# YaqiXia/Voltrix-SpMM

Hardware: AMD Instinct MI355X
Metric: spmm_gflops (higher is better)
Workload: dtype f16

## Files before the change

### include/voltrix_capi.h

```cpp
#ifndef VOLTRIX_CAPI_H_
#define VOLTRIX_CAPI_H_

#include <stdint.h>

#ifdef __cplusplus
extern "C" {
#endif

#define VOLTRIX_ABI_VERSION 2

#define VOLTRIX_CSR_AUTO (-1)
#define VOLTRIX_SLAB_AUTO (-1)
#define VOLTRIX_BLK_H 16
#define VOLTRIX_BLK_W 8

enum voltrix_rc {
  VOLTRIX_OK = 0,
  VOLTRIX_ERR_BAD_SHAPE = 1,
  VOLTRIX_ERR_LAUNCH = 2,
  VOLTRIX_ERR_BAD_CONFIG = 3,
  VOLTRIX_ERR_OVERFLOW = 4,
  VOLTRIX_ERR_DUPLICATE = 5
};

int voltrix_abi_version(void);


void voltrix_launch_preprocess(void* edge_list, void* node_pointer, int num_nodes, void* block_partition,
                               void* edge_to_column, void* edge_to_row, void* pointer1, int* return_code);

void voltrix_launch_hmat_gen(void* node_pointer, void* edge_list, void* block_partition, void* edge_to_column,
                             void* edge_to_row, void* pointer1, int num_row_windows, int num_nodes, int num_edges,
                             void* hspa, void* hind, int* return_code);

void voltrix_launch_hmat_packed_swizzle(int num_row_windows, void* pointer1, void* hspa, void* hspa_packed,
                                        int* return_code);

void voltrix_launch_spmm(void* blk_offsets, void* hspa_packed, void* hind, int num_nodes, int num_edges,
                         int embedding_dim, void* input, void* output, void* stream, int* return_code);


void voltrix_launch_spmm_f32_tile(void* blk_offsets, void* hspa_packed, void* hind, int num_nodes, int num_edges,
                                  int embedding_dim, void* input, void* output, int fs, int depth, int waves,
                                  void* window_order, void* out_scale, void* stream, int* return_code);

void voltrix_launch_spmm_f16(void* blk_offsets, void* hspa_packed, void* hind, int num_nodes, int num_edges,
                             int embedding_dim, void* input, void* output, void* stream, int* return_code);
void voltrix_launch_spmm_f16_tile(void* blk_offsets, void* hspa_packed, void* hind, int num_nodes, int num_edges,
                                  int embedding_dim, void* input, void* output, int fs, int depth, int waves,
                                  void* window_order, void* out_scale, void* stream, int* return_code);

int64_t voltrix_spmm_f32_workspace_bytes(int64_t input_rows, int embedding_dim);
void voltrix_launch_spmm_f32_as_f16(void* blk_offsets, void* hspa_packed, void* hind, int num_nodes, int num_edges,
                                    int embedding_dim, void* input, int64_t input_rows, void* output, void* workspace,
                                    void* stream, int* return_code);

void voltrix_launch_spmm_bf16(void* blk_offsets, void* hspa_packed, void* hind, int num_nodes, int num_edges,
                              int embedding_dim, void* input, void* output, void* stream, int* return_code);
void voltrix_launch_spmm_bf16_tile(void* blk_offsets, void* hspa_packed, void* hind, int num_nodes, int num_edges,
                                   int embedding_dim, void* input, void* output, int fs, int depth, int waves,
                                   void* window_order, void* out_scale, void* stream, int* return_code);

void voltrix_launch_spmm_f16_sched(void* blk_offsets, void* hspa_packed, void* hind, int num_nodes, int num_edges,
                                   int embedding_dim, void* input, void* output, int fs, int depth, int waves,
                                   void* window_order, void* out_scale, int atomic_out, void* units, void* unit_ptr,
                                   int max_units_per_xcd, void* partials, void* row_map, int units_per_wave, void* stream,
                                   int* return_code);
void voltrix_launch_spmm_bf16_sched(void* blk_offsets, void* hspa_packed, void* hind, int num_nodes, int num_edges,
                                    int embedding_dim, void* input, void* output, int fs, int depth, int waves,
                                    void* window_order, void* out_scale, int atomic_out, void* units, void* unit_ptr,
                                    int max_units_per_xcd, void* partials, void* row_map, int units_per_wave, void* stream,
                                    int* return_code);
void voltrix_launch_combine_partials(void* cuts, int num_cuts, void* partials, void* output, int num_nodes,
                                     int embedding_dim, int accumulate, void* row_map, void* stream, int* return_code);

int64_t voltrix_unit_table_workspace_bytes(int num_nodes);
int64_t voltrix_unit_table_fill_workspace_bytes(int64_t num_units);
void voltrix_launch_unit_table_count(void* blk_offsets, int num_nodes, int max_stages, void* xcd_ptr, void* workspace,
                                     void* header, void* stream, int* return_code);
void voltrix_launch_unit_table_fill(void* blk_offsets, int num_nodes, void* xcd_ptr, void* workspace, void* fill_workspace,
                                    int num_units, int num_cuts, int top, void* units, void* unit_ptr, void* cuts,
                                    void* stream, int* return_code);

int64_t voltrix_stream_table_workspace_bytes(int num_nodes);
int64_t voltrix_stream_table_fill_workspace_bytes(int64_t num_units);
void voltrix_launch_stream_table_count(void* blk_offsets, void* hspa_packed, void* hind, int num_nodes, int run_cost,
                                       int cut_stages, void* workspace, void* header, void* stream, int* return_code);
void voltrix_launch_stream_table_fill(void* blk_offsets, int num_nodes, void* workspace, void* fill_workspace, int num_units,
                                      int num_cuts, int run_bound, int run_cost, void* units, void* cuts, void* runs,
                                      void* run_ptr, void* header2, void* stream, int* return_code);
void voltrix_launch_spmm_stream_f16(void* hspa_packed, void* hind, int num_nodes, int embedding_dim, void* input,
                                    int64_t input_rows, void* output, void* units, void* runs, void* run_ptr,
                                    int max_runs_per_xcd, void* partials, void* out_scale, int fs, int depth, int waves,
                                    int slab_policy, void* stream, int* return_code);
void voltrix_launch_spmm_stream_bf16(void* hspa_packed, void* hind, int num_nodes, int embedding_dim, void* input,
                                     int64_t input_rows, void* output, void* units, void* runs, void* run_ptr,
                                     int max_runs_per_xcd, void* partials, void* out_scale, int fs, int depth, int waves,
                                     int slab_policy, void* stream, int* return_code);

void voltrix_launch_window_order(void* blk_offsets, int num_nodes, int chunk, void* order_out, void* stream,
                                 int* return_code);

#define VOLTRIX_PANEL_KSTEPS_PIPELINED 17
void voltrix_launch_spmm_panel_f16(void* panel_ptr, void* panel_cols, void* panel_bits, void* panel_order, void* xcd_ptr,
                                   int max_panels_per_xcd, int num_nodes, int embedding_dim, void* input, int64_t input_rows, void* output,
                                   int accumulate, int fs, int depth, int waves, int row_blocks, int ksteps,
                                   int slab_policy, void* out_scale, void* stream, int* return_code);
void voltrix_launch_spmm_panel_bf16(void* panel_ptr, void* panel_cols, void* panel_bits, void* panel_order, void* xcd_ptr,
                                    int max_panels_per_xcd, int num_nodes, int embedding_dim, void* input, int64_t input_rows, void* output,
                                    int accumulate, int fs, int depth, int waves, int row_blocks, int ksteps,
                                    int slab_policy, void* out_scale, void* stream, int* return_code);

void voltrix_launch_spmm_panel_parts_f16(void* panel_ptr, void* panel_cols, void* panel_bits, void* parts, int num_parts,
                                         void* xcd_ptr, int max_parts_per_xcd, void* partials, int num_nodes, int embedding_dim,
                                         void* input, int64_t input_rows, void* output, int accumulate, int fs, int depth,
                                         int waves, int row_blocks, int ksteps, int slab_policy, void* out_scale, void* stream,
                                         int* return_code);
void voltrix_launch_spmm_panel_parts_bf16(void* panel_ptr, void* panel_cols, void* panel_bits, void* parts, int num_parts,
                                          void* xcd_ptr, int max_parts_per_xcd, void* partials, int num_nodes, int embedding_dim,
                                          void* input, int64_t input_rows, void* output, int accumulate, int fs, int depth,
                                          int waves, int row_blocks, int ksteps, int slab_policy, void* out_scale, void* stream,
                                          int* return_code);
void voltrix_launch_combine_panel_partials(void* cuts, int num_cuts, void* partials, void* output, int num_nodes,
                                           int embedding_dim, int panel_rows, int accumulate, void* stream, int* return_code);

void voltrix_launch_xcd_ranges_of_work(void* work, int num_items, int align, void* xcd_ptr, void* stream, int* return_code);
void voltrix_launch_xcd_ranges_of_windows(void* blk_offsets, int num_nodes, int align, void* xcd_ptr, void* stream,
                                          int* return_code);
void voltrix_launch_xcd_ranges_of_panels(void* panel_ptr, void* resid_blk_offsets, int num_nodes, int panel_rows,
                                         int kstep_cost_x10, void* xcd_ptr, void* window_xcd_ptr, void* stream,
                                         int* return_code);
int64_t voltrix_panel_parts_workspace_bytes(int num_panels);
void voltrix_launch_panel_parts_count(void* panel_ptr, int num_panels, int cap, void* panel_xcd_ptr, void* workspace,
                                      void* header, void* stream, int* return_code);
void voltrix_launch_panel_parts_fill(void* panel_ptr, int num_panels, int cap, void* panel_xcd_ptr, void* workspace,
                                     void* parts, void* part_xcd_ptr, void* cuts, void* stream, int* return_code);

void voltrix_launch_spmm_fused_f16(void* panel_ptr, void* panel_cols, void* panel_bits, void* panel_order, void* xcd_ptr,
                                   int max_panels_per_xcd, void* wave_ptr, void* records, int num_nodes, int embedding_dim, void* input,
                                   void* output, int fs, int depth, int pace_blocks, void* out_scale, void* stream,
                                   int* return_code);
void voltrix_launch_spmm_fused_bf16(void* panel_ptr, void* panel_cols, void* panel_bits, void* panel_order, void* xcd_ptr,
                                    int max_panels_per_xcd, void* wave_ptr, void* records, int num_nodes, int embedding_dim, void* input,
                                    void* output, int fs, int depth, int pace_blocks, void* out_scale, void* stream,
                                   int* return_code);

void voltrix_fused_panel_geometry(int* waves, int* row_blocks);
int64_t voltrix_fused_records_workspace_bytes(int num_nodes);
void voltrix_launch_fused_records_count(void* blk_offsets, void* hspa_packed, int num_nodes, void* workspace, void* wave_ptr,
                                        void* stream, int* return_code);
void voltrix_launch_fused_records_fill(void* blk_offsets, void* hspa_packed, void* hind, int num_nodes, void* wave_ptr,
                                       int64_t num_records, void* records, void* stream, int* return_code);

int64_t voltrix_panel_plan_workspace_bytes(int num_nodes, int waves, int row_blocks);
void voltrix_launch_panel_plan_count(void* node_pointer, void* edge_list, int num_nodes, int num_cols, int64_t num_edges,
                                     int waves, int row_blocks, int tau, void* workspace, void* panel_ptr,
                                     void* resid_node_pointer, void* status, void* stream, int* return_code);
void voltrix_launch_panel_plan_fill(void* node_pointer, void* edge_list, int num_nodes, int num_cols, int64_t num_edges,
                                    int waves, int row_blocks, int tau, void* workspace, void* panel_ptr,
                                    void* resid_node_pointer, int64_t total_ksteps, void* resid_edge_list,
                                    void* panel_cols, void* panel_bits, void* stream, int* return_code);

void voltrix_launch_panel_order(void* panel_ptr, int num_panels, int group, void* xcd_ptr, void* order_out, void* stream,
                                int* return_code);

void voltrix_spmm_default_tile(int embedding_dim, int is_f16, int* fs, int* depth, int* waves);

int voltrix_spmm_num_tiles(int is_f16);
void voltrix_spmm_tile_at(int is_f16, int index, int* fs, int* depth, int* waves);

void voltrix_launch_cast_f32_f16(void* src, void* dst, int64_t count, void* stream, int* return_code);

void voltrix_launch_cast_f32_f16_scaled(void* src, void* dst, int64_t count, void* scale, void* stream,
                                        int* return_code);

void voltrix_launch_spmm_csr_rows(void* indptr, void* indices, int num_rows, int embedding_dim, void* input, int dtype, void* output,
                                  int xcd_ranges, void* stream, int* return_code);

void voltrix_launch_spmm_csr_rows_weighted(void* indptr, void* indices, void* values, int num_rows, int embedding_dim, void* input, int dtype,
                                           void* output, int xcd_ranges, void* stream, int* return_code);

void voltrix_launch_scatter_values(void* values, void* slots, void* plane, int64_t count, int dtype, void* stream, int* return_code);

void voltrix_launch_sddmm_csr(void* indptr, void* indices, int num_rows, int64_t nnz, int embedding_dim, void* x, int x_dtype, void* y,
                              int y_dtype, void* out, void* stream, int* return_code);

int64_t voltrix_edge_softmax_workspace_bytes(int num_rows, int64_t nnz);
void voltrix_launch_edge_softmax_csr(void* indptr, int num_rows, int64_t nnz, void* scores, float scale, void* out, void* workspace,
                                     void* stream, int* return_code);

void voltrix_launch_edge_softmax_backward_csr(void* indptr, int num_rows, int64_t nnz, void* alpha, void* grad_alpha, float scale,
                                              void* grad_scores, void* workspace, void* stream, int* return_code);

void voltrix_launch_sddmm_heads_csr(void* indptr, void* indices, int num_rows, int64_t nnz, int heads, int head_dim, void* x, int x_dtype,
                                    void* y, int y_dtype, void* out, void* stream, int* return_code);

int64_t voltrix_edge_softmax_heads_workspace_bytes(int num_rows, int64_t nnz, int heads);
void voltrix_launch_edge_softmax_heads_csr(void* indptr, int num_rows, int64_t nnz, int heads, void* scores, float scale, void* out,
                                           void* workspace, void* stream, int* return_code);
void voltrix_launch_edge_softmax_heads_backward_csr(void* indptr, int num_rows, int64_t nnz, int heads, void* alpha, void* grad_alpha,
                                                    float scale, void* grad_scores, void* workspace, void* stream, int* return_code);

void voltrix_launch_spmm_csr_heads(void* indptr, void* indices, void* values, int num_rows, int heads, int head_dim, void* input,
                                   int dtype, void* output, void* stream, int* return_code);

void voltrix_launch_gat_score_csr(void* indptr, void* indices, int num_rows, int64_t nnz, int heads, void* el, void* er, float slope,
                                  void* out, void* stream, int* return_code);

int64_t voltrix_gat_score_workspace_bytes(int num_rows, int64_t nnz, int heads);
void voltrix_launch_gat_score_rowsum_csr(void* indptr, void* indices, void* order, int num_rows, int64_t nnz, int heads, void* a, void* b,
                                         void* grad, float slope, void* out, void* workspace, void* stream, int* return_code);

void voltrix_launch_gatv2_score_csr(void* indptr, void* indices, int num_rows, int64_t nnz, int heads, int head_dim, void* xl, void* xr,
                                    int dtype, void* a, float slope, void* out, void* stream, int* return_code);

void voltrix_launch_gatv2_rowsum_csr(void* indptr, void* indices, void* order, int num_rows, int64_t nnz, int heads, int head_dim, void* p,
                                     void* q, int dtype, void* grad, float slope, void* out, void* stream, int* return_code);

void voltrix_launch_attn_aggregate_csr(void* indptr, void* indices, void* scores, int num_rows, int64_t nnz, int heads, int head_dim,
                                       void* feat, int dtype, float scale, void* out, void* m, void* l, void* stream, int* return_code);

void voltrix_launch_attn_aggregate_grad_scores_csr(void* indptr, void* indices, int num_rows, int64_t nnz, int heads, int head_dim,
                                                   void* grad_out, void* feat, int dtype, void* scores, void* m, void* l, void* delta,
                                                   float scale, void* grad_scores, void* stream, int* return_code);

void voltrix_launch_attn_aggregate_grad_feat_csr(void* t_indptr, void* t_indices, void* order, int num_cols, int64_t nnz, int heads,
                                                 int head_dim, void* grad_out, int dtype, void* scores, void* m, void* l, float scale,
                                                 void* grad_feat, void* stream, int* return_code);

void voltrix_launch_dropout_mask(int64_t nnz, int heads, uint32_t threshold, uint64_t seed, uint64_t offset, void* mask, void* stream,
                                 int* return_code);

void voltrix_launch_attn_aggregate_dropout_csr(void* indptr, void* indices, void* scores, int num_rows, int64_t nnz, int heads,
                                               int head_dim, void* feat, int dtype, float scale, void* out, void* m, void* l, void* mask,
                                               float keep_scale, void* stream, int* return_code);
void voltrix_launch_attn_aggregate_dropout_grad_scores_csr(void* indptr, void* indices, int num_rows, int64_t nnz, int heads,
                                                           int head_dim, void* grad_out, void* feat, int dtype, void* scores, void* m,
                                                           void* l, void* delta, float scale, void* grad_scores, void* mask,
                                                           float keep_scale, void* stream, int* return_code);
void voltrix_launch_attn_aggregate_dropout_grad_feat_csr(void* t_indptr, void* t_indices, void* order, int num_cols, int64_t nnz,
                                                         int heads, int head_dim, void* grad_out, int dtype, void* scores, void* m,
                                                         void* l, float scale, void* grad_feat, void* mask, float keep_scale,
                                                         void* stream, int* return_code);

void voltrix_launch_scale_rows(void* src, void* scale, void* dst, int64_t rows, int num_feats, int dtype, void* stream,
                               int* return_code);

int64_t voltrix_csr_preprocess_workspace_bytes(int num_nodes, int num_cols, int64_t num_edges, int path);
void voltrix_launch_csr_window_count(void* node_pointer, void* edge_list, int num_nodes, int num_cols, int64_t num_edges,
                                     int path, void* workspace, void* block_partition, void* pointer1, void* status,
                                     void* stream, int* return_code);
void voltrix_launch_csr_fill(void* node_pointer, void* edge_list, int num_nodes, int num_cols, int64_t num_edges,
                             int path, void* workspace, void* pointer1, void* hspa_packed, void* hind, void* stream,
                             int* return_code);

int64_t voltrix_csr_transpose_workspace_bytes(int64_t num_edges);
void voltrix_launch_csr_transpose(void* indptr, void* indices, int num_rows, int num_cols, int64_t num_edges, void* workspace,
                                  void* t_indptr, void* t_indices, void* stream, int* return_code);
void voltrix_launch_bfs_seed(int start, int num_nodes, void* level, void* queue, void* ctrl, void* level_off, void* stream,
                             int* return_code);
void voltrix_launch_bfs_levels(void* indptr, void* indices, void* t_indptr, void* t_indices, int num_nodes, int t_rows,
                               void* level, void* queue, void* ctrl, void* level_off, int wide_levels, void* stream,
                               int* return_code);
int64_t voltrix_cm_rank_workspace_bytes(int64_t max_level);
void voltrix_launch_cm_rank(void* indptr, void* indices, void* t_indptr, void* t_indices, int num_nodes, int t_rows,
                            void* level, void* rank, void* tie, void* queue, void* level_off, const int* level_off_host,
                            int num_levels, int base, void* workspace, void* stream, int* return_code);

void voltrix_launch_chol_inv_transposed(void* gram, int k, double eps, void* out, void* stream, int* return_code);

#ifdef __cplusplus
}
#endif
#endif
```

### voltrix-spmm_amd/csrc/capi_spmm_panel.hip

```cpp
#include <hip/hip_runtime.h>

#include "voltrix/panel_plan.hpp"
#include "voltrix/spmm_panel_kernels.hpp"
#include "voltrix_capi.h"

namespace {

#define VOLTRIX_PANEL_SPACE(X)                                                                       \
  X(128, 3, 8, 4, 1) X(128, 4, 8, 4, 1) X(128, 6, 8, 4, 1) X(128, 8, 8, 4, 1) X(128, 4, 4, 4, 1) X(128, 6, 4, 4, 1) X(128, 8, 4, 4, 1) \
  X(128, 4, 8, 2, 1) X(128, 6, 8, 2, 1) X(128, 8, 8, 2, 1) X(128, 6, 4, 2, 1)                                    \
  X(64, 4, 4, 4, 1) X(64, 6, 4, 4, 1) X(64, 4, 8, 4, 2) X(64, 6, 8, 4, 2) X(64, 6, 4, 4, 2)                      \
  X(32, 4, 4, 4, 2) X(32, 6, 4, 4, 2) X(32, 6, 8, 4, 2) X(64, 6, 4, 2, 2) X(64, 6, 8, 2, 2) X(32, 6, 4, 2, 2) X(32, 6, 8, 2, 2) \
  X(128, 3, 4, 4, 1) X(128, 4, 4, 2, 1)

constexpr int kPipelined = 17;
static_assert(kPipelined == VOLTRIX_PANEL_KSTEPS_PIPELINED, "include/voltrix_capi.h");
#define VOLTRIX_PANEL_PIPE_SPACE(X) X(128, 3, 8, 4) X(128, 4, 8, 4) X(128, 4, 8, 2) X(128, 6, 8, 2) X(64, 4, 8, 4) X(64, 6, 8, 4)

template <bool BF16>
int dispatch(int fs, int depth, int waves, int rb, int ks, const int* panel_ptr, const int* panel_cols,
             const uint32_t* panel_bits, const int* panel_order, int num_nodes, int embedding_dim, const void* input,
             float* output, int accumulate, const float* out_scale, hipStream_t stream, int64_t input_rows,
             int slab_policy, const int* xcd_ptr, int max_panels_per_xcd, const int* parts = nullptr, int num_parts = 0,
             float* partials = nullptr) {
#define X(FS, D, W, RB, KS)                                                                                          \
  if (fs == FS && depth == D && waves == W && rb == RB && ks == KS)                                                  \
    return voltrix::launch_spmm_panel<voltrix::PanelTile<FS, D, W, RB, KS, BF16>>(                                   \
        panel_ptr, panel_cols, panel_bits, panel_order, num_nodes, embedding_dim, input, output, accumulate, out_scale, \
        stream, 0, 0, input_rows, slab_policy, xcd_ptr, max_panels_per_xcd, parts, num_parts, partials);
  VOLTRIX_PANEL_SPACE(X)
#undef X
#define X(FS, D, W, RB)                                                                                              \
  if (fs == FS && depth == D && waves == W && rb == RB && ks == kPipelined)                                           \
    return voltrix::launch_spmm_panel<voltrix::PanelTile<FS, D, W, RB, 1, BF16, true>>(                               \
        panel_ptr, panel_cols, panel_bits, panel_order, num_nodes, embedding_dim, input, output, accumulate, out_scale, \
        stream, 0, 0, input_rows, slab_policy, xcd_ptr, max_panels_per_xcd, parts, num_parts, partials);
  VOLTRIX_PANEL_PIPE_SPACE(X)
#undef X
  return voltrix::kErrBadConfig;
}

}

extern "C" {

void voltrix_launch_spmm_panel_f16(void* panel_ptr, void* panel_cols, void* panel_bits, void* panel_order, void* xcd_ptr,
                                   int max_panels_per_xcd, int num_nodes, int embedding_dim, void* input, int64_t input_rows, void* output,
                                   int accumulate, int fs, int depth, int waves, int row_blocks, int ksteps,
                                   int slab_policy, void* out_scale, void* stream, int* return_code) {
  *return_code = dispatch<false>(fs, depth, waves, row_blocks, ksteps, static_cast<const int*>(panel_ptr),
                                 static_cast<const int*>(panel_cols), static_cast<const uint32_t*>(panel_bits),
                                 static_cast<const int*>(panel_order), num_nodes, embedding_dim, input,
                                 static_cast<float*>(output), accumulate, static_cast<const float*>(out_scale),
                                 static_cast<hipStream_t>(stream), input_rows, slab_policy,
                                 static_cast<const int*>(xcd_ptr), max_panels_per_xcd);
}

void voltrix_launch_spmm_panel_bf16(void* panel_ptr, void* panel_cols, void* panel_bits, void* panel_order, void* xcd_ptr,
                                    int max_panels_per_xcd, int num_nodes, int embedding_dim, void* input, int64_t input_rows, void* output,
                                    int accumulate, int fs, int depth, int waves, int row_blocks, int ksteps,
                                    int slab_policy, void* out_scale, void* stream, int* return_code) {
  *return_code = dispatch<true>(fs, depth, waves, row_blocks, ksteps, static_cast<const int*>(panel_ptr),
                                static_cast<const int*>(panel_cols), static_cast<const uint32_t*>(panel_bits),
                                static_cast<const int*>(panel_order), num_nodes, embedding_dim, input,
                                static_cast<float*>(output), accumulate, static_cast<const float*>(out_scale),
                                static_cast<hipStream_t>(stream), input_rows, slab_policy,
                                static_cast<const int*>(xcd_ptr), max_panels_per_xcd);
}

void voltrix_launch_spmm_panel_parts_f16(void* panel_ptr, void* panel_cols, void* panel_bits, void* parts, int num_parts,
                                         void* xcd_ptr, int max_parts_per_xcd, void* partials, int num_nodes, int embedding_dim,
                                         void* input, int64_t input_rows, void* output, int accumulate, int fs, int depth,
                                         int waves, int row_blocks, int ksteps, int slab_policy, void* out_scale, void* stream,
                                         int* return_code) {
  *return_code = parts == nullptr ? voltrix::kErrBadShape
                                  : dispatch<false>(fs, depth, waves, row_blocks, ksteps, static_cast<const int*>(panel_ptr),
                                                    static_cast<const int*>(panel_cols), static_cast<const uint32_t*>(panel_bits),
                                                    nullptr, num_nodes, embedding_dim, input, static_cast<float*>(output),
                                                    accumulate, static_cast<const float*>(out_scale),
                                                    static_cast<hipStream_t>(stream), input_rows, slab_policy,
                                                    static_cast<const int*>(xcd_ptr), max_parts_per_xcd,
                                                    static_cast<const int*>(parts), num_parts, static_cast<float*>(partials));
}

void voltrix_launch_spmm_panel_parts_bf16(void* panel_ptr, void* panel_cols, void* panel_bits, void* parts, int num_parts,
                                          void* xcd_ptr, int max_parts_per_xcd, void* partials, int num_nodes, int embedding_dim,
                                          void* input, int64_t input_rows, void* output, int accumulate, int fs, int depth,
                                          int waves, int row_blocks, int ksteps, int slab_policy, void* out_scale, void* stream,
                                          int* return_code) {
  *return_code = parts == nullptr ? voltrix::kErrBadShape
                                  : dispatch<true>(fs, depth, waves, row_blocks, ksteps, static_cast<const int*>(panel_ptr),
                                                   static_cast<const int*>(panel_cols), static_cast<const uint32_t*>(panel_bits),
                                                   nullptr, num_nodes, embedding_dim, input, static_cast<float*>(output),
                                                   accumulate, static_cast<const float*>(out_scale),
                                                   static_cast<hipStream_t>(stream), input_rows, slab_policy,
                                                   static_cast<const int*>(xcd_ptr), max_parts_per_xcd,
                                                   static_cast<const int*>(parts), num_parts, static_cast<float*>(partials));
}

void voltrix_launch_combine_panel_partials(void* cuts, int num_cuts, void* partials, void* output, int num_nodes,
                                           int embedding_dim, int panel_rows, int accumulate, void* stream, int* return_code) {
  *return_code = voltrix::launch_combine_panel_partials(static_cast<const int*>(cuts), num_cuts,
                                                        static_cast<const float*>(partials), static_cast<float*>(output),
                                                        num_nodes, embedding_dim, panel_rows, accumulate,
                                                        static_cast<hipStream_t>(stream));
}

void voltrix_launch_panel_order(void* panel_ptr, int num_panels, int group, void* xcd_ptr, void* order_out, void* stream,
                                int* return_code) {
  *return_code = voltrix::panel_order(static_cast<const int*>(panel_ptr), num_panels, group, static_cast<int*>(order_out),
                                      static_cast<hipStream_t>(stream), static_cast<const int*>(xcd_ptr));
}

int64_t voltrix_panel_plan_workspace_bytes(int num_nodes, int waves, int row_blocks) {
  return voltrix::panel_plan_workspace_bytes(num_nodes, waves, row_blocks);
}

void voltrix_launch_panel_plan_count(void* node_pointer, void* edge_list, int num_nodes, int num_cols, int64_t num_edges,
                                     int waves, int row_blocks, int tau, void* workspace, void* panel_ptr,
                                     void* resid_node_pointer, void* status, void* stream, int* return_code) {
  *return_code = voltrix::panel_plan_count(static_cast<const int*>(node_pointer), static_cast<const int*>(edge_list),
                                           num_nodes, num_cols, num_edges, waves, row_blocks, tau, workspace,
                                           static_cast<int*>(panel_ptr), static_cast<int*>(resid_node_pointer),
                                           static_cast<int*>(status), static_cast<hipStream_t>(stream));
}

void voltrix_launch_panel_plan_fill(void* node_pointer, void* edge_list, int num_nodes, int num_cols, int64_t num_edges,
                                    int waves, int row_blocks, int tau, void* workspace, void* panel_ptr,
                                    void* resid_node_pointer, int64_t total_ksteps, void* resid_edge_list,
                                    void* panel_cols, void* panel_bits, void* stream, int* return_code) {
  *return_code = voltrix::panel_plan_fill(static_cast<const int*>(node_pointer), static_cast<const int*>(edge_list),
                                          num_nodes, num_cols, num_edges, waves, row_blocks, tau, workspace,
                                          static_cast<const int*>(panel_ptr), static_cast<const int*>(resid_node_pointer),
                                          total_ksteps, static_cast<int*>(resid_edge_list), static_cast<int*>(panel_cols),
                                          static_cast<uint32_t*>(panel_bits), static_cast<hipStream_t>(stream));
}

}
```

### voltrix-spmm_amd/voltrix/capi.py

```python
from __future__ import annotations

import ctypes
import os
import subprocess

_PKG = os.path.dirname(os.path.abspath(__file__))
_ROOT = os.path.dirname(_PKG)
LIB_PATH = os.path.join(_ROOT, "lib", "libvoltrix_hip.so")
CSRC_DIR = os.path.join(_ROOT, "csrc")

_lib = None

SYMBOLS = (
    "voltrix_abi_version",
    "voltrix_launch_preprocess",
    "voltrix_launch_hmat_gen",
    "voltrix_launch_hmat_packed_swizzle",
    "voltrix_launch_spmm",
    "voltrix_launch_spmm_f32_tile",
    "voltrix_launch_spmm_f16",
    "voltrix_launch_spmm_f16_tile",
    "voltrix_spmm_f32_workspace_bytes",
    "voltrix_launch_spmm_f32_as_f16",
    "voltrix_launch_spmm_f16_sched",
    "voltrix_launch_spmm_bf16_sched",
    "voltrix_launch_combine_partials",
    "voltrix_stream_table_workspace_bytes",
    "voltrix_stream_table_fill_workspace_bytes",
    "voltrix_launch_stream_table_count",
    "voltrix_launch_stream_table_fill",
    "voltrix_launch_spmm_stream_f16",
    "voltrix_launch_spmm_stream_bf16",
    "voltrix_launch_spmm_panel_f16",
    "voltrix_launch_spmm_panel_bf16",
    "voltrix_launch_spmm_panel_parts_f16",
    "voltrix_launch_spmm_panel_parts_bf16",
    "voltrix_launch_combine_panel_partials",
    "voltrix_launch_xcd_ranges_of_work",
    "voltrix_launch_xcd_ranges_of_windows",
    "voltrix_launch_xcd_ranges_of_panels",
    "voltrix_panel_parts_workspace_bytes",
    "voltrix_launch_panel_parts_count",
    "voltrix_launch_panel_parts_fill",
    "voltrix_launch_spmm_fused_f16",
    "voltrix_launch_spmm_fused_bf16",
    "voltrix_fused_panel_geometry",
    "voltrix_fused_records_workspace_bytes",
    "voltrix_launch_fused_records_count",
    "voltrix_launch_fused_records_fill",
    "voltrix_panel_plan_workspace_bytes",
    "voltrix_launch_panel_plan_count",
    "voltrix_launch_panel_plan_fill",
    "voltrix_launch_panel_order",
    "voltrix_spmm_default_tile",
    "voltrix_spmm_num_tiles",
    "voltrix_spmm_tile_at",
    "voltrix_launch_window_order",
    "voltrix_launch_spmm_bf16",
    "voltrix_launch_spmm_bf16_tile",
    "voltrix_launch_cast_f32_f16",
    "voltrix_launch_cast_f32_f16_scaled",
    "voltrix_launch_scale_rows",
    "voltrix_launch_spmm_csr_rows",
    "voltrix_launch_spmm_csr_rows_weighted",
    "voltrix_launch_scatter_values",
    "voltrix_launch_sddmm_csr",
    "voltrix_edge_softmax_workspace_bytes",
    "voltrix_launch_edge_softmax_csr",
    "voltrix_launch_edge_softmax_backward_csr",
    "voltrix_launch_sddmm_heads_csr",
    "voltrix_edge_softmax_heads_workspace_bytes",
    "voltrix_launch_edge_softmax_heads_csr",
    "voltrix_launch_edge_softmax_heads_backward_csr",
    "voltrix_launch_spmm_csr_heads",
    "voltrix_launch_gat_score_csr",
    "voltrix_gat_score_workspace_bytes",
    "voltrix_launch_gat_score_rowsum_csr",
    "voltrix_launch_gatv2_score_csr",
    "voltrix_launch_gatv2_rowsum_csr",
    "voltrix_launch_attn_aggregate_csr",
    "voltrix_launch_attn_aggregate_grad_scores_csr",
    "voltrix_launch_attn_aggregate_grad_feat_csr",
    "voltrix_launch_dropout_mask",
    "voltrix_launch_attn_aggregate_dropout_csr",
    "voltrix_launch_attn_aggregate_dropout_grad_scores_csr",
    "voltrix_launch_attn_aggregate_dropout_grad_feat_csr",
    "voltrix_csr_preprocess_workspace_bytes",
    "voltrix_launch_csr_window_count",
    "voltrix_launch_csr_fill",
    "voltrix_unit_table_workspace_bytes",
    "voltrix_unit_table_fill_workspace_bytes",
    "voltrix_launch_unit_table_count",
    "voltrix_launch_unit_table_fill",
    "voltrix_csr_transpose_workspace_bytes",
    "voltrix_launch_csr_transpose",
    "voltrix_launch_bfs_seed",
    "voltrix_launch_bfs_levels",
    "voltrix_cm_rank_workspace_bytes",
    "voltrix_launch_cm_rank",
    "voltrix_launch_chol_inv_transposed",
)


def build(force: bool = False) -> str:
    cmd = ["make", "-s", "-C", CSRC_DIR, "-j4"]
    if force:
        subprocess.check_call(["make", "-s", "-C", CSRC_DIR, "clean"])
    subprocess.check_call(cmd)
    return LIB_PATH


def lib() -> ctypes.CDLL:
    global _lib
    if _lib is None:
        if not os.path.exists(LIB_PATH):
            build()
        _lib = ctypes.CDLL(LIB_PATH)
        _lib.voltrix_abi_version.restype = ctypes.c_int
        _lib.voltrix_spmm_num_tiles.restype = ctypes.c_int
        _lib.voltrix_csr_preprocess_workspace_bytes.restype = ctypes.c_int64
        _lib.voltrix_panel_plan_workspace_bytes.restype = ctypes.c_int64
        _lib.voltrix_spmm_f32_workspace_bytes.restype = ctypes.c_int64
        _lib.voltrix_fused_records_workspace_bytes.restype = ctypes.c_int64
        _lib.voltrix_unit_table_workspace_bytes.restype = ctypes.c_int64
        _lib.voltrix_unit_table_fill_workspace_bytes.restype = ctypes.c_int64
        _lib.voltrix_cm_rank_workspace_bytes.restype = ctypes.c_int64
        _lib.voltrix_csr_transpose_workspace_bytes.restype = ctypes.c_int64
        _lib.voltrix_edge_softmax_workspace_bytes.restype = ctypes.c_int64
        _lib.voltrix_edge_softmax_heads_workspace_bytes.restype = ctypes.c_int64
        _lib.voltrix_gat_score_workspace_bytes.restype = ctypes.c_int64
        for name in SYMBOLS:
            if name.startswith("voltrix_launch_") or name in ("voltrix_spmm_default_tile", "voltrix_spmm_tile_at"):
                getattr(_lib, name).restype = None
    return _lib


class VoltrixError(RuntimeError):
    pass


_RC = {1: "bad shape / alignment", 2: "HIP launch error", 3: "tile configuration not instantiated",
       4: "int32 overflow of the block format", 5: "duplicate CSR entries"}


def check(rc: int, what: str) -> None:
    if rc != 0:
        raise VoltrixError(f"{what}: return code {rc} ({_RC.get(rc, 'unknown')})")


def _ptr(t):
    return ctypes.c_void_p(t.data_ptr())


def default_tile(embedding_dim: int, is_f16: bool):
    fs, d, w = ctypes.c_int(), ctypes.c_int(), ctypes.c_int()
    lib().voltrix_spmm_default_tile(ctypes.c_int(embedding_dim), ctypes.c_int(int(is_f16)), ctypes.byref(fs),
                                    ctypes.byref(d), ctypes.byref(w))
    return fs.value, d.value, w.value


def tiles(is_f16: bool):
    out = []
    for i in range(lib().voltrix_spmm_num_tiles(ctypes.c_int(int(is_f16)))):
        fs, d, w = ctypes.c_int(), ctypes.c_int(), ctypes.c_int()
        lib().voltrix_spmm_tile_at(ctypes.c_int(int(is_f16)), ctypes.c_int(i), ctypes.byref(fs), ctypes.byref(d),
                                   ctypes.byref(w))
        out.append((fs.value, d.value, w.value))
    return out


CSR_PATHS = {None: -1, "auto": -1, "sort": 0, "bitmap": 1, "mixed": 2}
SLAB_AUTO, SLAB_ONE_GRID, SLAB_LAUNCHES = -1, 0, 1


def csr_preprocess_workspace_bytes(num_nodes: int, num_cols: int, num_edges: int, path=None) -> int:
    return int(lib().voltrix_csr_preprocess_workspace_bytes(ctypes.c_int(num_nodes), ctypes.c_int(num_cols),
                                                            ctypes.c_int64(num_edges), ctypes.c_int(CSR_PATHS[path])))


def launch_csr_window_count(indptr, indices, num_nodes, num_cols, workspace, block_partition, pointer1, status,
                            stream, path=None) -> None:
    rc = ctypes.c_int(-1)
    lib().voltrix_launch_csr_window_count(_ptr(indptr), _ptr(indices), ctypes.c_int(num_nodes), ctypes.c_int(num_cols),
                                          ctypes.c_int64(indices.numel()), ctypes.c_int(CSR_PATHS[path]), _ptr(workspace),
                                          _ptr(block_partition), _ptr(pointer1), _ptr(status), ctypes.c_void_p(stream),
                                          ctypes.byref(rc))
    check(rc.value, "voltrix_launch_csr_window_count")


def launch_csr_fill(indptr, indices, num_nodes, num_cols, workspace, pointer1, hspa_packed, hind, stream, path=None) -> None:
    rc = ctypes.c_int(-1)
    lib().voltrix_launch_csr_fill(_ptr(indptr), _ptr(indices), ctypes.c_int(num_nodes), ctypes.c_int(num_cols),
                                  ctypes.c_int64(indices.numel()), ctypes.c_int(CSR_PATHS[path]), _ptr(workspace),
                                  _ptr(pointer1), _ptr(hspa_packed), _ptr(hind), ctypes.c_void_p(stream), ctypes.byref(rc))
    check(rc.value, "voltrix_launch_csr_fill")


def launch_spmm(blk_offsets, hspa_packed, hind, num_nodes, num_edges, embedding_dim, input_ptr, output_ptr, is_f16,
                tile, stream, window_order=0, out_scale=0) -> int:
    rc = ctypes.c_int(-1)
    if is_f16 == "bf16":
        fn = lib().voltrix_launch_spmm_bf16_tile
    else:
        fn = lib().voltrix_launch_spmm_f16_tile if is_f16 else lib().voltrix_launch_spmm_f32_tile
    fn(ctypes.c_void_p(blk_offsets), ctypes.c_void_p(hspa_packed), ctypes.c_void_p(hind), ctypes.c_int(num_nodes),
       ctypes.c_int(num_edges), ctypes.c_int(embedding_dim), ctypes.c_void_p(input_ptr), ctypes.c_void_p(output_ptr),
       ctypes.c_int(tile[0]), ctypes.c_int(tile[1]), ctypes.c_int(tile[2]), ctypes.c_void_p(window_order),
       ctypes.c_void_p(out_scale), ctypes.c_void_p(stream), ctypes.byref(rc))
    return rc.value


def launch_spmm_sched(blk_offsets, hspa_packed, hind, num_nodes, num_edges, embedding_dim, input_ptr, output_ptr, tile,
                      stream, window_order=0, out_scale=0, atomic_out=False, bf16=False, table=None, partials=0,
                      row_map=0, units_per_wave=1) -> int:
    rc = ctypes.c_int(-1)
    fn = lib().voltrix_launch_spmm_bf16_sched if bf16 else lib().voltrix_launch_spmm_f16_sched
    fn(ctypes.c_void_p(blk_offsets), ctypes.c_void_p(hspa_packed), ctypes.c_void_p(hind), ctypes.c_int(num_nodes),
       ctypes.c_int(num_edges), ctypes.c_int(embedding_dim), ctypes.c_void_p(input_ptr), ctypes.c_void_p(output_ptr),
       ctypes.c_int(tile[0]), ctypes.c_int(tile[1]), ctypes.c_int(tile[2]), ctypes.c_void_p(window_order),
       ctypes.c_void_p(out_scale), ctypes.c_int(int(atomic_out)),
       ctypes.c_void_p(table.units.data_ptr() if table is not None else 0),
       ctypes.c_void_p(table.unit_ptr.data_ptr() if table is not None else 0),
       ctypes.c_int(table.max_units_per_xcd if table is not None else 0), ctypes.c_void_p(partials),
       ctypes.c_void_p(row_map), ctypes.c_int(int(units_per_wave)), ctypes.c_void_p(stream), ctypes.byref(rc))
    return rc.value


def launch_combine_partials(table, partials_ptr, output_ptr, num_nodes, embedding_dim, accumulate, stream,
                            row_map=0) -> int:
    rc = ctypes.c_int(-1)
    lib().voltrix_launch_combine_partials(ctypes.c_void_p(table.cuts.data_ptr()), ctypes.c_int(table.num_cuts),
                                          ctypes.c_void_p(partials_ptr), ctypes.c_void_p(output_ptr),
                                          ctypes.c_int(num_nodes), ctypes.c_int(embedding_dim),
                                          ctypes.c_int(int(accumulate)), ctypes.c_void_p(row_map),
                                          ctypes.c_void_p(stream), ctypes.byref(rc))
    return rc.value


def build_unit_table(blk_offsets, num_nodes: int, max_stages: int = 0, stream=None, xcd_ptr=None):
    import torch

    dev = blk_offsets.device
    stream = torch.cuda.current_stream().cuda_stream if stream is None else stream
    workspace = torch.empty(max(16, int(lib().voltrix_unit_table_workspace_bytes(ctypes.c_int(num_nodes)))),
                            dtype=torch.uint8, device=dev)
    header = torch.empty(8, dtype=torch.int32, device=dev)
    rc = ctypes.c_int(-1)
    xp = ctypes.c_void_p(xcd_ptr.data_ptr() if xcd_ptr is not None else 0)
    lib().voltrix_launch_unit_table_count(_ptr(blk_offsets), ctypes.c_int(num_nodes), ctypes.c_int(int(max_stages)), xp,
                                          _ptr(workspace), _ptr(header), ctypes.c_void_p(stream), ctypes.byref(rc))
    check(rc.value, "voltrix_launch_unit_table_count")
    head = [int(v) for v in header.tolist()]
    num_units, num_cuts, top = head[0], head[1], head[5]
    units = torch.empty((num_units, 4), dtype=torch.int32, device=dev)
    cuts = torch.empty((num_cuts, 4), dtype=torch.int32, device=dev)
    unit_ptr = torch.empty(9, dtype=torch.int32, device=dev)
    fill_ws = torch.empty(max(16, int(lib().voltrix_unit_table_fill_workspace_bytes(ctypes.c_int64(num_units)))),
                          dtype=torch.uint8, device=dev)
    lib().voltrix_launch_unit_table_fill(_ptr(blk_offsets), ctypes.c_int(num_nodes), xp, _ptr(workspace), _ptr(fill_ws),
                                         ctypes.c_int(num_units), ctypes.c_int(num_cuts), ctypes.c_int(top), _ptr(units),
                                         _ptr(unit_ptr), _ptr(cuts), ctypes.c_void_p(stream), ctypes.byref(rc))
    check(rc.value, "voltrix_launch_unit_table_fill")
    return units, unit_ptr, cuts, head


def build_stream_table(blk_offsets, hspa_packed, hind, num_nodes: int, run_cost: int = 0, cut_stages: int = 0, stream=None):
    import torch

    dev = blk_offsets.device
    stream = torch.cuda.current_stream().cuda_stream if stream is None else stream
    L = lib()
    workspace = torch.empty(max(16, int(L.voltrix_stream_table_workspace_bytes(ctypes.c_int(num_nodes)))), dtype=torch.uint8,
                            device=dev)
    header = torch.empty(8, dtype=torch.int32, device=dev)
    rc = ctypes.c_int(-1)
    L.voltrix_launch_stream_table_count(_ptr(blk_offsets), _ptr(hspa_packed), _ptr(hind), ctypes.c_int(num_nodes),
                                        ctypes.c_int(int(run_cost)), ctypes.c_int(int(cut_stages)), _ptr(workspace),
                                        _ptr(header), ctypes.c_void_p(stream), ctypes.byref(rc))
    check(rc.value, "voltrix_launch_stream_table_count")
    num_units, num_cuts, num_slots, run_bound, rcost, cut = [int(v) for v in header.tolist()][:6]
    units = torch.empty((num_units, 8), dtype=torch.int32, device=dev)
    cuts = torch.empty((num_cuts, 4), dtype=torch.int32, device=dev)
    runs = torch.empty((max(1, run_bound), 4), dtype=torch.int32, device=dev)
    run_ptr = torch.empty(9, dtype=torch.int32, device=dev)
    header2 = torch.empty(4, dtype=torch.int32, device=dev)
    fill_ws = torch.empty(max(16, int(L.voltrix_stream_table_fill_workspace_bytes(ctypes.c_int64(num_units)))),
                          dtype=torch.uint8, device=dev)
    L.voltrix_launch_stream_table_fill(_ptr(blk_offsets), ctypes.c_int(num_nodes), _ptr(workspace), _ptr(fill_ws),
                                       ctypes.c_int(num_units), ctypes.c_int(num_cuts), ctypes.c_int(run_bound),
                                       ctypes.c_int(max(2, rcost)), _ptr(units), _ptr(cuts), _ptr(runs), _ptr(run_ptr),
                                       _ptr(header2), ctypes.c_void_p(stream), ctypes.byref(rc))
    check(rc.value, "voltrix_launch_stream_table_fill")
    num_runs, max_runs, oversized = [int(v) for v in header2.tolist()][:3]
    assert oversized == 0, "stream table with a run of more than 64 units (run_cost > 128?): the kernel cannot walk it"
    return units, runs[:num_runs], run_ptr, cuts, (num_units, num_cuts, num_slots, num_runs, max_runs, rcost, cut)


def launch_spmm_stream(hspa_packed, hind, num_nodes: int, embedding_dim: int, feat, output, table, partials, out_scale=None,
                       tile=(0, 0, 0), stream=None, input_rows: int = 0, slab_policy: int = -1) -> int:
    import torch

    stream = torch.cuda.current_stream().cuda_stream if stream is None else stream
    fn = lib().voltrix_launch_spmm_stream_bf16 if feat.dtype == torch.bfloat16 else lib().voltrix_launch_spmm_stream_f16
    from .utils import timed_launch

    rc = ctypes.c_int(-1)
    with timed_launch("spmm_stream", stream):
        fn(_ptr(hspa_packed), _ptr(hind), ctypes.c_int(num_nodes), ctypes.c_int(embedding_dim), _ptr(feat),
           ctypes.c_int64(int(input_rows)), _ptr(output), _ptr(table.units), _ptr(table.runs), _ptr(table.run_ptr),
           ctypes.c_int(table.max_runs_per_xcd), _ptr(partials), ctypes.c_void_p(out_scale.data_ptr() if out_scale is not None else 0),
           ctypes.c_int(tile[0]), ctypes.c_int(tile[1]), ctypes.c_int(tile[2]), ctypes.c_int(int(slab_policy)),
           ctypes.c_void_p(stream), ctypes.byref(rc))
    return rc.value


def xcd_ranges_of_work(work, align: int = 1, stream=None):
    import torch

    out = torch.empty(9, dtype=torch.int32, device=work.device)
    rc = ctypes.c_int(-1)
    stream = torch.cuda.current_stream().cuda_stream if stream is None else stream
    lib().voltrix_launch_xcd_ranges_of_work(_ptr(work), ctypes.c_int(work.numel()), ctypes.c_int(int(align)), _ptr(out),
                                            ctypes.c_void_p(stream), ctypes.byref(rc))
    check(rc.value, "voltrix_launch_xcd_ranges_of_work")
    return out


def xcd_ranges_of_windows(blk_offsets, num_nodes: int, align: int = 1, stream=None):
    import torch

    out = torch.empty(9, dtype=torch.int32, device=blk_offsets.device)
    rc = ctypes.c_int(-1)
    stream = torch.cuda.current_stream().cuda_stream if stream is None else stream
    lib().voltrix_launch_xcd_ranges_of_windows(_ptr(blk_offsets), ctypes.c_int(num_nodes), ctypes.c_int(int(align)), _ptr(out),
                                               ctypes.c_void_p(stream), ctypes.byref(rc))
    check(rc.value, "voltrix_launch_xcd_ranges_of_windows")
    return out


def xcd_ranges_of_panels(panel_ptr, resid_blk_offsets, num_nodes: int, panel_rows: int, kstep_cost_x10: int, stream=None):
    import torch

    dev = panel_ptr.device
    out, out_w = torch.empty(9, dtype=torch.int32, device=dev), torch.empty(9, dtype=torch.int32, device=dev)
    rc = ctypes.c_int(-1)
    stream = torch.cuda.current_stream().cuda_stream if stream is None else stream
    lib().voltrix_launch_xcd_ranges_of_panels(_ptr(panel_ptr), _ptr(resid_blk_offsets), ctypes.c_int(num_nodes),
                                              ctypes.c_int(panel_rows), ctypes.c_int(int(kstep_cost_x10)), _ptr(out),
                                              _ptr(out_w), ctypes.c_void_p(stream), ctypes.byref(rc))
    check(rc.value, "voltrix_launch_xcd_ranges_of_panels")
    return out, out_w


def build_panel_parts(panel_ptr, cap: int, panel_xcd_ptr=None, stream=None):
    import torch

    dev = panel_ptr.device
    num_panels = panel_ptr.numel() - 1
    stream = torch.cuda.current_stream().cuda_stream if stream is None else stream
    workspace = torch.empty(max(16, int(lib().voltrix_panel_parts_workspace_bytes(ctypes.c_int(num_panels)))),
                            dtype=torch.uint8, device=dev)
    header = torch.empty(8, dtype=torch.int32, device=dev)
    rc = ctypes.c_int(-1)
    xp = ctypes.c_void_p(panel_xcd_ptr.data_ptr() if panel_xcd_ptr is not None else 0)
    lib().voltrix_launch_panel_parts_count(_ptr(panel_ptr), ctypes.c_int(num_panels), ctypes.c_int(int(cap)), xp,
                                           _ptr(workspace), _ptr(header), ctypes.c_void_p(stream), ctypes.byref(rc))
    check(rc.value, "voltrix_launch_panel_parts_count")
    head = [int(v) for v in header.tolist()]
    parts = torch.empty((head[0], 4), dtype=torch.int32, device=dev)
    cuts = torch.empty((max(1, head[1]), 4), dtype=torch.int32, device=dev)
    part_xcd_ptr = torch.empty(9, dtype=torch.int32, device=dev)
    lib().voltrix_launch_panel_parts_fill(_ptr(panel_ptr), ctypes.c_int(num_panels), ctypes.c_int(int(cap)), xp,
                                          _ptr(workspace), _ptr(parts), _ptr(part_xcd_ptr), _ptr(cuts),
                                          ctypes.c_void_p(stream), ctypes.byref(rc))
    check(rc.value, "voltrix_launch_panel_parts_fill")
    return parts, part_xcd_ptr, cuts[:head[1]], head


def spmm_f32_workspace_bytes(input_rows: int, embedding_dim: int) -> int:
    return int(lib().voltrix_spmm_f32_workspace_bytes(ctypes.c_int64(input_rows), ctypes.c_int(embedding_dim)))


def launch_spmm_f32_as_f16(blk_offsets, hspa_packed, hind, num_nodes, num_edges, embedding_dim, feat, output, workspace,
                           stream) -> int:
    rc = ctypes.c_int(-1)
    lib().voltrix_launch_spmm_f32_as_f16(_ptr(blk_offsets), _ptr(hspa_packed), _ptr(hind), ctypes.c_int(num_nodes),
                                         ctypes.c_int(num_edges), ctypes.c_int(embedding_dim), _ptr(feat),
                                         ctypes.c_int64(feat.shape[0]), _ptr(output), _ptr(workspace),
                                         ctypes.c_void_p(stream), ctypes.byref(rc))
    return rc.value


def launch_spmm_panel(plan, input_ptr, output_ptr, embedding_dim, accumulate, bf16, tile, out_scale, stream,
                      input_rows: int = 0, slab_policy: int = SLAB_AUTO, partials_ptr: int = 0) -> int:
    rc = ctypes.c_int(-1)
    parts = getattr(plan, "parts", None)
    if parts is not None:
        fn = lib().voltrix_launch_spmm_panel_parts_bf16 if bf16 else lib().voltrix_launch_spmm_panel_parts_f16
        fn(_ptr(plan.panel_ptr), _ptr(plan.panel_cols), _ptr(plan.panel_bits), _ptr(parts.parts), ctypes.c_int(parts.num_parts),
           _ptr(parts.xcd_ptr), ctypes.c_int(parts.max_parts_per_xcd), ctypes.c_void_p(partials_ptr),
           ctypes.c_int(plan.num_nodes), ctypes.c_int(embedding_dim), ctypes.c_void_p(input_ptr), ctypes.c_int64(input_rows),
           ctypes.c_void_p(output_ptr), ctypes.c_int(int(accumulate)), ctypes.c_int(tile[0]), ctypes.c_int(tile[1]),
           ctypes.c_int(plan.waves), ctypes.c_int(plan.row_blocks), ctypes.c_int(tile[2]), ctypes.c_int(slab_policy),
           ctypes.c_void_p(out_scale), ctypes.c_void_p(stream), ctypes.byref(rc))
        return rc.value
    fn = lib().voltrix_launch_spmm_panel_bf16 if bf16 else lib().voltrix_launch_spmm_panel_f16
    order = plan.panel_order.data_ptr() if plan.panel_order is not None else 0
    xcd_ptr = getattr(plan, "xcd_ptr", None)
    fn(_ptr(plan.panel_ptr), _ptr(plan.panel_cols), _ptr(plan.panel_bits), ctypes.c_void_p(order),
       ctypes.c_void_p(xcd_ptr.data_ptr() if xcd_ptr is not None else 0),
       ctypes.c_int(plan.max_panels_per_xcd if xcd_ptr is not None else 0), ctypes.c_int(plan.num_nodes), ctypes.c_int(embedding_dim), ctypes.c_void_p(input_ptr), ctypes.c_int64(input_rows),
       ctypes.c_void_p(output_ptr), ctypes.c_int(int(accumulate)), ctypes.c_int(tile[0]), ctypes.c_int(tile[1]),
       ctypes.c_int(plan.waves), ctypes.c_int(plan.row_blocks), ctypes.c_int(tile[2]), ctypes.c_int(slab_policy),
       ctypes.c_void_p(out_scale), ctypes.c_void_p(stream), ctypes.byref(rc))
    return rc.value


def launch_combine_panel_partials(parts, partials_ptr, output_ptr, num_nodes, embedding_dim, panel_rows, accumulate,
                                  stream) -> int:
    rc = ctypes.c_int(-1)
    lib().voltrix_launch_combine_panel_partials(_ptr(parts.cuts), ctypes.c_int(parts.num_cuts), ctypes.c_void_p(partials_ptr),
                                                ctypes.c_void_p(output_ptr), ctypes.c_int(num_nodes),
                                                ctypes.c_int(embedding_dim), ctypes.c_int(panel_rows),
                                                ctypes.c_int(int(accumulate)), ctypes.c_void_p(stream), ctypes.byref(rc))
    return rc.value


def launch_spmm_fused(plan, fused, input_ptr, output_ptr, embedding_dim, bf16, tile, out_scale, stream,
                      pace_blocks: int = 0) -> int:
    rc = ctypes.c_int(-1)
    fn = lib().voltrix_launch_spmm_fused_bf16 if bf16 else lib().voltrix_launch_spmm_fused_f16
    order = plan.panel_order.data_ptr() if plan.panel_order is not None else 0
    xcd_ptr = getattr(plan, "xcd_ptr", None)
    fn(_ptr(plan.panel_ptr), _ptr(plan.panel_cols), _ptr(plan.panel_bits), ctypes.c_void_p(order),
       ctypes.c_void_p(xcd_ptr.data_ptr() if xcd_ptr is not None else 0),
       ctypes.c_int(plan.max_panels_per_xcd if xcd_ptr is not None else 0), _ptr(fused.wave_ptr),
       _ptr(fused.records), ctypes.c_int(plan.num_nodes), ctypes.c_int(embedding_dim), ctypes.c_void_p(input_ptr),
       ctypes.c_void_p(output_ptr), ctypes.c_int(tile[0]), ctypes.c_int(tile[1]), ctypes.c_int(int(pace_blocks)),
       ctypes.c_void_p(out_scale), ctypes.c_void_p(stream), ctypes.byref(rc))
    return rc.value


def fused_panel_geometry():
    waves, row_blocks = ctypes.c_int(0), ctypes.c_int(0)
    lib().voltrix_fused_panel_geometry(ctypes.byref(waves), ctypes.byref(row_blocks))
    assert waves.value * row_blocks.value * 16 == 512, (waves.value, row_blocks.value)
    return waves.value, row_blocks.value


def build_fused_records(blk_offsets, hspa_packed, hind, num_nodes: int, stream=None):
    import torch

    dev = blk_offsets.device
    stream = torch.cuda.current_stream().cuda_stream if stream is None else stream
    num_waves = fused_panel_geometry()[0] * ((num_nodes + 511) // 512)
    workspace = torch.empty(max(16, int(lib().voltrix_fused_records_workspace_bytes(ctypes.c_int(num_nodes)))),
                            dtype=torch.uint8, device=dev)
    wave_ptr = torch.empty(num_waves + 1, dtype=torch.int32, device=dev)
    rc = ctypes.c_int(-1)
    lib().voltrix_launch_fused_records_count(_ptr(blk_offsets), _ptr(hspa_packed), ctypes.c_int(num_nodes), _ptr(workspace),
                                             _ptr(wave_ptr), ctypes.c_void_p(stream), ctypes.byref(rc))
    check(rc.value, "voltrix_launch_fused_records_count")
    num_records = int(wave_ptr[-1])
    assert 0 <= num_records <= 4 * (hspa_packed.numel() // 16 + 1), num_records
    records = torch.empty((num_records + 1, 64), dtype=torch.int32, device=dev).view(torch.uint32)
    lib().voltrix_launch_fused_records_fill(_ptr(blk_offsets), _ptr(hspa_packed), _ptr(hind), ctypes.c_int(num_nodes),
                                            _ptr(wave_ptr), ctypes.c_int64(num_records), _ptr(records),
                                            ctypes.c_void_p(stream), ctypes.byref(rc))
    check(rc.value, "voltrix_launch_fused_records_fill")
    return wave_ptr, records, num_records


def launch_panel_order(panel_ptr, num_panels: int, order_out, stream, group: int = 1, xcd_ptr=None) -> None:
    rc = ctypes.c_int(-1)
    lib().voltrix_launch_panel_order(_ptr(panel_ptr), ctypes.c_int(num_panels), ctypes.c_int(group),
                                     ctypes.c_void_p(xcd_ptr.data_ptr() if xcd_ptr is not None else 0), _ptr(order_out),
                                     ctypes.c_void_p(stream), ctypes.byref(rc))
    check(rc.value, "voltrix_launch_panel_order")


def panel_plan_workspace_bytes(num_nodes: int, waves: int, row_blocks: int) -> int:
    return int(lib().voltrix_panel_plan_workspace_bytes(ctypes.c_int(num_nodes), ctypes.c_int(waves),
                                                        ctypes.c_int(row_blocks)))


def launch_panel_plan_count(indptr, indices, num_nodes, num_cols, waves, row_blocks, tau, workspace, panel_ptr,
                            resid_indptr, status, stream) -> int:
    rc = ctypes.c_int(-1)
    lib().voltrix_launch_panel_plan_count(_ptr(indptr), _ptr(indices), ctypes.c_int(num_nodes), ctypes.c_int(num_cols),
                                          ctypes.c_int64(indices.numel()), ctypes.c_int(waves), ctypes.c_int(row_blocks),
                                          ctypes.c_int(tau), _ptr(workspace), _ptr(panel_ptr), _ptr(resid_indptr),
                                          _ptr(status), ctypes.c_void_p(stream), ctypes.byref(rc))
    return rc.value


def launch_panel_plan_fill(indptr, indices, num_nodes, num_cols, waves, row_blocks, tau, workspace, panel_ptr,
                           resid_indptr, total_ksteps, resid_indices, panel_cols, panel_bits, stream) -> None:
    rc = ctypes.c_int(-1)
    lib().voltrix_launch_panel_plan_fill(_ptr(indptr), _ptr(indices), ctypes.c_int(num_nodes), ctypes.c_int(num_cols),
                                         ctypes.c_int64(indices.numel()), ctypes.c_int(waves), ctypes.c_int(row_blocks),
                                         ctypes.c_int(tau), _ptr(workspace), _ptr(panel_ptr), _ptr(resid_indptr),
                                         ctypes.c_int64(total_ksteps), _ptr(resid_indices), _ptr(panel_cols),
                                         _ptr(panel_bits), ctypes.c_void_p(stream), ctypes.byref(rc))
    check(rc.value, "voltrix_launch_panel_plan_fill")


def launch_window_order(blk_offsets, num_nodes, order_out, stream, chunk: int = 256) -> None:
    rc = ctypes.c_int(-1)
    lib().voltrix_launch_window_order(_ptr(blk_offsets), ctypes.c_int(num_nodes), ctypes.c_int(chunk), _ptr(order_out),
                                      ctypes.c_void_p(stream), ctypes.byref(rc))
    check(rc.value, "voltrix_launch_window_order")


def launch_cast_f32_f16(src, dst, stream) -> None:
    rc = ctypes.c_int(-1)
    lib().voltrix_launch_cast_f32_f16(_ptr(src), _ptr(dst), ctypes.c_int64(src.numel()), ctypes.c_void_p(stream),
                                      ctypes.byref(rc))
    check(rc.value, "voltrix_launch_cast_f32_f16")


_cast_scaled = None


def launch_cast_f32_f16_scaled(src, dst, scale, stream) -> None:
    global _cast_scaled
    if _cast_scaled is None:
        fn = lib().voltrix_launch_cast_f32_f16_scaled
        fn.argtypes = [ctypes.c_void_p, ctypes.c_void_p, ctypes.c_int64, ctypes.c_void_p, ctypes.c_void_p,
                       ctypes.POINTER(ctypes.c_int)]
        _cast_scaled = fn
    rc = ctypes.c_int(-1)
    _cast_scaled(src.data_ptr(), dst.data_ptr(), src.numel(), scale.data_ptr(), stream, rc)
    if rc.value != 0:
        check(rc.value, "voltrix_launch_cast_f32_f16_scaled")


_P, _I, _L, _F, _RC_P = ctypes.c_void_p, ctypes.c_int, ctypes.c_int64, ctypes.c_float, ctypes.POINTER(ctypes.c_int)
_U32, _U64 = ctypes.c_uint32, ctypes.c_uint64
_ARGTYPES = {
    "voltrix_launch_spmm_csr_rows": [_P, _P, _I, _I, _P, _I, _P, _I, _P, _RC_P],
    "voltrix_launch_spmm_csr_rows_weighted": [_P, _P, _P, _I, _I, _P, _I, _P, _I, _P, _RC_P],
    "voltrix_launch_sddmm_csr": [_P, _P, _I, _L, _I, _P, _I, _P, _I, _P, _P, _RC_P],
    "voltrix_launch_edge_softmax_csr": [_P, _I, _L, _P, _F, _P, _P, _P, _RC_P],
    "voltrix_launch_edge_softmax_backward_csr": [_P, _I, _L, _P, _P, _F, _P, _P, _P, _RC_P],
    "voltrix_launch_sddmm_heads_csr": [_P, _P, _I, _L, _I, _I, _P, _I, _P, _I, _P, _P, _RC_P],
    "voltrix_launch_edge_softmax_heads_csr": [_P, _I, _L, _I, _P, _F, _P, _P, _P, _RC_P],
    "voltrix_launch_edge_softmax_heads_backward_csr": [_P, _I, _L, _I, _P, _P, _F, _P, _P, _P, _RC_P],
    "voltrix_launch_spmm_csr_heads": [_P, _P, _P, _I, _I, _I, _P, _I, _P, _P, _RC_P],
    "voltrix_launch_gat_score_csr": [_P, _P, _I, _L, _I, _P, _P, _F, _P, _P, _RC_P],
    "voltrix_launch_gat_score_rowsum_csr": [_P, _P, _P, _I, _L, _I, _P, _P, _P, _F, _P, _P, _P, _RC_P],
    "voltrix_launch_gatv2_score_csr": [_P, _P, _I, _L, _I, _I, _P, _P, _I, _P, _F, _P, _P, _RC_P],
    "voltrix_launch_gatv2_rowsum_csr": [_P, _P, _P, _I, _L, _I, _I, _P, _P, _I, _P, _F, _P, _P, _RC_P],
    "voltrix_launch_attn_aggregate_csr": [_P, _P, _P, _I, _L, _I, _I, _P, _I, _F, _P, _P, _P, _P, _RC_P],
    "voltrix_launch_attn_aggregate_grad_scores_csr": [_P, _P, _I, _L, _I, _I, _P, _P, _I, _P, _P, _P, _P, _F, _P, _P, _RC_P],
    "voltrix_launch_attn_aggregate_grad_feat_csr": [_P, _P, _P, _I, _L, _I, _I, _P, _I, _P, _P, _P, _F, _P, _P, _RC_P],
    "voltrix_launch_dropout_mask": [_L, _I, _U32, _U64, _U64, _P, _P, _RC_P],
    "voltrix_launch_attn_aggregate_dropout_csr": [_P, _P, _P, _I, _L, _I, _I, _P, _I, _F, _P, _P, _P, _P, _F, _P, _RC_P],
    "voltrix_launch_attn_aggregate_dropout_grad_scores_csr": [_P, _P, _I, _L, _I, _I, _P, _P, _I, _P, _P, _P, _P, _F, _P, _P, _F, _P,
                                                              _RC_P],
    "voltrix_launch_attn_aggregate_dropout_grad_feat_csr": [_P, _P, _P, _I, _L, _I, _I, _P, _I, _P, _P, _P, _F, _P, _P, _F, _P, _RC_P],
    "voltrix_launch_scatter_values": [_P, _P, _P, _L, _I, _P, _RC_P],
    "voltrix_launch_scale_rows": [_P, _P, _P, _L, _I, _I, _P, _RC_P],
}
_bound_fns = {}


def _bound(name: str):
    fn = _bound_fns.get(name)
    if fn is None:
        fn = getattr(lib(), name)
        fn.argtypes = _ARGTYPES[name]
        _bound_fns[name] = fn
    return fn


def launch_spmm_csr_rows(indptr, indices, num_rows: int, feat, output, stream, xcd_ranges: int = 0, values=None) -> None:
    import torch

    assert indptr.dtype == torch.int32 and indices.dtype == torch.int32 and indptr.numel() == num_rows + 1
    assert feat.dim() == 2 and feat.is_contiguous() and output.is_contiguous() and output.dtype == torch.float32
    assert output.shape == (num_rows, feat.shape[1])
    dtype = {torch.float32: 0, torch.float16: 1, torch.bfloat16: 2}[feat.dtype]
    rc = ctypes.c_int(-1)
    if values is None:
        _bound("voltrix_launch_spmm_csr_rows")(indptr.data_ptr(), indices.data_ptr(), num_rows, feat.shape[1], feat.data_ptr(), dtype,
                                               output.data_ptr(), int(xcd_ranges), stream, rc)
        check(rc.value, "voltrix_launch_spmm_csr_rows")
        return
    assert values.dtype == torch.float32 and values.is_contiguous() and values.numel() == indices.numel() and values.is_cuda
    _bound("voltrix_launch_spmm_csr_rows_weighted")(indptr.data_ptr(), indices.data_ptr(), values.data_ptr(), num_rows, feat.shape[1],
                                                    feat.data_ptr(), dtype, output.data_ptr(), int(xcd_ranges), stream, rc)
    check(rc.value, "voltrix_launch_spmm_csr_rows_weighted")


def launch_sddmm_csr(indptr, indices, num_rows: int, x, y, out, stream) -> None:
    import torch

    assert indptr.dtype == torch.int32 and indices.dtype == torch.int32 and indptr.numel() == num_rows + 1
    assert x.dim() == 2 and y.dim() == 2 and x.is_contiguous() and y.is_contiguous() and x.shape[0] == num_rows
    assert x.shape[1] == y.shape[1] and out.dtype == torch.float32 and out.is_contiguous() and out.numel() == indices.numel()
    codes = {torch.float32: 0, torch.float16: 1, torch.bfloat16: 2}
    rc = ctypes.c_int(-1)
    _bound("voltrix_launch_sddmm_csr")(indptr.data_ptr(), indices.data_ptr(), num_rows, indices.numel(), x.shape[1], x.data_ptr(),
                                       codes[x.dtype], y.data_ptr(), codes[y.dtype], out.data_ptr(), stream, rc)
    check(rc.value, "voltrix_launch_sddmm_csr")


def edge_softmax_workspace_bytes(num_rows: int, nnz: int) -> int:
    return int(lib().voltrix_edge_softmax_workspace_bytes(ctypes.c_int(num_rows), ctypes.c_int64(nnz)))


def launch_edge_softmax_csr(indptr, num_rows: int, scores, scale: float, out, workspace, stream) -> None:
    import torch

    assert indptr.dtype == torch.int32 and indptr.numel() == num_rows + 1 and indptr.is_contiguous()
    assert scores.dtype == torch.float32 and out.dtype == torch.float32 and scores.is_contiguous() and out.is_contiguous()
    assert out.numel() == scores.numel() and workspace.numel() >= edge_softmax_workspace_bytes(num_rows, scores.numel())
    rc = ctypes.c_int(-1)
    _bound("voltrix_launch_edge_softmax_csr")(indptr.data_ptr(), num_rows, scores.numel(), scores.data_ptr(), float(scale), out.data_ptr(),
                                              workspace.data_ptr(), stream, rc)
    check(rc.value, "voltrix_launch_edge_softmax_csr")


def launch_edge_softmax_backward_csr(indptr, num_rows: int, alpha, grad_alpha, scale: float, grad_scores, workspace, stream) -> None:
    import torch

    assert indptr.dtype == torch.int32 and indptr.numel() == num_rows + 1 and indptr.is_contiguous()
    for t in (alpha, grad_alpha, grad_scores):
        assert t.dtype == torch.float32 and t.is_contiguous() and t.numel() == alpha.numel()
    assert workspace.numel() >= edge_softmax_workspace_bytes(num_rows, alpha.numel())
    rc = ctypes.c_int(-1)
    _bound("voltrix_launch_edge_softmax_backward_csr")(indptr.data_ptr(), num_rows, alpha.numel(), alpha.data_ptr(), grad_alpha.data_ptr(),
                                                       float(scale), grad_scores.data_ptr(), workspace.data_ptr(), stream, rc)
    check(rc.value, "voltrix_launch_edge_softmax_backward_csr")


_CODES = None


def _dtype_code(dtype) -> int:
    import torch

    global _CODES
    if _CODES is None:
        _CODES = {torch.float32: 0, torch.float16: 1, torch.bfloat16: 2}
    return _CODES[dtype]


def launch_sddmm_heads_csr(indptr, indices, num_rows: int, x, y, out, stream) -> None:
    import torch

    assert indptr.dtype == torch.int32 and indices.dtype == torch.int32 and indptr.numel() == num_rows + 1
    assert x.dim() == 3 and y.dim() == 3 and x.is_contiguous() and y.is_contiguous() and x.shape[0] == num_rows
    assert x.shape[1:] == y.shape[1:] and out.dtype == torch.float32 and out.is_contiguous()
    assert out.shape == (indices.numel(), x.shape[1])
    rc = ctypes.c_int(-1)
    _bound("voltrix_launch_sddmm_heads_csr")(indptr.data_ptr(), indices.data_ptr(), num_rows, indices.numel(), x.shape[1], x.shape[2],
                                             x.data_ptr(), _dtype_code(x.dtype), y.data_ptr(), _dtype_code(y.dtype), out.data_ptr(), stream,
                                             rc)
    check(rc.value, "voltrix_launch_sddmm_heads_csr")


def edge_softmax_heads_workspace_bytes(num_rows: int, nnz: int, heads: int) -> int:
    return int(lib().voltrix_edge_softmax_heads_workspace_bytes(ctypes.c_int(num_rows), ctypes.c_int64(nnz), ctypes.c_int(heads)))


def launch_edge_softmax_heads_csr(indptr, num_rows: int, scores, scale: float, out, workspace, stream) -> None:
    import torch

    assert indptr.dtype == torch.int32 and indptr.numel() == num_rows + 1 and indptr.is_contiguous()
    assert scores.dim() == 2 and scores.dtype == torch.float32 and out.dtype == torch.float32
    assert scores.is_contiguous() and out.is_contiguous() and out.shape == scores.shape
    nnz, heads = scores.shape
    assert workspace.numel() >= edge_softmax_heads_workspace_bytes(num_rows, nnz, heads)
    rc = ctypes.c_int(-1)
    _bound("voltrix_launch_edge_softmax_heads_csr")(indptr.data_ptr(), num_rows, nnz, heads, scores.data_ptr(), float(scale),
                                                    out.data_ptr(), workspace.data_ptr(), stream, rc)
    check(rc.value, "voltrix_launch_edge_softmax_heads_csr")


def launch_edge_softmax_heads_backward_csr(indptr, num_rows: int, alpha, grad_alpha, scale: float, grad_scores, workspace, stream) -> None:
    import torch

    assert indptr.dtype == torch.int32 and indptr.numel() == num_rows + 1 and indptr.is_contiguous()
    for t in (alpha, grad_alpha, grad_scores):
        assert t.dim() == 2 and t.dtype == torch.float32 and t.is_contiguous() and t.shape == alpha.shape
    nnz, heads = alpha.shape
    assert workspace.numel() >= edge_softmax_heads_workspace_bytes(num_rows, nnz, heads)
    rc = ctypes.c_int(-1)
    _bound("voltrix_launch_edge_softmax_heads_backward_csr")(indptr.data_ptr(), num_rows, nnz, heads, alpha.data_ptr(),
                                                             grad_alpha.data_ptr(), float(scale), grad_scores.data_ptr(),
                                                             workspace.data_ptr(), stream, rc)
    check(rc.value, "voltrix_launch_edge_softmax_heads_backward_csr")


def launch_spmm_csr_heads(indptr, indices, values, num_rows: int, feat, output, stream) -> None:
    import torch

    assert indptr.dtype == torch.int32 and indices.dtype == torch.int32 and indptr.numel() == num_rows + 1
    assert feat.dim() == 3 and feat.is_contiguous() and output.is_contiguous() and output.dtype == torch.float32
    assert output.shape == (num_rows,) + tuple(feat.shape[1:])
    assert values.dtype == torch.float32 and values.is_contiguous() and values.shape == (indices.numel(), feat.shape[1])
    rc = ctypes.c_int(-1)
    _bound("voltrix_launch_spmm_csr_heads")(indptr.data_ptr(), indices.data_ptr(), values.data_ptr(), num_rows, feat.shape[1],
                                            feat.shape[2], feat.data_ptr(), _dtype_code(feat.dtype), output.data_ptr(), stream, rc)
    check(rc.value, "voltrix_launch_spmm_csr_heads")




def gat_score_workspace_bytes(num_rows: int, nnz: int, heads: int = 1) -> int:
    return int(lib().voltrix_gat_score_workspace_bytes(ctypes.c_int(num_rows), ctypes.c_int64(nnz), ctypes.c_int(heads)))


def launch_gat_score_csr(indptr, indices, num_rows: int, el, er, slope: float, out, stream) -> None:
    import torch

    assert indptr.dtype == torch.int32 and indices.dtype == torch.int32 and indptr.numel() == num_rows + 1
    assert indptr.is_contiguous() and indices.is_contiguous()
    for t in (el, er, out):
        assert t.dim() == 2 and t.dtype == torch.float32 and t.is_contiguous() and t.shape[1] == out.shape[1]
    assert el.shape[0] == num_rows and out.shape[0] == indices.numel()
    rc = ctypes.c_int(-1)
    _bound("voltrix_launch_gat_score_csr")(indptr.data_ptr(), indices.data_ptr(), num_rows, indices.numel(), out.shape[1], el.data_ptr(),
                                           er.data_ptr(), float(slope), out.data_ptr(), stream, rc)
    check(rc.value, "voltrix_launch_gat_score_csr")


def launch_gat_score_rowsum_csr(indptr, indices, order, num_rows: int, a, b, grad, slope: float, out, workspace, stream) -> None:
    import torch

    assert indptr.dtype == torch.int32 and indices.dtype == torch.int32 and indptr.numel() == num_rows + 1
    assert indptr.is_contiguous() and indices.is_contiguous()
    nnz, heads = grad.shape
    for t in (a, b, grad, out):
        assert t.dim() == 2 and t.dtype == torch.float32 and t.is_contiguous() and t.shape[1] == heads
    assert a.shape[0] == num_rows and out.shape[0] == num_rows and nnz == indices.numel()
    if order is not None:
        assert order.dtype == torch.int32 and order.is_contiguous() and order.numel() == nnz
    assert workspace.numel() >= gat_score_workspace_bytes(num_rows, nnz, heads)
    rc = ctypes.c_int(-1)
    _bound("voltrix_launch_gat_score_rowsum_csr")(indptr.data_ptr(), indices.data_ptr(), order.data_ptr() if order is not None else None,
                                                  num_rows, nnz, heads, a.data_ptr(), b.data_ptr(), grad.data_ptr(), float(slope),
                                                  out.data_ptr(), workspace.data_ptr(), stream, rc)
    check(rc.value, "voltrix_launch_gat_score_rowsum_csr")




def launch_gatv2_score_csr(indptr, indices, num_rows: int, xl, xr, a, slope: float, out, stream) -> None:
    import torch

    assert indptr.dtype == torch.int32 and indices.dtype == torch.int32 and indptr.numel() == num_rows + 1
    assert indptr.is_contiguous() and indices.is_contiguous()
    assert xl.dim() == 3 and xr.dim() == 3 and xl.is_contiguous() and xr.is_contiguous() and xl.shape[0] == num_rows
    assert xl.shape[1:] == xr.shape[1:] and xl.dtype == xr.dtype
    assert a.dtype == torch.float32 and a.is_contiguous() and a.shape == xl.shape[1:]
    assert out.dtype == torch.float32 and out.is_contiguous() and out.shape == (indices.numel(), xl.shape[1])
    rc = ctypes.c_int(-1)
    _bound("voltrix_launch_gatv2_score_csr")(indptr.data_ptr(), indices.data_ptr(), num_rows, indices.numel(), xl.shape[1], xl.shape[2],
                                             xl.data_ptr(), xr.data_ptr(), _dtype_code(xl.dtype), a.data_ptr(), float(slope),
                                             out.data_ptr(), stream, rc)
    check(rc.value, "voltrix_launch_gatv2_score_csr")


def launch_gatv2_rowsum_csr(indptr, indices, order, num_rows: int, p, q, grad, slope: float, out, stream) -> None:
    import torch

    assert indptr.dtype == torch.int32 and indices.dtype == torch.int32 and indptr.numel() == num_rows + 1
    assert indptr.is_contiguous() and indices.is_contiguous()
    assert p.dim() == 3 and q.dim() == 3 and p.is_contiguous() and q.is_contiguous() and p.shape[0] == num_rows
    assert p.shape[1:] == q.shape[1:] and p.dtype == q.dtype
    nnz, heads = grad.shape
    assert grad.dtype == torch.float32 and grad.is_contiguous() and nnz == indices.numel() and heads == p.shape[1]
    assert out.dtype == torch.float32 and out.is_contiguous() and out.shape == p.shape
    if order is not None:
        assert order.dtype == torch.int32 and order.is_contiguous() and order.numel() == nnz
    rc = ctypes.c_int(-1)
    _bound("voltrix_launch_gatv2_rowsum_csr")(indptr.data_ptr(), indices.data_ptr(), order.data_ptr() if order is not None else None,
                                              num_rows, nnz, heads, p.shape[2], p.data_ptr(), q.data_ptr(), _dtype_code(p.dtype),
                                              grad.data_ptr(), float(slope), out.data_ptr(), stream, rc)
    check(rc.value, "voltrix_launch_gatv2_rowsum_csr")




def _check_keep_mask(mask, nnz: int, heads: int) -> None:
    import torch

    assert mask.dtype == torch.int32 and mask.is_contiguous() and mask.is_cuda and mask.shape == (nnz, (heads + 31) // 32), \
        (mask.dtype, tuple(mask.shape), nnz, heads)


def launch_dropout_mask(nnz: int, heads: int, threshold: int, seed: int, offset: int, mask, stream) -> None:
    _check_keep_mask(mask, nnz, heads)
    assert 0 <= threshold < 2 ** 32 and 0 <= seed < 2 ** 64 and 0 <= offset < 2 ** 64
    rc = ctypes.c_int(-1)
    _bound("voltrix_launch_dropout_mask")(nnz, heads, threshold, seed, offset, mask.data_ptr(), stream, rc)
    check(rc.value, "voltrix_launch_dropout_mask")


def launch_attn_aggregate_csr(indptr, indices, scores, num_rows: int, feat, scale: float, out, m, l, stream, mask=None,
                              keep_scale: float = 1.0) -> None:
    import torch

    assert indptr.dtype == torch.int32 and indices.dtype == torch.int32 and indptr.numel() == num_rows + 1
    assert indptr.is_contiguous() and indices.is_contiguous()
    assert feat.dim() == 3 and feat.is_contiguous() and out.is_contiguous() and out.dtype == torch.float32
    heads = feat.shape[1]
    assert out.shape == (num_rows,) + tuple(feat.shape[1:])
    assert scores.dtype == torch.float32 and scores.is_contiguous() and scores.shape == (indices.numel(), heads)
    for t in (m, l):
        assert t.dtype == torch.float32 and t.is_contiguous() and t.shape == (num_rows, heads)
    rc = ctypes.c_int(-1)
    if mask is not None:
        _check_keep_mask(mask, indices.numel(), heads)
        _bound("voltrix_launch_attn_aggregate_dropout_csr")(indptr.data_ptr(), indices.data_ptr(), scores.data_ptr(), num_rows,
                                                            indices.numel(), heads, feat.shape[2], feat.data_ptr(),
                                                            _dtype_code(feat.dtype), float(scale), out.data_ptr(), m.data_ptr(),
                                                            l.data_ptr(), mask.data_ptr(), float(keep_scale), stream, rc)
        check(rc.value, "voltrix_launch_attn_aggregate_dropout_csr")
        return
    _bound("voltrix_launch_attn_aggregate_csr")(indptr.data_ptr(), indices.data_ptr(), scores.data_ptr(), num_rows, indices.numel(), heads,
                                                feat.shape[2], feat.data_ptr(), _dtype_code(feat.dtype), float(scale), out.data_ptr(),
                                                m.data_ptr(), l.data_ptr(), stream, rc)
    check(rc.value, "voltrix_launch_attn_aggregate_csr")


def launch_attn_aggregate_grad_scores_csr(indptr, indices, num_rows: int, grad_out, feat, scores, m, l, delta, scale: float, out,
                                          stream, mask=None, keep_scale: float = 1.0) -> None:
    import torch

    assert indptr.dtype == torch.int32 and indices.dtype == torch.int32 and indptr.numel() == num_rows + 1
    assert indptr.is_contiguous() and indices.is_contiguous()
    assert grad_out.dim() == 3 and feat.dim() == 3 and grad_out.is_contiguous() and feat.is_contiguous()
    assert grad_out.dtype == torch.float32 and grad_out.shape[0] == num_rows and grad_out.shape[1:] == feat.shape[1:]
    nnz, heads = indices.numel(), feat.shape[1]
    for t in (scores, out):
        assert t.dtype == torch.float32 and t.is_contiguous() and t.shape == (nnz, heads)
    for t in (m, l, delta):
        assert t.dtype == torch.float32 and t.is_contiguous() and t.shape == (num_rows, heads)
    rc = ctypes.c_int(-1)
    if mask is not None:
        _check_keep_mask(mask, nnz, heads)
        _bound("voltrix_launch_attn_aggregate_dropout_grad_scores_csr")(indptr.data_ptr(), indices.data_ptr(), num_rows, nnz, heads,
                                                                        feat.shape[2], grad_out.data_ptr(), feat.data_ptr(),
                                                                        _dtype_code(feat.dtype), scores.data_ptr(), m.data_ptr(),
                                                                        l.data_ptr(), delta.data_ptr(), float(scale), out.data_ptr(),
                                                                        mask.data_ptr(), float(keep_scale), stream, rc)
        check(rc.value, "voltrix_launch_attn_aggregate_dropout_grad_scores_csr")
        return
    _bound("voltrix_launch_attn_aggregate_grad_scores_csr")(indptr.data_ptr(), indices.data_ptr(), num_rows, nnz, heads, feat.shape[2],
                                                            grad_out.data_ptr(), feat.data_ptr(), _dtype_code(feat.dtype),
                                                            scores.data_ptr(), m.data_ptr(), l.data_ptr(), delta.data_ptr(), float(scale),
                                                            out.data_ptr(), stream, rc)
    check(rc.value, "voltrix_launch_attn_aggregate_grad_scores_csr")


def launch_attn_aggregate_grad_feat_csr(t_indptr, t_indices, order, num_cols: int, grad_out, scores, m, l, scale: float, out,
                                        stream, mask=None, keep_scale: float = 1.0) -> None:
    import torch

    assert t_indptr.dtype == torch.int32 and t_indices.dtype == torch.int32 and t_indptr.numel() == num_cols + 1
    assert t_indptr.is_contiguous() and t_indices.is_contiguous()
    nnz = t_indices.numel()
    assert order.dtype == torch.int32 and order.is_contiguous() and order.numel() == nnz
    assert grad_out.dim() == 3 and grad_out.is_contiguous() and out.is_contiguous() and out.dtype == torch.float32
    heads = grad_out.shape[1]
    assert out.shape == (num_cols,) + tuple(grad_out.shape[1:])
    assert scores.dtype == torch.float32 and scores.is_contiguous() and scores.shape == (nnz, heads)
    for t in (m, l):
        assert t.dtype == torch.float32 and t.is_contiguous() and t.shape == (grad_out.shape[0], heads)
    rc = ctypes.c_int(-1)
    if mask is not None:
        _check_keep_mask(mask, nnz, heads)
        _bound("voltrix_launch_attn_aggregate_dropout_grad_feat_csr")(t_indptr.data_ptr(), t_indices.data_ptr(), order.data_ptr(),
                                                                      num_cols, nnz, heads, grad_out.shape[2], grad_out.data_ptr(),
                                                                      _dtype_code(grad_out.dtype), scores.data_ptr(), m.data_ptr(),
                                                                      l.data_ptr(), float(scale), out.data_ptr(), mask.data_ptr(),
                                                                      float(keep_scale), stream, rc)
        check(rc.value, "voltrix_launch_attn_aggregate_dropout_grad_feat_csr")
        return
    _bound("voltrix_launch_attn_aggregate_grad_feat_csr")(t_indptr.data_ptr(), t_indices.data_ptr(), order.data_ptr(), num_cols, nnz, heads,
                                                          grad_out.shape[2], grad_out.data_ptr(), _dtype_code(grad_out.dtype),
                                                          scores.data_ptr(), m.data_ptr(), l.data_ptr(), float(scale), out.data_ptr(),
                                                          stream, rc)
    check(rc.value, "voltrix_launch_attn_aggregate_grad_feat_csr")


def launch_scatter_values(values, slots, plane, stream) -> None:
    import torch

    assert values.dtype == torch.float32 and slots.dtype == torch.int64 and values.numel() == slots.numel()
    assert values.is_contiguous() and slots.is_contiguous() and plane.is_contiguous() and values.is_cuda and plane.is_cuda
    dtype = {torch.float32: 0, torch.float16: 1, torch.bfloat16: 2}[plane.dtype]
    rc = ctypes.c_int(-1)
    _bound("voltrix_launch_scatter_values")(values.data_ptr(), slots.data_ptr(), plane.data_ptr(), values.numel(), dtype, stream, rc)
    check(rc.value, "voltrix_launch_scatter_values")


def launch_scale_rows(src, scale, dst, stream) -> None:
    import torch

    assert src.dim() == 2 and src.is_contiguous() and dst.is_contiguous() and dst.shape == src.shape and dst.dtype == src.dtype
    assert scale.dtype == torch.float32 and scale.numel() == src.shape[0] and scale.is_contiguous()
    dtype = {torch.float32: 0, torch.float16: 1, torch.bfloat16: 2}[src.dtype]
    rc = ctypes.c_int(-1)
    _bound("voltrix_launch_scale_rows")(src.data_ptr(), scale.data_ptr(), dst.data_ptr(), src.shape[0], src.shape[1], dtype, stream, rc)
    check(rc.value, "voltrix_launch_scale_rows")


def _timed(fn, name, stream_index=None, stream_kw="stream"):
    import functools

    @functools.wraps(fn)
    def wrapper(*args, **kwargs):
        from .utils import KernelTimer

        if KernelTimer.active is None:
            return fn(*args, **kwargs)
        stream = kwargs.get(stream_kw)
        if stream is None and stream_index is not None and len(args) > stream_index:
            stream = args[stream_index]
        with KernelTimer.active.bracket(name, stream):
            return fn(*args, **kwargs)

    return wrapper


launch_spmm = _timed(launch_spmm, "spmm", 10)
launch_spmm_sched = _timed(launch_spmm_sched, "spmm", 9)
launch_spmm_panel = _timed(launch_spmm_panel, "spmm_panel", 8)
launch_spmm_fused = _timed(launch_spmm_fused, "spmm_fused", 8)
launch_combine_partials = _timed(launch_combine_partials, "combine_partials", 6)
launch_cast_f32_f16_scaled = _timed(launch_cast_f32_f16_scaled, "cast_f32_f16_scaled", 3)
launch_cast_f32_f16 = _timed(launch_cast_f32_f16, "cast_f32_f16", 2)
launch_scale_rows = _timed(launch_scale_rows, "scale_rows", 3)
launch_spmm_csr_rows = _timed(launch_spmm_csr_rows, "spmm_csr_rows", 5)
launch_sddmm_csr = _timed(launch_sddmm_csr, "sddmm_csr", 6)
launch_edge_softmax_csr = _timed(launch_edge_softmax_csr, "edge_softmax_csr", 6)
launch_edge_softmax_backward_csr = _timed(launch_edge_softmax_backward_csr, "edge_softmax_backward_csr", 7)
launch_sddmm_heads_csr = _timed(launch_sddmm_heads_csr, "sddmm_heads_csr", 6)
launch_edge_softmax_heads_csr = _timed(launch_edge_softmax_heads_csr, "edge_softmax_heads_csr", 6)
launch_edge_softmax_heads_backward_csr = _timed(launch_edge_softmax_heads_backward_csr, "edge_softmax_heads_backward_csr", 7)
launch_spmm_csr_heads = _timed(launch_spmm_csr_heads, "spmm_csr_heads", 6)
launch_gat_score_csr = _timed(launch_gat_score_csr, "gat_score_csr", 7)
launch_gat_score_rowsum_csr = _timed(launch_gat_score_rowsum_csr, "gat_score_rowsum_csr", 10)
launch_gatv2_score_csr = _timed(launch_gatv2_score_csr, "gatv2_score_csr", 8)
launch_gatv2_rowsum_csr = _timed(launch_gatv2_rowsum_csr, "gatv2_rowsum_csr", 9)
launch_attn_aggregate_csr = _timed(launch_attn_aggregate_csr, "attn_aggregate_csr", 9)
launch_attn_aggregate_grad_scores_csr = _timed(launch_attn_aggregate_grad_scores_csr, "attn_aggregate_grad_scores_csr", 11)
launch_attn_aggregate_grad_feat_csr = _timed(launch_attn_aggregate_grad_feat_csr, "attn_aggregate_grad_feat_csr", 10)
launch_spmm_f32_as_f16 = _timed(launch_spmm_f32_as_f16, "spmm_f32_as_f16", 9)
launch_window_order = _timed(launch_window_order, "window_order", 3)
launch_csr_window_count = _timed(launch_csr_window_count, "csr_window_count", 8)
launch_csr_fill = _timed(launch_csr_fill, "csr_fill", 8)


def csr_transpose(indptr, indices, num_rows: int, num_cols: int, stream=None):
    import torch

    dev = indptr.device
    stream = torch.cuda.current_stream().cuda_stream if stream is None else stream
    nnz = int(indices.numel())
    ws = torch.empty(max(16, int(lib().voltrix_csr_transpose_workspace_bytes(ctypes.c_int64(nnz)))), dtype=torch.uint8,
                     device=dev)
    t_indptr = torch.empty(num_cols + 1, dtype=torch.int32, device=dev)
    t_indices = torch.empty(nnz, dtype=torch.int32, device=dev)
    rc = ctypes.c_int(-1)
    lib().voltrix_launch_csr_transpose(_ptr(indptr), _ptr(indices), ctypes.c_int(num_rows), ctypes.c_int(num_cols),
                                       ctypes.c_int64(nnz), _ptr(ws), _ptr(t_indptr), _ptr(t_indices),
                                       ctypes.c_void_p(stream), ctypes.byref(rc))
    check(rc.value, "voltrix_launch_csr_transpose")
    return t_indptr, t_indices


def chol_inv_transposed(gram, eps: float = 1e-10, stream=None):
    import torch

    k = gram.shape[0]
    assert gram.is_cuda and gram.dtype == torch.float32 and gram.shape == (k, k) and gram.is_contiguous()
    out = torch.empty_like(gram)
    stream = torch.cuda.current_stream().cuda_stream if stream is None else stream
    rc = ctypes.c_int(-1)
    lib().voltrix_launch_chol_inv_transposed(_ptr(gram), ctypes.c_int(k), ctypes.c_double(eps), _ptr(out),
                                             ctypes.c_void_p(stream), ctypes.byref(rc))
    check(rc.value, "voltrix_launch_chol_inv_transposed")
    return out


class CmSearch:

    def __init__(self, indptr, indices, t_indptr, t_indices, num_nodes: int, t_rows: int, tie):
        import torch

        dev = indptr.device
        self.graph = (indptr, indices, t_indptr, t_indices)
        self.n, self.t_rows, self.tie = num_nodes, t_rows, tie
        self.level = torch.full((num_nodes,), -1, dtype=torch.int32, device=dev)
        self.rank = torch.full((num_nodes,), -1, dtype=torch.int32, device=dev)
        self.queue = torch.empty(num_nodes, dtype=torch.int32, device=dev)
        self.level_off = torch.zeros(num_nodes + 2, dtype=torch.int32, device=dev)
        self.ctrl = torch.zeros(8, dtype=torch.int32, device=dev)
        self.syncs = 0

    def _graph_args(self):
        a, b, c, d = self.graph
        return (_ptr(a), _ptr(b), _ptr(c), _ptr(d), ctypes.c_int(self.n), ctypes.c_int(self.t_rows))

    def levels(self, start: int, wide_levels: int = 4, stream=None):
        import torch

        stream = torch.cuda.current_stream().cuda_stream if stream is None else stream
        rc = ctypes.c_int(-1)
        lib().voltrix_launch_bfs_seed(ctypes.c_int(int(start)), ctypes.c_int(self.n), _ptr(self.level), _ptr(self.queue),
                                      _ptr(self.ctrl), _ptr(self.level_off), ctypes.c_void_p(stream), ctypes.byref(rc))
        check(rc.value, "voltrix_launch_bfs_seed")
        while True:
            lib().voltrix_launch_bfs_levels(*self._graph_args(), _ptr(self.level), _ptr(self.queue), _ptr(self.ctrl),
                                            _ptr(self.level_off), ctypes.c_int(wide_levels), ctypes.c_void_p(stream),
                                            ctypes.byref(rc))
            check(rc.value, "voltrix_launch_bfs_levels")
            ctrl = self.ctrl.tolist()
            self.syncs += 1
            if ctrl[4]:
                return ctrl[1], ctrl[3] + 1

    def rank_component(self, levels: int, base: int, stream=None):
        import torch

        stream = torch.cuda.current_stream().cuda_stream if stream is None else stream
        offsets = self.level_off[:levels + 1].cpu()
        self.syncs += 1
        sizes = (offsets[1:] - offsets[:-1])
        big = int(sizes[sizes > 1024].max()) if bool((sizes > 1024).any()) else 0
        ws = torch.empty(max(16, int(lib().voltrix_cm_rank_workspace_bytes(ctypes.c_int64(big)))), dtype=torch.uint8,
                         device=self.level.device)
        host = (ctypes.c_int * (levels + 1))(*offsets.tolist())
        rc = ctypes.c_int(-1)
        lib().voltrix_launch_cm_rank(*self._graph_args(), _ptr(self.level), _ptr(self.rank), _ptr(self.tie), _ptr(self.queue),
                                     _ptr(self.level_off), host, ctypes.c_int(levels), ctypes.c_int(int(base)), _ptr(ws),
                                     ctypes.c_void_p(stream), ctypes.byref(rc))
        check(rc.value, "voltrix_launch_cm_rank")
        return offsets
```

### voltrix-spmm_amd/voltrix/hybrid.py

```python
from __future__ import annotations

import contextlib
import contextvars
import dataclasses
import os

import torch

from . import capi

DEFAULT_WAVES = 8
DEFAULT_ROW_BLOCKS = 4
DEFAULT_TAU = 3
KSTEP = 32
FUSED_WAVES = 4
FUSED_ROW_BLOCKS = 8


@dataclasses.dataclass
class PanelParts:
    parts: torch.Tensor
    cuts: torch.Tensor
    xcd_ptr: torch.Tensor
    max_parts_per_xcd: int
    num_parts: int
    num_cuts: int
    num_slots: int
    cap: int


@dataclasses.dataclass
class PanelPlan:
    panel_ptr: torch.Tensor
    panel_cols: torch.Tensor
    panel_bits: torch.Tensor
    panel_order: torch.Tensor
    num_nodes: int
    waves: int
    row_blocks: int
    tau: int
    num_ksteps: int
    num_shared_edges: int
    num_resid_edges: int
    xcd_ptr: torch.Tensor = None
    max_panels_per_xcd: int = 0
    parts: PanelParts = None

    @property
    def panel_rows(self) -> int:
        return self.waves * self.row_blocks * 16

    @property
    def num_panels(self) -> int:
        return (self.num_nodes + self.panel_rows - 1) // self.panel_rows


@dataclasses.dataclass(eq=False)
class TwoLevelHandle:
    blk_offsets: torch.Tensor
    hspa_packed: torch.Tensor
    hind: torch.Tensor
    plan: PanelPlan
    num_nodes: int
    num_edges: int
    hash_tag: str = None
    fused: "FusedRecords" = None
    window_xcd_ptr: torch.Tensor = None
    format_choice: dict = dataclasses.field(default_factory=dict)

    @property
    def residual(self):
        return self.blk_offsets, self.hspa_packed, self.hind


@dataclasses.dataclass
class FusedRecords:
    wave_ptr: torch.Tensor
    records: torch.Tensor
    num_records: int

    def nbytes(self) -> int:
        return self.wave_ptr.numel() * 4 + self.records.numel() * 4


RECORD_WORDS = 64


def build_fused_records_torch(blk_offsets: torch.Tensor, hspa_packed: torch.Tensor, hind: torch.Tensor, num_nodes: int,
                              waves: int = FUSED_WAVES, row_blocks: int = FUSED_ROW_BLOCKS) -> FusedRecords:
    assert blk_offsets.dtype == torch.int32 and hind.dtype == torch.int32 and hspa_packed.dtype == torch.uint32
    device = blk_offsets.device
    num_windows = (num_nodes + 15) // 16
    panel_rows = waves * row_blocks * 16
    num_waves = waves * ((num_nodes + panel_rows - 1) // panel_rows)
    bo = blk_offsets.to(torch.int64)
    kb0, kb1 = bo[:-1], bo[1:]
    nblk = kb1 - kb0
    packed = hspa_packed.view(torch.int32).view(-1, 4)
    hind64 = hind
    total_blocks = packed.shape[0]
    zero_first = (packed[kb0.clamp(max=max(total_blocks - 1, 0))] == 0).all(dim=1) if total_blocks else nblk < 0
    nstage = torch.where((nblk == 1) & zero_first, torch.zeros_like(nblk), (nblk + 3) // 4)
    win = torch.repeat_interleave(torch.arange(num_windows, device=device), nstage)
    first_stage = torch.cumsum(nstage, 0) - nstage
    sidx = torch.arange(win.numel(), device=device) - first_stage[win]
    sb = kb0[win] + 4 * sidx
    first_col = hind64[8 * sb].to(torch.int64)
    ncols = int(first_col.max()) + 1 if win.numel() else 1
    order = torch.argsort(((win // row_blocks) * ncols + first_col) * row_blocks + win % row_blocks, stable=True)
    win, sb = win[order], sb[order]
    wave_ptr = torch.zeros(num_waves + 1, dtype=torch.int64, device=device)
    wave_ptr[1:] = torch.cumsum(torch.bincount(win // row_blocks, minlength=num_waves), 0)
    num_records = int(win.numel())
    records = torch.zeros((num_records + 1, RECORD_WORDS), dtype=torch.int32, device=device)
    chunk = 1 << 20
    for lo in range(0, num_records, chunk):
        hi = min(lo + chunk, num_records)
        w_, sb_ = win[lo:hi], sb[lo:hi]
        end = kb1[w_][:, None]
        k = torch.arange(32, device=device)[None, :]
        blk = sb_[:, None] + k // 8
        inwin = blk < end
        blk = torch.where(inwin, blk, kb0[w_][:, None])
        c = k % 8
        words = packed[blk, 2 * (c >> 2)] | packed[blk, 2 * (c >> 2) + 1]
        colmask = ((0x11111111 << (c & 3)) & 0xFFFFFFFF).to(torch.int64)
        used = inwin & (((words.to(torch.int64) & 0xFFFFFFFF) & colmask) != 0)
        safe = hind64[8 * kb0[w_]][:, None]
        records[lo:hi, :32] = torch.where(used, hind64[8 * blk + c], safe)
        t = torch.arange(16, device=device)[None, :]
        blk = sb_[:, None] + t // 4
        inwin = blk < end
        blk = torch.where(inwin, blk, kb0[w_][:, None])
        records[lo:hi, 32:48] = torch.where(inwin, packed[blk, t % 4], torch.zeros((), dtype=torch.int32, device=device))
        records[lo:hi, 48] = (w_ % row_blocks).to(torch.int32)
    return FusedRecords(wave_ptr=wave_ptr.to(torch.int32), records=records.view(torch.uint32), num_records=num_records)


def build_fused_records(blk_offsets: torch.Tensor, hspa_packed: torch.Tensor, hind: torch.Tensor, num_nodes: int) -> FusedRecords:
    assert blk_offsets.is_cuda and hspa_packed.is_cuda and hind.is_cuda
    assert capi.fused_panel_geometry() == (FUSED_WAVES, FUSED_ROW_BLOCKS), "library / package out of step"
    wave_ptr, records, num_records = capi.build_fused_records(blk_offsets, hspa_packed, hind, num_nodes)
    return FusedRecords(wave_ptr=wave_ptr, records=records, num_records=num_records)


def split_shared_columns(indptr: torch.Tensor, indices: torch.Tensor, num_nodes: int, num_cols: int, panel_rows: int,
                         tau: int):
    device = indptr.device
    n, p = num_nodes, panel_rows
    deg = (indptr[1:] - indptr[:-1]).to(torch.int64)
    rows = torch.repeat_interleave(torch.arange(n, device=device, dtype=torch.int64), deg)
    cols = indices.to(torch.int64)
    key = ((rows // p) * num_cols + cols) * p + (rows % p)
    del rows, cols
    key = torch.unique(key, sorted=True)
    pc_all = key // p
    uniq, inverse, counts = torch.unique_consecutive(pc_all, return_inverse=True, return_counts=True)
    shared_u = counts >= tau
    shared_e = shared_u[inverse]
    rk = key[~shared_e]
    r_pc = rk // p
    r_row = (r_pc // num_cols) * p + (rk % p)
    r_key = torch.sort(r_row * num_cols + (r_pc % num_cols)).values
    resid_rows = r_key // num_cols
    resid_indices = (r_key % num_cols).to(torch.int32)
    resid_indptr = torch.zeros(n + 1, dtype=torch.int64, device=device)
    resid_indptr[1:] = torch.cumsum(torch.bincount(resid_rows, minlength=n), 0)
    new_index = torch.cumsum(shared_u.to(torch.int64), 0) - 1
    sk = key[shared_e]
    return (resid_indptr.to(torch.int32), resid_indices, uniq[shared_u], sk % p, new_index[inverse[shared_e]])


MAX_PLAN_COLS = 1 << 22
MAX_PLAN_EDGE_PASSES = 2 * 10 ** 10


def canonical_csr(indptr: torch.Tensor, indices: torch.Tensor, num_nodes: int, num_cols: int):
    deg = (indptr[1:] - indptr[:-1]).to(torch.int64)
    rows = torch.repeat_interleave(torch.arange(num_nodes, device=indptr.device, dtype=torch.int64), deg)
    key = torch.unique(rows * num_cols + indices.to(torch.int64), sorted=True)
    rows = key // num_cols
    out_indptr = torch.zeros(num_nodes + 1, dtype=torch.int64, device=indptr.device)
    out_indptr[1:] = torch.cumsum(torch.bincount(rows, minlength=num_nodes), 0)
    return out_indptr.to(torch.int32), (key - rows * num_cols).to(torch.int32)


def empty_plan(num_nodes, waves, row_blocks, tau, device, num_edges):
    np_ = (num_nodes + waves * row_blocks * 16 - 1) // (waves * row_blocks * 16)
    return PanelPlan(panel_ptr=torch.zeros(np_ + 1, dtype=torch.int32, device=device),
                     panel_cols=torch.zeros(2 * KSTEP, dtype=torch.int32, device=device),
                     panel_bits=torch.zeros(waves * 64, dtype=torch.int32, device=device).view(torch.uint32),
                     panel_order=None, num_nodes=num_nodes, waves=waves, row_blocks=row_blocks, tau=tau, num_ksteps=0,
                     num_shared_edges=0, num_resid_edges=num_edges)


KSTEP_COST_IN_STAGES = 6.6
KSTEP_COST_X10 = 66


def balance_xcd_ranges(two: "TwoLevelHandle") -> None:
    plan = two.plan
    if plan.num_ksteps == 0 or plan.num_panels < 2 * 8:
        return
    cost_x10 = max(1, KSTEP_COST_X10 * plan.panel_rows // 512)
    if plan.panel_ptr.is_cuda:
        xcd_ptr, two.window_xcd_ptr = capi.xcd_ranges_of_panels(plan.panel_ptr, two.blk_offsets, two.num_nodes, plan.panel_rows,
                                                                cost_x10)
    else:
        xcd_ptr, two.window_xcd_ptr = xcd_ranges_of_panels_torch(plan.panel_ptr, two.blk_offsets, two.num_nodes,
                                                                 plan.panel_rows, cost_x10)
    longest_range, longest_panel = torch.stack([(xcd_ptr[1:] - xcd_ptr[:-1]).max(),
                                                (plan.panel_ptr[1:] - plan.panel_ptr[:-1]).max()]).tolist()
    plan.xcd_ptr = xcd_ptr
    plan.max_panels_per_xcd = int(longest_range)
    plan.panel_order = longest_first_order(plan.panel_ptr, xcd_ptr=xcd_ptr)
    cap = default_part_cap(plan.num_ksteps)
    if PANEL_PART_FACTOR > 0 and longest_panel > cap:
        plan.parts = panel_parts(plan.panel_ptr, cap, xcd_ptr)


def xcd_ranges_of_panels_torch(panel_ptr: torch.Tensor, resid_blk_offsets: torch.Tensor, num_nodes: int, panel_rows: int,
                               kstep_cost_x10: int):
    from .schedule import split_equal_work

    dev = panel_ptr.device
    num_panels = panel_ptr.numel() - 1
    windows_per_panel = panel_rows // 16
    num_windows = (num_nodes + 15) // 16
    nst = ((resid_blk_offsets[1:num_windows + 1] - resid_blk_offsets[:num_windows]).to(torch.int64) + 3) // 4
    pad = num_panels * windows_per_panel - num_windows
    stages = torch.cat([nst, torch.zeros(pad, dtype=torch.int64, device=dev)]).view(num_panels, windows_per_panel).sum(1)
    tenths = (panel_ptr[1:] - panel_ptr[:-1]).to(torch.int64) * kstep_cost_x10
    q, r = tenths // 10, tenths % 10
    q = q + ((r > 5) | ((r == 5) & (q % 2 == 1))).to(torch.int64)
    xcd_ptr = split_equal_work(q + stages)
    return xcd_ptr, (xcd_ptr.to(torch.int64) * windows_per_panel).clamp(max=num_windows).to(torch.int32)


PANEL_PART_FACTOR = 1.0
NUM_CUS = 256


def default_part_cap(num_ksteps: int) -> int:
    return max(32, int(PANEL_PART_FACTOR * num_ksteps / NUM_CUS))


def panel_parts(panel_ptr: torch.Tensor, cap: int, panel_xcd_ptr: torch.Tensor = None) -> PanelParts:
    if not panel_ptr.is_cuda:
        return panel_parts_torch(panel_ptr, cap, panel_xcd_ptr)
    assert cap >= 1
    parts, part_xcd_ptr, cuts, head = capi.build_panel_parts(panel_ptr, cap, panel_xcd_ptr)
    return PanelParts(parts, cuts, part_xcd_ptr, head[3], head[0], head[1], head[2], cap)


def panel_parts_torch(panel_ptr: torch.Tensor, cap: int, panel_xcd_ptr: torch.Tensor = None) -> PanelParts:
    assert cap >= 1
    dev = panel_ptr.device
    num_panels = panel_ptr.numel() - 1
    nks = (panel_ptr[1:] - panel_ptr[:-1]).to(torch.int64)
    k = torch.clamp((nks + cap - 1) // cap, min=1)
    p = torch.repeat_interleave(torch.arange(num_panels, dtype=torch.int64, device=dev), k)
    first = torch.cumsum(k, 0) - k
    j = torch.arange(p.numel(), dtype=torch.int64, device=dev) - first[p]
    base, rem = nks[p] // k[p], nks[p] % k[p]
    length = base + (j < rem).to(torch.int64)
    begin = j * base + torch.minimum(j, rem)
    cut = k > 1
    k_cut = torch.where(cut, k, torch.zeros_like(k))
    slot_first = torch.cumsum(k_cut, 0) - k_cut
    slot = torch.where(cut[p], slot_first[p] + j, torch.full_like(p, -1))
    if panel_xcd_ptr is not None:
        xcd = torch.searchsorted(panel_xcd_ptr.to(torch.int64)[1:8].contiguous(), p, right=True)
    else:
        xcd = p // max(1, (num_panels + 7) // 8)
    top = int(length.max()) if p.numel() else 0
    order = torch.argsort(xcd * (top + 1) + (top - length), stable=True)
    parts = torch.stack([p[order], begin[order], length[order], slot[order]], dim=1).to(torch.int32).contiguous()
    counts = torch.bincount(xcd, minlength=8)
    xcd_ptr = torch.zeros(9, dtype=torch.int64, device=dev)
    xcd_ptr[1:] = torch.cumsum(counts, 0)
    cp = torch.nonzero(cut).flatten()
    cuts = torch.stack([cp, slot_first[cp], k[cp], torch.zeros_like(cp)], dim=1).to(torch.int32).contiguous()
    return PanelParts(parts, cuts, xcd_ptr.to(torch.int32), int(counts.max()) if p.numel() else 0, int(p.numel()),
                      int(cp.numel()), int(k_cut.sum()), cap)


def longest_first_order(panel_ptr: torch.Tensor, group: int = 1, xcd_ptr: torch.Tensor = None) -> torch.Tensor:
    num_panels = panel_ptr.numel() - 1
    if num_panels <= 0:
        return torch.zeros(0, dtype=torch.int32, device=panel_ptr.device)
    if panel_ptr.is_cuda:
        order = torch.empty(num_panels, dtype=torch.int32, device=panel_ptr.device)
        capi.launch_panel_order(panel_ptr, num_panels, order, torch.cuda.current_stream().cuda_stream, group, xcd_ptr)
        return order
    nks = (panel_ptr[1:] - panel_ptr[:-1]).to(torch.int64)
    per_xcd = (num_panels + 7) // 8
    idx = torch.arange(num_panels, device=panel_ptr.device)
    if xcd_ptr is not None:
        assert group == 1
        xcd = torch.searchsorted(xcd_ptr.to(torch.int64)[1:8].contiguous(), idx, right=True)
        top = int(nks.max())
        return torch.argsort(xcd * (top + 1) + (top - nks), stable=True).to(torch.int32)
    xcd = idx // per_xcd
    gid = xcd * (per_xcd // group + 2) + (idx - xcd * per_xcd) // group
    gsum = torch.zeros(int(gid.max()) + 1, dtype=torch.int64, device=panel_ptr.device).index_add_(0, gid, nks)
    top = int(gsum.max())
    key = ((xcd * (top + 1) + (top - gsum[gid])) * (per_xcd + 1) + (idx - xcd * per_xcd) // group) * (group + 1) + (
        idx - xcd * per_xcd) % group
    return torch.argsort(key, stable=True).to(torch.int32)


def build_panel_plan(indptr: torch.Tensor, indices: torch.Tensor, num_nodes: int, num_cols: int = None,
                     waves: int = DEFAULT_WAVES, row_blocks: int = DEFAULT_ROW_BLOCKS, tau: int = DEFAULT_TAU,
                     min_share: float = 0.0):
    assert indptr.is_cuda and indices.is_cuda and indptr.dtype == torch.int32 and indices.dtype == torch.int32
    assert indptr.is_contiguous() and indices.is_contiguous() and indptr.numel() == num_nodes + 1
    assert waves in (4, 8) and row_blocks in (2, 4) and 1 <= tau <= 65535
    device = indptr.device
    num_cols = num_nodes if num_cols is None else int(num_cols)
    if (num_cols > MAX_PLAN_COLS or num_nodes == 0
            or ((num_cols + (1 << 16) - 1) >> 16) * indices.numel() > MAX_PLAN_EDGE_PASSES):
        return indptr, indices, empty_plan(num_nodes, waves, row_blocks, tau, device, indices.numel())
    stream = torch.cuda.current_stream().cuda_stream
    panel_rows = waves * row_blocks * 16
    num_panels = (num_nodes + panel_rows - 1) // panel_rows
    for attempt in range(2):
        workspace = torch.empty(capi.panel_plan_workspace_bytes(num_nodes, waves, row_blocks), dtype=torch.uint8,
                                device=device)
        panel_ptr = torch.empty(num_panels + 1, dtype=torch.int32, device=device)
        resid_indptr = torch.empty(num_nodes + 1, dtype=torch.int32, device=device)
        status = torch.empty(1, dtype=torch.int32, device=device)
        rc = capi.launch_panel_plan_count(indptr, indices, num_nodes, num_cols, waves, row_blocks, tau, workspace, panel_ptr,
                                          resid_indptr, status, stream)
        capi.check(rc, "voltrix_launch_panel_plan_count")
        total_ksteps, num_resid, bad = torch.cat([panel_ptr[-1:], resid_indptr[-1:], status]).tolist()
        if bad == 0:
            break
        if attempt == 1 or int(indices.min()) < 0 or int(indices.max()) >= num_cols:
            return indptr, indices, empty_plan(num_nodes, waves, row_blocks, tau, device, indices.numel())
        indptr, indices = canonical_csr(indptr, indices, num_nodes, num_cols)
    if total_ksteps == 0 or indices.numel() - num_resid < min_share * max(1, indices.numel()):
        plan = empty_plan(num_nodes, waves, row_blocks, tau, device, indices.numel())
        plan.num_shared_edges = indices.numel() - num_resid
        return indptr, indices, plan
    resid_indices = torch.empty(num_resid, dtype=torch.int32, device=device)
    panel_cols = torch.empty(KSTEP * (total_ksteps + 2), dtype=torch.int32, device=device)
    panel_bits = torch.empty((total_ksteps + 1) * waves * 64, dtype=torch.int32, device=device).view(torch.uint32)
    capi.launch_panel_plan_fill(indptr, indices, num_nodes, num_cols, waves, row_blocks, tau, workspace, panel_ptr,
                                resid_indptr, total_ksteps, resid_indices, panel_cols, panel_bits, stream)
    plan = PanelPlan(panel_ptr=panel_ptr, panel_cols=panel_cols, panel_bits=panel_bits,
                     panel_order=longest_first_order(panel_ptr) if total_ksteps > 0 else None,
                     num_nodes=num_nodes, waves=waves, row_blocks=row_blocks, tau=tau, num_ksteps=total_ksteps,
                     num_shared_edges=indices.numel() - num_resid, num_resid_edges=num_resid)
    return resid_indptr, resid_indices, plan


def build_panel_plan_torch(indptr: torch.Tensor, indices: torch.Tensor, num_nodes: int, num_cols: int = None,
                           waves: int = DEFAULT_WAVES, row_blocks: int = DEFAULT_ROW_BLOCKS, tau: int = DEFAULT_TAU):
    assert indptr.device == indices.device and indptr.dtype == torch.int32 and indices.dtype == torch.int32
    assert waves in (4, 8) and row_blocks in (2, 4) and tau >= 1
    device = indptr.device
    num_cols = num_nodes if num_cols is None else int(num_cols)
    p = waves * row_blocks * 16
    num_panels = (num_nodes + p - 1) // p
    resid_indptr, resid_indices, pc, rp, inv = split_shared_columns(indptr, indices, num_nodes, num_cols, p, tau)

    su_panel = pc // num_cols
    su_col = pc % num_cols
    cnt = torch.bincount(su_panel, minlength=num_panels)
    nks = (cnt + KSTEP - 1) // KSTEP
    panel_ptr = torch.zeros(num_panels + 1, dtype=torch.int64, device=device)
    panel_ptr[1:] = torch.cumsum(nks, 0)
    total_ksteps = int(panel_ptr[-1].item())
    assert total_ksteps < 2 ** 26, "k-step offsets are int32 (x 32 columns)"
    col_start = torch.cumsum(cnt, 0) - cnt
    rank = torch.arange(pc.numel(), device=device, dtype=torch.int64) - col_start[su_panel]
    slot = (panel_ptr[su_panel] + rank // KSTEP) * KSTEP + rank % KSTEP

    panel_of_kstep = torch.repeat_interleave(torch.arange(num_panels, device=device), nks)
    first_col = torch.zeros(num_panels, dtype=torch.int64, device=device)
    has = cnt > 0
    first_col[has] = su_col[col_start[has]]
    panel_cols = torch.zeros(KSTEP * (total_ksteps + 2), dtype=torch.int64, device=device)
    panel_cols[:KSTEP * total_ksteps] = first_col[panel_of_kstep].repeat_interleave(KSTEP)
    panel_cols[slot] = su_col

    e_slot = slot[inv]
    k = e_slot % KSTEP
    v = rp // (16 * row_blocks)
    j = (rp % (16 * row_blocks)) // 16
    word = (e_slot // KSTEP) * (waves * 64) + v * 64 + (k // 8) * 16 + (rp % 16)
    bits = torch.zeros((total_ksteps + 1) * waves * 64, dtype=torch.int64, device=device)
    bits.index_add_(0, word, torch.ones_like(word) << (16 * (k % 2) + 4 * j + (k % 8) // 2))
    panel_bits = ((bits + 2 ** 31) % 2 ** 32 - 2 ** 31).to(torch.int32).view(torch.uint32)

    plan = PanelPlan(panel_ptr=panel_ptr.to(torch.int32), panel_cols=panel_cols.to(torch.int32), panel_bits=panel_bits,
                     panel_order=None, num_nodes=num_nodes, waves=waves, row_blocks=row_blocks, tau=tau,
                     num_ksteps=total_ksteps, num_shared_edges=int(rp.numel()),
                     num_resid_edges=int(resid_indices.numel()))
    return resid_indptr, resid_indices, plan


KSTEPS_PIPELINED = 17


def default_panel_tile(embedding_dim: int, waves: int, row_blocks: int = DEFAULT_ROW_BLOCKS):
    if embedding_dim <= 32:
        return (32, 6, 2)
    if embedding_dim <= 64:
        return (64, 6, 2)
    if waves == 8:
        return (128, 3, 1) if row_blocks == 4 else (128, 4, KSTEPS_PIPELINED)
    return (128, 4, 1)


PANEL_DOMINATED_RATIO = 2.0
PANEL_DOMINATED_ROW_BLOCKS = 2


def panel_dominated(plan: "PanelPlan") -> bool:
    resid_stages = max(1.0, plan.num_resid_edges / 32.0)
    return plan.num_ksteps * KSTEP_COST_IN_STAGES >= PANEL_DOMINATED_RATIO * resid_stages


_SIDE_STREAMS = {}


def side_stream(device) -> "torch.cuda.Stream":
    key = device.index if device.index is not None else torch.cuda.current_device()
    if key not in _SIDE_STREAMS:
        _SIDE_STREAMS[key] = torch.cuda.Stream(device=device)
    return _SIDE_STREAMS[key]


def run_two_level(plan: PanelPlan, operand: torch.Tensor, output: torch.Tensor, run_window, out_scale=None,
                  tile=None, concurrent: bool = True) -> None:
    def finish(pending):
        if pending is not None:
            pending.run()

    if plan.num_ksteps == 0:
        finish(run_window(False))
        return
    if not concurrent:
        finish(run_window(False))
        launch_panel(plan, operand, output, accumulate=1, out_scale=out_scale, tile=tile)
        return
    from .utils import timed_launch

    main = torch.cuda.current_stream()
    side = side_stream(operand.device)
    with timed_launch("zero_fill", main):
        output.zero_()
    fork = torch.cuda.Event()
    fork.record(main)
    side.wait_event(fork)
    pending_panel = launch_panel(plan, operand, output, accumulate=2, out_scale=out_scale, tile=tile,
                                 stream=side.cuda_stream, defer_combine=True)
    join = torch.cuda.Event()
    join.record(side)
    pending = run_window(True)
    main.wait_event(join)
    finish(pending)
    finish(pending_panel)


class PendingPanelCombine:

    def __init__(self, plan, partials, output, num_feats, accumulate):
        self.plan, self.partials, self.output, self.num_feats, self.accumulate = plan, partials, output, num_feats, accumulate

    def run(self, raw_stream: int = None):
        from .utils import timed_launch

        current = torch.cuda.current_stream()
        with timed_launch("combine_panel_partials", current) if raw_stream is None else contextlib.nullcontext():
            rc = capi.launch_combine_panel_partials(self.plan.parts, self.partials.data_ptr(), self.output.data_ptr(),
                                                    self.plan.num_nodes, self.num_feats, self.plan.panel_rows,
                                                    self.accumulate, current.cuda_stream if raw_stream is None else raw_stream)
        capi.check(rc, "voltrix_launch_combine_panel_partials")
        self.partials = None


def launch_panel(plan: PanelPlan, feat: torch.Tensor, output: torch.Tensor, accumulate, out_scale=None,
                 tile=None, stream=None, slab_policy: int = None, defer_combine: bool = False):
    assert feat.is_cuda and feat.is_contiguous() and feat.dtype in (torch.float16, torch.bfloat16)
    assert output.is_cuda and output.is_contiguous() and output.dtype == torch.float32
    f = feat.shape[1]
    assert output.shape == (plan.num_nodes, f)
    tile = tile or default_panel_tile(f, plan.waves, plan.row_blocks)
    assert tile is not None, f"no panel tile for F={f} with {plan.waves} waves"
    stream = torch.cuda.current_stream().cuda_stream if stream is None else stream
    if slab_policy is None:
        from .jit_kernels import spmm as _spmm_wrapper

        slab_policy = _spmm_wrapper.SLAB_POLICY
    parts = plan.parts
    partials = None
    if parts is not None and parts.num_slots > 0:
        partials = torch.empty(parts.num_slots * plan.panel_rows * f, dtype=torch.float32, device=feat.device)
    rc = capi.launch_spmm_panel(plan, feat.data_ptr(), output.data_ptr(), f, int(accumulate),
                                feat.dtype == torch.bfloat16, tile, out_scale.data_ptr() if out_scale is not None else 0,
                                stream, input_rows=feat.shape[0], slab_policy=slab_policy,
                                partials_ptr=partials.data_ptr() if partials is not None else 0)
    capi.check(rc, "voltrix_launch_spmm_panel")
    if partials is None:
        return None
    pending = PendingPanelCombine(plan, partials, output, f, 1 if int(accumulate) else 0)
    if defer_combine:
        return pending
    pending.run(None if stream == torch.cuda.current_stream().cuda_stream else stream)
    return None


def default_fused_tile(embedding_dim: int):
    if embedding_dim <= 32:
        return (32, 4)
    if embedding_dim <= 64:
        return (64, 4)
    return (128, 3)


FUSED_PACE_BLOCKS = 0


def fused_enabled() -> bool:
    return os.getenv("VOLTRIX_FUSED", "0") in ("1", "on")


def launch_fused(plan: PanelPlan, fused: FusedRecords, feat: torch.Tensor, output: torch.Tensor, out_scale=None,
                 tile=None, stream=None, pace_blocks: int = None) -> None:
    assert feat.is_cuda and feat.is_contiguous() and feat.dtype in (torch.float16, torch.bfloat16)
    assert output.is_cuda and output.is_contiguous() and output.dtype == torch.float32
    assert plan.waves == DEFAULT_WAVES and plan.row_blocks == DEFAULT_ROW_BLOCKS, "the fused kernel owns 8 x 4 x 16-row panels"
    f = feat.shape[1]
    assert output.shape == (plan.num_nodes, f)
    tile = tile or default_fused_tile(f)
    stream = torch.cuda.current_stream().cuda_stream if stream is None else stream
    pace_blocks = FUSED_PACE_BLOCKS if pace_blocks is None else pace_blocks
    rc = capi.launch_spmm_fused(plan, fused, feat.data_ptr(), output.data_ptr(), f, feat.dtype == torch.bfloat16, tile,
                                out_scale.data_ptr() if out_scale is not None else 0, stream, pace_blocks)
    capi.check(rc, "voltrix_launch_spmm_fused")


def min_shared_fraction() -> float:
    default = "0.38" if hybrid_mode() == "auto" else "0.2"
    return float(os.getenv("VOLTRIX_HYBRID_MIN_SHARE", default))


_MODE_OVERRIDE = contextvars.ContextVar("voltrix_hybrid_mode", default=None)


@contextlib.contextmanager
def mode_override(value: str):
    token = _MODE_OVERRIDE.set(value)
    try:
        yield
    finally:
        _MODE_OVERRIDE.reset(token)


def hybrid_mode() -> str:
    v = _MODE_OVERRIDE.get()
    v = os.getenv("VOLTRIX_HYBRID", "auto") if v is None else v
    if v in ("0", "", "off"):
        return "off"
    if v in ("1", "on"):
        return "on"
    return "tune" if v == "tune" else "auto"


AUTO_MIN_EDGES = 1 << 22
AUTO_MIN_MEAN_DEGREE = 64
AUTO_MIN_ROWS = 110_000


def handle_bytes(tensors) -> int:
    return int(sum(t.numel() * t.element_size() for t in tensors if isinstance(t, torch.Tensor)))


def two_level_bytes(two: "TwoLevelHandle") -> int:
    plan = two.plan
    total = handle_bytes((two.blk_offsets, two.hspa_packed, two.hind, plan.panel_ptr, plan.panel_cols, plan.panel_bits,
                          plan.panel_order))
    if two.fused is not None:
        total += two.fused.nbytes()
    return total
```

### voltrix-spmm_amd/voltrix/include/voltrix/panel_plan.hpp

```cpp
#pragma once

#include <hip/hip_runtime.h>

#include <cstdint>

#include "voltrix/csr_preprocess.hpp"
#include "voltrix/traits.hpp"

namespace voltrix {

constexpr int kPlanThreads = 1024;
constexpr int kPlanWaves = kPlanThreads / kWave;
constexpr int kPlanRange = 1 << 16;
constexpr int kPlanFlagWords = kPlanRange / 32;
constexpr int kPlanMaxPanelRows = 512;
constexpr int kPlanMaxRanges = 64;
constexpr int kPlanBatch = 8;
constexpr int kPlanVecBatch = 8;
constexpr int kPlanRowBatch = 8;

struct PlanLds {
  unsigned counters[kPlanRange / 2];
  unsigned flags[kPlanFlagWords];
  int prefix[kPlanFlagWords];
  int rpos[kPlanMaxPanelRows];
  int wsum[kPlanWaves];
  int total;
  int first_col;
};

__device__ __forceinline__ void plan_count_range(PlanLds& s, const int* __restrict__ indices, const long long lo,
                                                 const long long hi, const int c0) {
  for (int i = threadIdx.x; i < kPlanRange / 2; i += kPlanThreads) s.counters[i] = 0u;
  __syncthreads();
  auto bump = [&](const int c) {
    if ((unsigned)c < (unsigned)kPlanRange) atomicAdd(&s.counters[c >> 1], 1u << (16 * (c & 1)));
  };
  const long long head_end = lo + ((4 - (int)(((uintptr_t)(indices + lo) & 15) >> 2)) & 3);
  const long long vec_lo = head_end < hi ? head_end : hi;
  const long long vec_hi = vec_lo + ((hi - vec_lo) & ~3ll);
  for (long long e = lo + threadIdx.x; e < vec_lo; e += kPlanThreads) bump(indices[e] - c0);
  for (long long e = vec_hi + threadIdx.x; e < hi; e += kPlanThreads) bump(indices[e] - c0);
  const int4* const vec = reinterpret_cast<const int4*>(indices + vec_lo);
  const long long nvec = (vec_hi - vec_lo) >> 2;
  for (long long base = threadIdx.x; base < nvec; base += (long long)kPlanThreads * kPlanVecBatch) {
    int4 c[kPlanVecBatch];
#pragma unroll
    for (int b = 0; b < kPlanVecBatch; ++b) {
      const long long i = base + (long long)b * kPlanThreads;
      c[b] = i < nvec ? vec[i] : make_int4(-1, -1, -1, -1);
    }
#pragma unroll
    for (int b = 0; b < kPlanVecBatch; ++b) {
      if (base + (long long)b * kPlanThreads < nvec) {
        bump(c[b].x - c0);
        bump(c[b].y - c0);
        bump(c[b].z - c0);
        bump(c[b].w - c0);
      }
    }
  }
  __syncthreads();
}

__device__ __forceinline__ unsigned plan_counter(const PlanLds& s, const int c) {
  return (s.counters[c >> 1] >> (16 * (c & 1))) & 0xFFFFu;
}

__device__ __forceinline__ int plan_block_sum(PlanLds& s, int v) {
#pragma unroll
  for (int off = kWave / 2; off > 0; off >>= 1) v += __shfl_xor(v, off, kWave);
  __syncthreads();
  if ((threadIdx.x & (kWave - 1)) == 0) s.wsum[threadIdx.x / kWave] = v;
  __syncthreads();
  int t = 0;
#pragma unroll
  for (int k = 0; k < kPlanWaves; ++k) t += s.wsum[k];
  return t;
}

static __global__ __launch_bounds__(kPlanThreads) void panel_plan_count_kernel(
    const int* __restrict__ indptr, const int* __restrict__ indices, const int num_nodes, const int num_cols,
    const int panel_rows, const unsigned tau, const int nranges, int* __restrict__ shared_count ,
    int* __restrict__ resid_count , int* __restrict__ status) {
  extern __shared__ __attribute__((aligned(16))) char smem[];
  PlanLds& s = *reinterpret_cast<PlanLds*>(smem);
  const int p = blockIdx.x / nranges, rho = blockIdx.x % nranges;
  const int r0 = p * panel_rows;
  const int r1 = r0 + panel_rows < num_nodes ? r0 + panel_rows : num_nodes;
  const int c0 = rho * kPlanRange;
  const long long lo = indptr[r0], hi = indptr[r1];
  plan_count_range(s, indices, lo, hi, c0);

  int mine = 0;
  for (int i = threadIdx.x; i < kPlanRange / 2; i += kPlanThreads) {
    const unsigned w = s.counters[i];
    mine += ((w & 0xFFFFu) >= tau) + ((w >> 16) >= tau);
  }
  const int total = plan_block_sum(s, mine);
  if (threadIdx.x == 0 && total) atomicAdd(&shared_count[p], total);

  const int lane = threadIdx.x & (kWave - 1), wave = threadIdx.x / kWave;
  static_assert(kPlanMaxPanelRows <= kPlanWaves * kWave, "one lane per row of the wave");
  const int my_row = r0 + wave + kPlanWaves * lane;
  const int my_a = my_row < r1 ? indptr[my_row] : 0, my_b = my_row < r1 ? indptr[my_row + 1] : 0;
  for (int row = r0 + wave, ri = 0; row < r1; row += kPlanWaves, ++ri) {
    const long long a = __shfl(my_a, ri, kWave), b = __shfl(my_b, ri, kWave);
    int cnt = 0, bad = 0, prev_last = -1;
    for (long long e0 = a; e0 < b; e0 += kWave * kPlanRowBatch) {
      int cs[kPlanRowBatch];
#pragma unroll
      for (int k = 0; k < kPlanRowBatch; ++k) {
        const long long e = e0 + k * kWave + lane;
        cs[k] = e < b ? indices[e] : 0x7FFFFFFF;
      }
#pragma unroll
      for (int k = 0; k < kPlanRowBatch; ++k) {
        if (e0 + k * kWave >= b) break;
        const long long e = e0 + k * kWave + lane;
        const int c = cs[k];
        if (rho == 0) {
          int prev = __shfl_up(c, 1, kWave);
          if (lane == 0) prev = prev_last;
          bad += (e < b && (c <= prev || c < 0 || c >= num_cols)) ? 1 : 0;
          prev_last = __shfl(c, kWave - 1, kWave);
        }
        const int cr = c - c0;
        const bool resid = e < b && (unsigned)cr < (unsigned)kPlanRange && plan_counter(s, cr) < tau;
        cnt += __popcll(__ballot(resid));
      }
    }
    if (lane == 0 && cnt) atomicAdd(&resid_count[row], cnt);
    if (rho == 0) {
#pragma unroll
      for (int off = kWave / 2; off > 0; off >>= 1) bad += __shfl_xor(bad, off, kWave);
      if (lane == 0 && bad) atomicAdd(status, bad);
    }
  }
}

static __global__ __launch_bounds__(256) void panel_ptr_kernel(const int* __restrict__ shared_count, const int num_panels,
                                                               int* __restrict__ panel_ptr) {
  __shared__ int wsum[4];
  __shared__ int carry_s;
  if (threadIdx.x == 0) {
    carry_s = 0;
    panel_ptr[0] = 0;
  }
  __syncthreads();
  for (int base = 0; base < num_panels; base += 256) {
    const int i = base + threadIdx.x;
    const int v = i < num_panels ? (shared_count[i] + kStageK - 1) / kStageK : 0;
    const int inc = wave_inclusive_scan(v);
    if ((threadIdx.x & (kWave - 1)) == kWave - 1) wsum[threadIdx.x / kWave] = inc;
    __syncthreads();
    int woff = 0;
    for (int k = 0; k < (int)(threadIdx.x / kWave); ++k) woff += wsum[k];
    const int carry = carry_s;
    if (i < num_panels) panel_ptr[i + 1] = carry + woff + inc;
    __syncthreads();
    if (threadIdx.x == 255) carry_s = carry + woff + inc;
    __syncthreads();
  }
}

static __global__ __launch_bounds__(kPlanThreads) void panel_plan_fill_kernel(
    const int* __restrict__ indptr, const int* __restrict__ indices, const int num_nodes, const int panel_rows,
    const int waves, const int row_blocks, const unsigned tau, const int nranges, const int* __restrict__ panel_ptr,
    const int* __restrict__ shared_count, const int* __restrict__ resid_indptr, int* __restrict__ resid_indices,
    int* __restrict__ panel_cols, unsigned* __restrict__ panel_bits ) {
  extern __shared__ __attribute__((aligned(16))) char smem[];
  PlanLds& s = *reinterpret_cast<PlanLds*>(smem);
  const int p = blockIdx.x;
  const int r0 = p * panel_rows;
  const int r1 = r0 + panel_rows < num_nodes ? r0 + panel_rows : num_nodes;
  const long long lo = indptr[r0], hi = indptr[r1];
  const long long ks0 = panel_ptr[p];
  const int lane = threadIdx.x & (kWave - 1), wave = threadIdx.x / kWave;
  for (int i = threadIdx.x; i < r1 - r0; i += kPlanThreads) s.rpos[i] = resid_indptr[r0 + i];
  if (threadIdx.x == 0) s.first_col = 0;
  int rank_base = 0;
  const int my_row = r0 + wave + kPlanWaves * lane;
  const int my_a = my_row < r1 ? indptr[my_row] : 0, my_b = my_row < r1 ? indptr[my_row + 1] : 0;

  for (int rho = 0; rho < nranges; ++rho) {
    const int c0 = rho * kPlanRange;
    plan_count_range(s, indices, lo, hi, c0);

    constexpr int WPT = kPlanFlagWords / kPlanThreads;
    unsigned fl[WPT];
    int pc = 0;
#pragma unroll
    for (int k = 0; k < WPT; ++k) {
      const int w = threadIdx.x * WPT + k;
      unsigned f = 0u;
#pragma unroll
      for (int i = 0; i < 16; ++i) {
        const unsigned cw = s.counters[w * 16 + i];
        f |= ((cw & 0xFFFFu) >= tau ? 1u : 0u) << (2 * i);
        f |= ((cw >> 16) >= tau ? 1u : 0u) << (2 * i + 1);
      }
      fl[k] = f;
      pc += __popc(f);
    }
    const int inc = wave_inclusive_scan(pc);
    if (lane == kWave - 1) s.wsum[wave] = inc;
    __syncthreads();
    int woff = 0, range_total = 0;
#pragma unroll
    for (int k = 0; k < kPlanWaves; ++k) {
      woff += k < wave ? s.wsum[k] : 0;
      range_total += s.wsum[k];
    }
    int run = woff + inc - pc;
#pragma unroll
    for (int k = 0; k < WPT; ++k) {
      const int w = threadIdx.x * WPT + k;
      s.flags[w] = fl[k];
      s.prefix[w] = run;
      unsigned f = fl[k];
      int rank = rank_base + run;
      while (f) {
        const int i = __ffs(f) - 1;
        f &= f - 1u;
        const int col = c0 + 32 * w + i;
        panel_cols[ks0 * kStageK + rank] = col;
        if (rank == 0) s.first_col = col;
        ++rank;
      }
      run += __popc(fl[k]);
    }
    __syncthreads();

    for (int row = r0 + wave, ri = 0; row < r1; row += kPlanWaves, ++ri) {
      const int rp = row - r0;
      const int v = rp / (16 * row_blocks), j = (rp % (16 * row_blocks)) / 16, r16 = rp % 16;
      const long long a = __shfl(my_a, ri, kWave), b = __shfl(my_b, ri, kWave);
      int pos = s.rpos[rp];
      for (long long e0 = a; e0 < b; e0 += kWave * kPlanRowBatch) {
        int cs[kPlanRowBatch];
#pragma unroll
        for (int q = 0; q < kPlanRowBatch; ++q) {
          const long long e = e0 + q * kWave + lane;
          cs[q] = e < b ? indices[e] : 0x7FFFFFFF;
        }
#pragma unroll
        for (int q = 0; q < kPlanRowBatch; ++q) {
          if (e0 + q * kWave >= b) break;
          const long long e = e0 + q * kWave + lane;
          const int c = cs[q];
          const int cr = c - c0;
          const bool in_range = e < b && (unsigned)cr < (unsigned)kPlanRange;
          const bool shared = in_range && ((s.flags[cr >> 5] >> (cr & 31)) & 1u);
          const bool resid = in_range && !shared;
          const unsigned long long rmask = __ballot(resid);
          if (resid) resid_indices[pos + __popcll(rmask & ((1ull << lane) - 1ull))] = c;
          pos += __popcll(rmask);
          if (shared) {
            const int rank = rank_base + s.prefix[cr >> 5] + __popc(s.flags[cr >> 5] & ((1u << (cr & 31)) - 1u));
            const long long ks = ks0 + (rank >> 5);
            const int k = rank & 31;
            atomicOr(&panel_bits[(ks * waves + v) * kWave + (k >> 3) * 16 + r16],
                     1u << (16 * (k & 1) + 4 * j + ((k & 7) >> 1)));
          }
        }
      }
      if (lane == 0) s.rpos[rp] = pos;
    }
    rank_base += range_total;
    __syncthreads();
  }

  const int cnt = shared_count[p];
  const int padded = (cnt + kStageK - 1) / kStageK * kStageK;
  if ((int)threadIdx.x < padded - cnt) panel_cols[ks0 * kStageK + cnt + threadIdx.x] = s.first_col;
}

static __global__ __launch_bounds__(256) void panel_order_kernel(const int* __restrict__ panel_ptr, const int num_panels,
                                                                 const int per_xcd, const int group,
                                                                 const int* __restrict__ xcd_ptr,
                                                                 int* __restrict__ order_out) {
  for (int p = blockIdx.x * 256 + threadIdx.x; p < num_panels; p += gridDim.x * 256) {
    int lo = (p / per_xcd) * per_xcd;
    int hi = lo + per_xcd < num_panels ? lo + per_xcd : num_panels;
    if (xcd_ptr != nullptr) {
      int x = 0;
      for (int i = 1; i < kNumXcd; ++i) x += p >= xcd_ptr[i] ? 1 : 0;
      lo = xcd_ptr[x];
      hi = xcd_ptr[x + 1];
    }
    const int my_group = (p - lo) / group;
    const int g0 = lo + my_group * group, g1 = g0 + group < hi ? g0 + group : hi;
    const int mine = panel_ptr[g1] - panel_ptr[g0];
    int before = 0;
    for (int q0 = lo, gi = 0; q0 < hi; q0 += group, ++gi) {
      const int q1 = q0 + group < hi ? q0 + group : hi;
      const int other = panel_ptr[q1] - panel_ptr[q0];
      if (other > mine || (other == mine && gi < my_group)) before += q1 - q0;
    }
    order_out[lo + before + (p - g0)] = p;
  }
}

inline int panel_order(const int* panel_ptr, int num_panels, int group, int* order_out, hipStream_t stream,
                       const int* xcd_ptr = nullptr) {
  if (num_panels < 0 || group < 1) return kErrBadShape;
  if (num_panels == 0) return kOk;
  const int per_xcd = (num_panels + kNumXcd - 1) / kNumXcd;
  hipLaunchKernelGGL(panel_order_kernel, dim3((num_panels + 255) / 256), dim3(256), 0, stream, panel_ptr, num_panels,
                     per_xcd, group, xcd_ptr, order_out);
  return hipGetLastError() == hipSuccess ? kOk : kErrLaunch;
}

struct PlanWorkspace {
  int* shared_count;
  int* resid_count;
  int* chunk_sums;
  long long bytes;
};

inline PlanWorkspace plan_workspace(void* base, int num_nodes, int panel_rows) {
  const int np = (num_nodes + panel_rows - 1) / panel_rows;
  PlanWorkspace ws;
  char* p = static_cast<char*>(base);
  ws.shared_count = reinterpret_cast<int*>(p);
  p += align16(4ll * (np + 1));
  ws.resid_count = reinterpret_cast<int*>(p);
  p += align16(4ll * (num_nodes + 1));
  ws.chunk_sums = reinterpret_cast<int*>(p);
  p += align16(4ll * ((num_nodes + kScanChunk - 1) / kScanChunk + 1));
  ws.bytes = p - static_cast<char*>(base);
  return ws;
}

inline int plan_check(int num_nodes, int num_cols, long long num_edges, int waves, int row_blocks, int tau) {
  if (num_nodes < 0 || num_edges < 0 || num_edges > 0x7FFFFFFFll || num_cols < 0) return kErrBadShape;
  if (!(waves == 4 || waves == 8) || !(row_blocks == 2 || row_blocks == 4) || tau < 1 || tau > 65535) return kErrBadShape;
  if ((num_cols + kPlanRange - 1) / kPlanRange > kPlanMaxRanges) return kErrBadConfig;
  return kOk;
}

inline int panel_plan_count(const int* indptr, const int* indices, int num_nodes, int num_cols, long long num_edges,
                            int waves, int row_blocks, int tau, void* workspace, int* panel_ptr, int* resid_indptr,
                            int* status, hipStream_t stream) {
  if (int rc = plan_check(num_nodes, num_cols, num_edges, waves, row_blocks, tau)) return rc;
  if (((uintptr_t)workspace & 15) || status == nullptr) return kErrBadShape;
  const int panel_rows = waves * row_blocks * 16;
  const int np = (num_nodes + panel_rows - 1) / panel_rows;
  if (hipMemsetAsync(status, 0, sizeof(int), stream) != hipSuccess) return kErrLaunch;
  if (hipMemsetAsync(panel_ptr, 0, sizeof(int), stream) != hipSuccess) return kErrLaunch;
  if (hipMemsetAsync(resid_indptr, 0, sizeof(int), stream) != hipSuccess) return kErrLaunch;
  if (num_nodes == 0) return kOk;
  const PlanWorkspace ws = plan_workspace(workspace, num_nodes, panel_rows);
  if (hipMemsetAsync(workspace, 0, (size_t)ws.bytes, stream) != hipSuccess) return kErrLaunch;
  const int nranges = num_cols > 0 ? (num_cols + kPlanRange - 1) / kPlanRange : 1;
  if ((long long)np * nranges > 0x7FFFFFFFll) return kErrBadShape;
  if (int rc = bm_set_lds(panel_plan_count_kernel, sizeof(PlanLds))) return rc;
  hipLaunchKernelGGL(panel_plan_count_kernel, dim3(np * nranges), dim3(kPlanThreads), sizeof(PlanLds), stream, indptr,
                     indices, num_nodes, num_cols, panel_rows, (unsigned)tau, nranges, ws.shared_count, ws.resid_count,
                     status);
  hipLaunchKernelGGL(panel_ptr_kernel, dim3(1), dim3(256), 0, stream, ws.shared_count, np, panel_ptr);
  const int nchunks = (num_nodes + kScanChunk - 1) / kScanChunk;
  hipLaunchKernelGGL(scan_chunk_sums_kernel, dim3(nchunks), dim3(256), 0, stream, ws.resid_count, num_nodes,
                     ws.chunk_sums);
  hipLaunchKernelGGL(scan_chunk_offsets_kernel, dim3(1), dim3(256), 0, stream, ws.chunk_sums, nchunks);
  hipLaunchKernelGGL(scan_apply_kernel, dim3(nchunks), dim3(256), 0, stream, ws.resid_count, num_nodes, ws.chunk_sums,
                     resid_indptr);
  return hipGetLastError() == hipSuccess ? kOk : kErrLaunch;
}

inline int panel_plan_fill(const int* indptr, const int* indices, int num_nodes, int num_cols, long long num_edges,
                           int waves, int row_blocks, int tau, void* workspace, const int* panel_ptr,
                           const int* resid_indptr, long long total_ksteps, int* resid_indices, int* panel_cols,
                           uint32_t* panel_bits, hipStream_t stream) {
  if (int rc = plan_check(num_nodes, num_cols, num_edges, waves, row_blocks, tau)) return rc;
  if (((uintptr_t)workspace & 15) || total_ksteps < 0) return kErrBadShape;
  const int panel_rows = waves * row_blocks * 16;
  const int np = (num_nodes + panel_rows - 1) / panel_rows;
  if (hipMemsetAsync(panel_bits, 0, (size_t)(total_ksteps + 1) * waves * kWave * 4, stream) != hipSuccess) return kErrLaunch;
  if (hipMemsetAsync(panel_cols + total_ksteps * kStageK, 0, 2 * kStageK * 4, stream) != hipSuccess) return kErrLaunch;
  if (num_nodes == 0) return kOk;
  const PlanWorkspace ws = plan_workspace(workspace, num_nodes, panel_rows);
  const int nranges = num_cols > 0 ? (num_cols + kPlanRange - 1) / kPlanRange : 1;
  if (int rc = bm_set_lds(panel_plan_fill_kernel, sizeof(PlanLds))) return rc;
  hipLaunchKernelGGL(panel_plan_fill_kernel, dim3(np), dim3(kPlanThreads), sizeof(PlanLds), stream, indptr, indices,
                     num_nodes, panel_rows, waves, row_blocks, (unsigned)tau, nranges, panel_ptr, ws.shared_count,
                     resid_indptr, resid_indices, panel_cols, panel_bits);
  return hipGetLastError() == hipSuccess ? kOk : kErrLaunch;
}

inline long long panel_plan_workspace_bytes(int num_nodes, int waves, int row_blocks) {
  if (num_nodes < 0 || waves <= 0 || row_blocks <= 0) return 0;
  return plan_workspace(nullptr, num_nodes, waves * row_blocks * 16).bytes;
}

}
```

### voltrix-spmm_amd/voltrix/include/voltrix/spmm_panel_kernels.hpp

```cpp
#pragma once

#include <hip/hip_runtime.h>

#include <cstdint>
#include <type_traits>

#include "voltrix/spmm_kernels.hpp"

#ifndef VOLTRIX_PANEL_DIAG
#define VOLTRIX_PANEL_DIAG 0
#endif
namespace voltrix {


template <int FS_, int DEPTH_, int WAVES_, int RB_, int KS_ = 1, bool BF16_ = false, bool PIPE_ = false>
struct PanelTile {
  static constexpr int FS = FS_, DEPTH = DEPTH_, WAVES = WAVES_, RB = RB_, KS = KS_;
  static constexpr bool BF16 = BF16_, PIPE = PIPE_;
  static_assert(!PIPE || (KS == 1 && FS >= 32), "pipelined loop: one k-step per ring slot");
  static_assert(FS == 32 || FS == 64 || FS == 128, "feature slab");
  static_assert(RB >= 1 && RB <= 4, "a lane's adjacency word holds four row blocks");
  static_assert(KS == 1 || KS == 2, "one index DMA covers 64 columns");
  static_assert(DEPTH >= 3 && DEPTH <= 8, "ring depth");
  static constexpr int PANEL_ROWS = WAVES * RB * 16;
  static constexpr int THREADS = WAVES * kWave;
  static constexpr int ROW_BYTES = FS * 2;
  static constexpr int KSTEP_BYTES = kStageK * ROW_BYTES;
  static constexpr int STAGE_BYTES = KS * KSTEP_BYTES;
  static constexpr int NDMA = STAGE_BYTES / 1024;
  static_assert(NDMA % WAVES == 0 || WAVES % NDMA == 0, "row DMAs per step vs waves");
  static constexpr int DPW = NDMA >= WAVES ? NDMA / WAVES : 1;
  static constexpr int ROWS_PER_DMA = 1024 / ROW_BYTES;
  static constexpr int LANES_PER_ROW = ROW_BYTES / 16;
  static constexpr int SLOTS = FS / 16;
  static constexpr int BITS_BYTES = KS * WAVES * 256;
  static constexpr int META_BYTES = BITS_BYTES + 256;
  static constexpr int META_SLOTS = PIPE ? 2 * DEPTH : 2 * DEPTH - 1;
  static constexpr int NBITS_DMA = BITS_BYTES / 1024;
  static_assert(BITS_BYTES % 1024 == 0 && NBITS_DMA + 1 <= WAVES, "metadata DMA roles");
  static constexpr int VM_PER_STEP = DPW + 1;
  static constexpr int VM_PER_STEP_PLAIN = DPW;
  static constexpr int DATA_LDS = DEPTH * STAGE_BYTES;
  static constexpr int BLOCK_LDS = DATA_LDS + META_SLOTS * META_BYTES;
  static_assert(BLOCK_LDS <= 160 * 1024, "LDS per CU");
  static_assert(VM_PER_STEP * (DEPTH - 2) <= 63, "vmcnt is a 6-bit counter on gfx9");
};

__device__ __forceinline__ half8_t adjacency_to_half8_x2(unsigned w, int p0) {
  uint4_t r;
#pragma unroll
  for (int i = 0; i < 4; ++i) {
    const int p = p0 + i;
    r[i] = (p <= 14 ? (w << (14 - p)) : (w >> (p - 14))) & 0x40004000u;
  }
  return __builtin_bit_cast(half8_t, r);
}

template <class T>
struct PanelArgs {
  using in_t = typename std::conditional<T::BF16, bfloat16_bits, _Float16>::type;
  const int* panel_ptr;
  const int* panel_cols;
  const uint32_t* panel_bits;
  const int* panel_order;
  const int* xcd_ptr;
  const int* parts;
  float* partials;
  const in_t* input;
  float* output;
  const float* out_scale;
  int num_nodes;
  int num_panels;
  int panels_per_xcd;
  int F;
  int meta_nt;
  int slab_first;
  int accumulate;
};

template <class T>
static __global__ __launch_bounds__(T::THREADS) void spmm_panel_kernel(const PanelArgs<T> a) {
  constexpr int FS = T::FS, D = T::DEPTH, MS = T::META_SLOTS, KS = T::KS, RB = T::RB;
  constexpr int ROW_BYTES = T::ROW_BYTES, STAGE_BYTES = T::STAGE_BYTES, DPW = T::DPW;
  constexpr int RPD = T::ROWS_PER_DMA, LPR = T::LANES_PER_ROW, SLOTS = T::SLOTS;

  extern __shared__ __attribute__((aligned(16))) char smem[];
  const int wave = __builtin_amdgcn_readfirstlane((int)(threadIdx.x / kWave));

  const int xcd = blockIdx.x % kNumXcd;
  const int pos = (a.xcd_ptr ? a.xcd_ptr[xcd] : xcd * a.panels_per_xcd) + (int)(blockIdx.x / kNumXcd);
  const int pos_end = a.xcd_ptr ? a.xcd_ptr[xcd + 1]
                                : ((xcd + 1) * a.panels_per_xcd < a.num_panels ? (xcd + 1) * a.panels_per_xcd : a.num_panels);
  if (pos >= pos_end) return;
  int panel, ks0, nks, slot = -1;
  if (a.parts) {
    const int4_t part = *reinterpret_cast<const int4_t*>(a.parts + 4 * (long long)pos);
    panel = part[0];
    ks0 = a.panel_ptr[panel] + part[1];
    nks = part[2];
    slot = part[3];
  } else {
    panel = a.panel_order ? a.panel_order[pos] : pos;
    ks0 = a.panel_ptr[panel];
    nks = a.panel_ptr[panel + 1] - ks0;
  }
  const int fs0 = (a.slab_first + blockIdx.y) * FS;
  const int F = a.F;
  const int lane = threadIdx.x & (kWave - 1);

  const int ngroups = (nks + KS - 1) / KS;
  if (ngroups == 0 && a.accumulate && slot < 0) return;

  float4_t acc[RB][SLOTS];
#pragma unroll
  for (int j = 0; j < RB; ++j)
#pragma unroll
    for (int s = 0; s < SLOTS; ++s) acc[j][s] = float4_t{0.f, 0.f, 0.f, 0.f};

  const unsigned data0 = (unsigned)(uintptr_t)(lds_ptr)smem;
  const unsigned meta0 = data0 + T::DATA_LDS;
  const bool meta_wave = wave <= T::NBITS_DMA;

  if (ngroups > 0) {
    const unsigned row_bytes = (unsigned)F * 2u;
    const int dma0 = (wave * DPW) % T::NDMA;
    const char* cbase[DPW];
    unsigned hr_off[DPW];
#pragma unroll
    for (int d = 0; d < DPW; ++d) {
      const int r = (dma0 + d) * RPD + lane / LPR;
      const int c = lane % LPR;
      int col = fs0 + (((c >> 1) ^ slot_swizzle<SLOTS>(r & 31)) * 16) + (c & 1) * 8;
      col = col < F ? col : fs0;
      unsigned long long cb = (unsigned long long)((const char*)a.input + (long long)col * 2);
      asm volatile("" : "+v"(cb));
      cbase[d] = (const char*)cb;
      hr_off[d] = T::BITS_BYTES + 4 * r;
    }
    const int* const cols_base = a.panel_cols + (long long)ks0 * kStageK;
    auto issue_meta = [&](int s, int ms) {
      const int sc = s < ngroups ? s : ngroups - 1;
      const unsigned dst = meta0 + (unsigned)ms * T::META_BYTES;
      int ml = lane;
      asm volatile("" : "+v"(ml));
      if (wave < T::NBITS_DMA) {
        const char* src = (const char*)(a.panel_bits + (long long)(ks0 + sc * KS) * (T::WAVES * kWave)) + wave * 1024 + ml * 16;
        if (a.meta_nt) dma_b128_nt(src, dst + wave * 1024); else dma_b128(src, dst + wave * 1024);
      } else if (wave == T::NBITS_DMA) {
        const int* src = cols_base + (long long)sc * (KS * kStageK) + ml;
        if (a.meta_nt) dma_b32_nt(src, dst + T::BITS_BYTES); else dma_b32(src, dst + T::BITS_BYTES);
      }
    };
    auto issue_rows = [&](int ms, int ds) {
      const unsigned mslot = meta0 + (unsigned)ms * T::META_BYTES;
      const unsigned dst = data0 + (unsigned)ds * STAGE_BYTES + (unsigned)dma0 * 1024u;
      unsigned hrow[DPW];
#pragma unroll
      for (int d = 0; d < DPW; ++d) hrow[d] = lds_read_b32(mslot + hr_off[d]);
      wait_lgkmcnt0();
#pragma unroll
      for (int d = 0; d < DPW; ++d)
        if (!(VOLTRIX_PANEL_DIAG & 2)) dma_b128(cbase[d] + (unsigned long long)hrow[d] * row_bytes, dst + d * 1024);
    };

    constexpr int PRO = T::PIPE ? D : D - 1;
#pragma unroll
    for (int s = 0; s < PRO; ++s) issue_meta(s, s % MS);
    wait_vmcnt<0>();
    __builtin_amdgcn_s_barrier();
#pragma unroll
    for (int s = 0; s < PRO; ++s) {
      issue_rows(s % MS, s % D);
      issue_meta(s + PRO, (s + PRO) % MS);
    }

    const int g = lane >> 4;
    const int q = (lane >> 2) & 3, p = lane & 3;
    const int trow = 8 * g + q;
    const int tr_z = slot_swizzle<SLOTS>(trow);
    unsigned rd_off = trow * ROW_BYTES + 8 * p + (tr_z << 5);
    int tr_delta[3];
#pragma unroll
    for (int b = 0; b < 3; ++b) {
      tr_delta[b] = ((tr_z >> b) & 1) ? -(32 << b) : (32 << b);
      asm volatile("" : "+v"(tr_delta[b]));
    }
    asm volatile("" : "+v"(rd_off));

    if constexpr (T::PIPE) {
      constexpr int HS = SLOTS / 2 > 0 ? SLOTS / 2 : 1;
      constexpr int NH = SLOTS / HS;
      static_assert(NH == 2, "two halves");
      uint2_t b0lo[HS], b0hi[HS], b1lo[HS], b1hi[HS];
      if (data0 & 255u) __builtin_trap();
      auto half_addr = [&](const unsigned dt, const int s) -> unsigned { return dt ^ ((unsigned)s << 5); };
      auto read_half = [&](const int h, const unsigned dt, uint2_t (&lo)[HS], uint2_t (&hi)[HS]) {
#pragma unroll
        for (int s = 0; s < HS; ++s) {
          const unsigned ad = half_addr(dt, h * HS + s);
          if (VOLTRIX_PANEL_DIAG & 8) {
            lo[s] = uint2_t{ad, 1u};
            hi[s] = uint2_t{ad, 2u};
            continue;
          }
          lo[s] = lds_read_tr16_b64<0>(ad);
          hi[s] = lds_read_tr16_b64<4 * ROW_BYTES>(ad);
        }
      };
      auto mfma_half = [&](const int h, unsigned aw, const uint2_t (&lo)[HS], const uint2_t (&hi)[HS]) {
        if constexpr (RB == 4) asm volatile("" : "+v"(aw));
#pragma unroll
        for (int j = 0; j < RB; ++j) {
          const half8_t afrag = adjacency_to_half8_x2(aw, 4 * j);
#pragma unroll
          for (int s = 0; s < HS; ++s) {
            const uint4_t bq = {lo[s][0], lo[s][1], hi[s][0], hi[s][1]};
            if (VOLTRIX_PANEL_DIAG & 1) {
              asm volatile("" ::"v"(afrag), "v"(bq));
              continue;
            }
            if constexpr (T::BF16)
              acc[j][h * HS + s] = __builtin_amdgcn_mfma_f32_16x16x32_bf16(__builtin_bit_cast(bf16x8_t, afrag),
                                                                             __builtin_bit_cast(bf16x8_t, bq), acc[j][h * HS + s], 0, 0, 0);
            else
              acc[j][h * HS + s] = __builtin_amdgcn_mfma_f32_16x16x32_f16(afrag, __builtin_bit_cast(half8_t, bq),
                                                                            acc[j][h * HS + s], 0, 0, 0);
          }
        }
      };
      auto issue_rows_of = [&](const unsigned (&hrow)[DPW], const int ds) {
        const unsigned dst = data0 + (unsigned)ds * STAGE_BYTES + (unsigned)dma0 * 1024u;
#pragma unroll
        for (int d = 0; d < DPW; ++d)
          if (!(VOLTRIX_PANEL_DIAG & 2)) dma_b128(cbase[d] + (unsigned long long)hrow[d] * row_bytes, dst + d * 1024);
      };
      const int total_steps = ngroups > D ? ngroups : D;
      auto wait_group = [&](const int young, auto per_step) {
        constexpr int VM = decltype(per_step)::value;
        if (young >= D - 2 && D >= 2) {
          wait_vmcnt<VM * (D - 2)>();
        } else {
          switch (young) {
            case 0: wait_vmcnt<0>(); break;
            case 1: wait_vmcnt<VM * 1>(); break;
            case 2: wait_vmcnt<VM * 2>(); break;
            case 3: wait_vmcnt<VM * 3>(); break;
            case 4: wait_vmcnt<VM * 4>(); break;
            default: wait_vmcnt<VM * 5>(); break;
          }
        }
      };
      if (meta_wave) wait_vmcnt<T::VM_PER_STEP * (D - 1)>();
      else wait_vmcnt<T::VM_PER_STEP_PLAIN * (D - 1)>();
      if (!(VOLTRIX_PANEL_DIAG & 4)) __builtin_amdgcn_s_barrier();
      __builtin_amdgcn_sched_barrier(0);
      unsigned aw_cur = lds_read_b32(meta0 + 256 * wave + 4 * lane);
      read_half(0, data0 + rd_off, b0lo, b0hi);
      wait_lgkmcnt0();
      int ds_t = 0;
      int ds_n = 1 % D;
      int ms_t = 0;
      int ms_n = 1 % MS;
      int ms_d = D % MS;
      for (int t = 0; t < ngroups; ++t) {
        const unsigned dt = data0 + (unsigned)ds_t * STAGE_BYTES + rd_off;
        const bool refill = t + D < ngroups;
        read_half(1, dt, b1lo, b1hi);
        unsigned hrow[DPW];
#pragma unroll
        for (int d = 0; d < DPW; ++d) {
          unsigned ad;
          asm volatile("v_lshrrev_b32 %0, %2, %1\n\tv_lshl_add_u32 %0, %0, 2, %3"
                       : "=&v"(ad)
                       : "v"(lane), "n"(LPR == 16 ? 4 : (LPR == 8 ? 3 : 2)),
                         "s"(meta0 + (unsigned)ms_d * T::META_BYTES + T::BITS_BYTES + 4u * (unsigned)((dma0 + d) * RPD)));
          hrow[d] = lds_read_b32(ad);
        }
        __builtin_amdgcn_sched_barrier(0);
        mfma_half(0, aw_cur, b0lo, b0hi);
        __builtin_amdgcn_sched_barrier(0);
        wait_lgkmcnt0();
#pragma unroll
        for (int d = 0; d < DPW; ++d) asm volatile("" ::"v"(hrow[d]));
        unsigned aw_next = aw_cur;
        if (t + 1 < ngroups) {
          const int young = total_steps - 2 - t;
          if (meta_wave) wait_group(young, std::integral_constant<int, T::VM_PER_STEP>{});
          else wait_group(young, std::integral_constant<int, T::VM_PER_STEP_PLAIN>{});
          if (!(VOLTRIX_PANEL_DIAG & 4))
            __builtin_amdgcn_s_barrier();
          __builtin_amdgcn_sched_barrier(0);
          if (refill) {
            issue_rows_of(hrow, ds_t);
            if (!(VOLTRIX_PANEL_DIAG & 16)) issue_meta(t + 2 * D, ms_t);
          }
          aw_next = lds_read_b32(meta0 + (unsigned)ms_n * T::META_BYTES + 256 * wave + 4 * lane);
          read_half(0, data0 + (unsigned)ds_n * STAGE_BYTES + rd_off, b0lo, b0hi);
          __builtin_amdgcn_sched_barrier(0);
        }
        mfma_half(1, aw_cur, b1lo, b1hi);
        __builtin_amdgcn_sched_barrier(0);
        wait_lgkmcnt0();
        aw_cur = aw_next;
        ds_t = ds_n;
        ds_n = ds_n + 1 == D ? 0 : ds_n + 1;
        ms_t = ms_n;
        ms_n = ms_n + 1 == MS ? 0 : ms_n + 1;
        ms_d = ms_d + 1 == MS ? 0 : ms_d + 1;
      }
    } else {
    int ds_t = 0, ms_t = 0;
    int ds_r = (D - 1) % D, ms_r = (D - 1) % MS;
    int ms_m = (2 * D - 2) % MS;
    for (int t = 0; t < ngroups; ++t) {
      const int young = ngroups - 1 - t;
      auto wait_steps = [&](auto per_step) {
        constexpr int VM = decltype(per_step)::value;
        if (young >= D - 2) {
          wait_vmcnt<VM*(D - 2)>();
        } else {
          switch (young) {
            case 0: wait_vmcnt<0>(); break;
            case 1: wait_vmcnt<VM * 1>(); break;
            case 2: wait_vmcnt<VM * 2>(); break;
            case 3: wait_vmcnt<VM * 3>(); break;
            case 4: wait_vmcnt<VM * 4>(); break;
            default: wait_vmcnt<VM * 5>(); break;
          }
        }
      };
      if (meta_wave) wait_steps(std::integral_constant<int, T::VM_PER_STEP>{});
      else wait_steps(std::integral_constant<int, T::VM_PER_STEP_PLAIN>{});
      if (!(VOLTRIX_PANEL_DIAG & 4))
        __builtin_amdgcn_s_barrier();
      __builtin_amdgcn_sched_barrier(0);

      if (t + D - 1 < ngroups) {
        issue_rows(ms_r, ds_r);
        if (!(VOLTRIX_PANEL_DIAG & 16)) issue_meta(t + 2 * D - 2, ms_m);
      }

      const unsigned mt = meta0 + (unsigned)ms_t * T::META_BYTES;
      const unsigned dt = data0 + (unsigned)ds_t * STAGE_BYTES + rd_off;
      ds_t = ds_t + 1 == D ? 0 : ds_t + 1;
      ds_r = ds_r + 1 == D ? 0 : ds_r + 1;
      ms_t = ms_t + 1 == MS ? 0 : ms_t + 1;
      ms_r = ms_r + 1 == MS ? 0 : ms_r + 1;
      ms_m = ms_m + 1 == MS ? 0 : ms_m + 1;
#pragma unroll
      for (int k = 0; k < KS; ++k) {
        if (t * KS + k < nks) {
          const unsigned aw = lds_read_b32(mt + 256 * (k * T::WAVES + wave) + 4 * lane);
          unsigned taddr[SLOTS];
          taddr[0] = dt + k * T::KSTEP_BYTES;
#pragma unroll
          for (int b = 0; (1 << b) < SLOTS; ++b)
#pragma unroll
            for (int s = (1 << b); s < (2 << b) && s < SLOTS; ++s) taddr[s] = taddr[s - (1 << b)] + tr_delta[b];
          uint2_t blo[SLOTS], bhi[SLOTS];
#pragma unroll
          for (int s = 0; s < SLOTS; ++s) {
            if (VOLTRIX_PANEL_DIAG & 8) {
              blo[s] = uint2_t{taddr[s], 1u};
              bhi[s] = uint2_t{taddr[s], 2u};
              continue;
            }
            blo[s] = lds_read_tr16_b64<0>(taddr[s]);
            bhi[s] = lds_read_tr16_b64<4 * ROW_BYTES>(taddr[s]);
          }
          wait_lgkmcnt0();
#pragma unroll
          for (int j = 0; j < RB; ++j) {
            const half8_t afrag = adjacency_to_half8_x2(aw, 4 * j);
#pragma unroll
            for (int s = 0; s < SLOTS; ++s) {
              const uint4_t bq = {blo[s][0], blo[s][1], bhi[s][0], bhi[s][1]};
              if (VOLTRIX_PANEL_DIAG & 1) {
                asm volatile("" ::"v"(afrag), "v"(bq));
                continue;
              }
              if constexpr (T::BF16)
                acc[j][s] = __builtin_amdgcn_mfma_f32_16x16x32_bf16(__builtin_bit_cast(bf16x8_t, afrag),
                                                                    __builtin_bit_cast(bf16x8_t, bq), acc[j][s], 0, 0, 0);
              else
                acc[j][s] = __builtin_amdgcn_mfma_f32_16x16x32_f16(afrag, __builtin_bit_cast(half8_t, bq), acc[j][s], 0,
                                                                   0, 0);
            }
          }
        }
      }
    }
    }
    wait_vmcnt<0>();
  }

  const float oscale = kAScaleInv * (a.out_scale ? *a.out_scale : 1.0f);
  const int ocol0 = fs0 + (lane & 15);
  if (slot >= 0) {
    float* const tile = a.partials + (long long)slot * T::PANEL_ROWS * F;
    const int trow0 = wave * (RB * 16) + 4 * (lane >> 4);
#pragma unroll
    for (int j = 0; j < RB; ++j)
#pragma unroll
      for (int s = 0; s < SLOTS; ++s)
#pragma unroll
        for (int i = 0; i < 4; ++i) {
          const int col = ocol0 + 16 * s;
          if (col < F) tile[(long long)(trow0 + 16 * j + i) * F + col] = acc[j][s][i] * oscale;
        }
    return;
  }
  const int prow0 = panel * T::PANEL_ROWS + wave * (RB * 16) + 4 * (lane >> 4);
  if (a.accumulate == 2) {
#pragma unroll
    for (int j = 0; j < RB; ++j) {
#pragma unroll
      for (int s = 0; s < SLOTS; ++s) {
#pragma unroll
        for (int i = 0; i < 4; ++i) {
          const int row = prow0 + 16 * j + i, col = ocol0 + 16 * s;
          if (col < F && row < a.num_nodes) unsafeAtomicAdd(a.output + ((long long)row * F + col), acc[j][s][i] * oscale);
        }
      }
    }
    return;
  }
#pragma unroll
  for (int j = 0; j < RB; ++j) {
    float prev[SLOTS][4];
#pragma unroll
    for (int s = 0; s < SLOTS; ++s) {
#pragma unroll
      for (int i = 0; i < 4; ++i) {
        const int row = prow0 + 16 * j + i, col = ocol0 + 16 * s;
        prev[s][i] = (a.accumulate && col < F && row < a.num_nodes) ? a.output[(long long)row * F + col] : 0.0f;
      }
    }
#pragma unroll
    for (int s = 0; s < SLOTS; ++s) {
#pragma unroll
      for (int i = 0; i < 4; ++i) {
        const int row = prow0 + 16 * j + i, col = ocol0 + 16 * s;
        if (col < F && row < a.num_nodes) a.output[(long long)row * F + col] = prev[s][i] + acc[j][s][i] * oscale;
      }
    }
  }
}

static __global__ __launch_bounds__(256) void combine_panel_partials_kernel(const int* __restrict__ cuts,
                                                                            const float* __restrict__ partials,
                                                                            float* __restrict__ output, int num_nodes, int F,
                                                                            int panel_rows, int accumulate) {
  const int4_t cut = *reinterpret_cast<const int4_t*>(cuts + 4 * (long long)blockIdx.x);
  const int panel = cut[0], first = cut[1], pieces = cut[2];
  const int f4 = F / 4;
  const long long tile = (long long)panel_rows * F;
  for (int e = threadIdx.x; e < 16 * f4; e += 256) {
    const int r = blockIdx.y * 16 + e / f4, c = 4 * (e % f4);
    const long long row = (long long)panel * panel_rows + r;
    if (row >= num_nodes) continue;
    const float* src = partials + (long long)first * tile + (long long)r * F + c;
    float4_t sum = *reinterpret_cast<const float4_t*>(src);
    for (int j = 1; j < pieces; ++j) sum += *reinterpret_cast<const float4_t*>(src + j * tile);
    float4_t* dst = reinterpret_cast<float4_t*>(output + row * F + c);
    *dst = accumulate ? *dst + sum : sum;
  }
}

inline int launch_combine_panel_partials(const int* cuts, int num_cuts, const float* partials, float* output, int num_nodes,
                                         int embedding_dim, int panel_rows, int accumulate, hipStream_t stream) {
  if (num_cuts < 0 || num_nodes < 0 || embedding_dim < 0 || panel_rows < 16 || panel_rows % 16 != 0) return kErrBadShape;
  if (num_cuts == 0 || num_nodes == 0 || embedding_dim == 0) return kOk;
  if (embedding_dim % 4 != 0 || cuts == nullptr || partials == nullptr || output == nullptr) return kErrBadShape;
  hipLaunchKernelGGL(combine_panel_partials_kernel, dim3((unsigned)num_cuts, (unsigned)(panel_rows / 16)), dim3(256), 0, stream,
                     cuts, partials, output, num_nodes, embedding_dim, panel_rows, accumulate);
  return hipGetLastError() == hipSuccess ? kOk : kErrLaunch;
}

template <class T>
inline int launch_spmm_panel(const int* panel_ptr, const int* panel_cols, const uint32_t* panel_bits,
                             const int* panel_order, int num_nodes, int embedding_dim, const void* input, float* output,
                             int accumulate, const float* out_scale, hipStream_t stream, int slab_first = 0,
                             int slab_count = 0 ,
                             long long input_rows = 0 ,
                             int slab_policy = kSlabAuto, const int* xcd_ptr = nullptr ,
                             int max_panels_per_xcd = 0 ,
                             const int* parts = nullptr , int num_parts = 0,
                             float* partials = nullptr) {
  if (num_nodes < 0 || embedding_dim < 0 || accumulate < 0 || accumulate > 2) return kErrBadShape;
  if (parts != nullptr && num_parts < 1) return kErrBadShape;
  if (num_nodes == 0 || embedding_dim == 0) return kOk;
  if (embedding_dim % 8 != 0 || ((uintptr_t)input & 15)) return kErrBadShape;
  PanelArgs<T> a;
  a.panel_ptr = panel_ptr;
  a.panel_cols = panel_cols;
  a.panel_bits = panel_bits;
  a.panel_order = panel_order;
  a.input = static_cast<const typename PanelArgs<T>::in_t*>(input);
  a.output = output;
  a.out_scale = out_scale;
  a.num_nodes = num_nodes;
  a.num_panels = (num_nodes + T::PANEL_ROWS - 1) / T::PANEL_ROWS;
  a.parts = parts;
  a.partials = partials;
  if (parts != nullptr) a.num_panels = num_parts;
  a.panels_per_xcd = (a.num_panels + kNumXcd - 1) / kNumXcd;
  a.xcd_ptr = nullptr;
  if (xcd_ptr != nullptr) {
    if (max_panels_per_xcd < 1 || max_panels_per_xcd > a.num_panels) return kErrBadShape;
    a.xcd_ptr = xcd_ptr;
    a.panels_per_xcd = max_panels_per_xcd;
  }
  a.F = embedding_dim;
  a.accumulate = accumulate;
  const int total_slabs = (embedding_dim + T::FS - 1) / T::FS;
  if (slab_first < 0 || slab_count < 0 || slab_first + slab_count > total_slabs) return kErrBadShape;
  if (const int group = slab_count == 0 ? slab_launch_group(total_slabs, T::ROW_BYTES,
                                                            input_rows > 0 ? input_rows : (long long)num_nodes, slab_policy)
                                        : 0) {
    for (int s = 0; s < total_slabs; s += group) {
      const int rc = launch_spmm_panel<T>(panel_ptr, panel_cols, panel_bits, panel_order, num_nodes, embedding_dim, input,
                                          output, accumulate, out_scale, stream, s,
                                          total_slabs - s < group ? total_slabs - s : group, input_rows, slab_policy, xcd_ptr,
                                          max_panels_per_xcd, parts, num_parts, partials);
      if (rc != kOk) return rc;
    }
    return kOk;
  }
  const int slabs = slab_count > 0 ? slab_count : total_slabs;
  a.slab_first = slab_count > 0 ? slab_first : 0;
  a.meta_nt = total_slabs == 1;
  const int lds_rc = ensure_dynamic_lds(reinterpret_cast<const void*>(&spmm_panel_kernel<T>), T::BLOCK_LDS);
  if (lds_rc != kOk) return lds_rc;
  hipLaunchKernelGGL(spmm_panel_kernel<T>, dim3((unsigned)(a.panels_per_xcd * kNumXcd), (unsigned)slabs),
                     dim3(T::THREADS), T::BLOCK_LDS, stream, a);
  return hipGetLastError() == hipSuccess ? kOk : kErrLaunch;
}

}
```

### voltrix-spmm_amd/voltrix/sidecar.py

```python
from __future__ import annotations

import dataclasses
import threading
import warnings
import weakref
from typing import Optional

import torch

_LOCK = threading.RLock()
_ENTRIES = {}
_SLIM = set()
_WARNED = [False]


def _key(t: torch.Tensor):
    st = t.untyped_storage()
    return (t.device.type, t.device.index, st.data_ptr(), t.storage_offset(), t.numel()), st


def register(hspa_packed: torch.Tensor, two) -> None:
    key, storage = _key(hspa_packed)
    with _LOCK:
        fresh = key not in _ENTRIES
        _ENTRIES[key] = two
    if fresh:
        weakref.finalize(storage, _drop, key)


def _drop(key) -> None:
    with _LOCK:
        _ENTRIES.pop(key, None)
        _SLIM.discard(key)
        _CSR.pop(key, None)


_CSR = {}


class CsrSideCar:
    __slots__ = ("indptr", "indices", "num_rows", "num_cols", "choice")

    def __init__(self, indptr, indices, num_rows, num_cols):
        self.indptr, self.indices, self.num_rows, self.num_cols, self.choice = indptr, indices, num_rows, num_cols, {}


def register_csr(hspa_packed: torch.Tensor, csr: "CsrSideCar") -> None:
    key, storage = _key(hspa_packed)
    with _LOCK:
        fresh = key not in _ENTRIES and key not in _CSR
        _CSR[key] = csr
    if fresh:
        weakref.finalize(storage, _drop, key)


def lookup_both(hspa_packed: torch.Tensor):
    key, _ = _key(hspa_packed)
    with _LOCK:
        if key in _ENTRIES:
            return True, _ENTRIES[key], _CSR.get(key)
        return False, None, _CSR.get(key)


def lookup_csr(hspa_packed: torch.Tensor):
    key, _ = _key(hspa_packed)
    with _LOCK:
        return _CSR.get(key)


def lookup(hspa_packed: torch.Tensor):
    key, _ = _key(hspa_packed)
    with _LOCK:
        if key in _ENTRIES:
            return True, _ENTRIES[key]
    return False, None


def copy_side_car(src_hspa_packed: torch.Tensor, dst_hspa_packed: torch.Tensor) -> bool:
    known, two = lookup(src_hspa_packed)
    if known:
        assert two is None or two.hspa_packed.device == dst_hspa_packed.device, "the side-car lives on another device"
        register(dst_hspa_packed, two)
    return known


def warn_if_unknown(hspa_packed: torch.Tensor, num_nodes: int, num_edges: int, min_edges: int, min_rows: int,
                    min_mean_degree: float) -> None:
    if _WARNED[0] or num_edges < min_edges or num_nodes < min_rows or num_edges < min_mean_degree * max(1, num_nodes):
        return
    _WARNED[0] = True
    warnings.warn(
        "voltrix.spmm: this handle's hspa_packed did not come from csr_preprocess in this process (a clone, a .to(), a "
        "reloaded file?), so the two-level side-car, if one was built, is not attached to it and the product runs in the "
        "window format.  Use voltrix.copy_side_car(original_hspa_packed, copy) after copying a handle, or "
        "voltrix.save_handle / voltrix.load_handle to move one between processes.", stacklevel=3)


def slim_handle(handle):
    blk_offsets, hspa_packed, hind = handle
    known, two = lookup(hspa_packed)
    if not known or two is None:
        return handle
    stub_packed = torch.zeros(4, dtype=hspa_packed.dtype, device=hspa_packed.device)
    stub_hind = torch.zeros(4, dtype=hind.dtype, device=hind.device)
    if getattr(hspa_packed, "hash_tag", None) is not None:
        stub_packed.hash_tag = hspa_packed.hash_tag
    register(stub_packed, two)
    with _LOCK:
        _SLIM.add(_key(stub_packed)[0])
    return blk_offsets, stub_packed, stub_hind


def is_slim(hspa_packed: torch.Tensor) -> bool:
    key, _ = _key(hspa_packed)
    with _LOCK:
        return key in _SLIM



def save_handle(path: str, handle, num_nodes: int) -> None:
    blk_offsets, hspa_packed, hind = handle
    known, two = lookup(hspa_packed)
    blob = {"format": "voltrix-handle-1", "num_nodes": int(num_nodes),
            "handle": [t.detach().cpu() for t in (blk_offsets, hspa_packed.view(torch.int32), hind)],
            "hash_tag": getattr(hspa_packed, "hash_tag", None), "decided": bool(known), "two_level": None}
    if two is not None:
        plan = two.plan
        blob["two_level"] = {
            "residual": [t.detach().cpu() for t in (two.blk_offsets, two.hspa_packed.view(torch.int32), two.hind)],
            "plan_tensors": {k: (getattr(plan, k).detach().cpu().view(torch.int32) if getattr(plan, k) is not None else None)
                             for k in ("panel_ptr", "panel_cols", "panel_bits", "panel_order", "xcd_ptr")},
            "parts_cap": plan.parts.cap if plan.parts is not None else None,
            "plan_scalars": {f.name: getattr(plan, f.name) for f in dataclasses.fields(plan)
                             if isinstance(getattr(plan, f.name), (int, float, str, bool))
                             or f.name in ("num_nodes", "waves", "row_blocks", "tau", "num_ksteps", "num_shared_edges",
                                           "num_resid_edges", "max_panels_per_xcd")},
            "window_xcd_ptr": two.window_xcd_ptr.cpu() if two.window_xcd_ptr is not None else None,
            "num_nodes": two.num_nodes, "num_edges": two.num_edges, "hash_tag": two.hash_tag,
            "format_choice": dict(two.format_choice),
            "fused": None if two.fused is None else {"wave_ptr": two.fused.wave_ptr.cpu(),
                                                     "records": two.fused.records.view(torch.int32).cpu(),
                                                     "num_records": two.fused.num_records},
        }
    torch.save(blob, path)


def load_handle(path: str, device: Optional[torch.device] = None):
    from . import hybrid

    device = torch.device("cuda", torch.cuda.current_device()) if device is None else torch.device(device)
    blob = torch.load(path, map_location="cpu", weights_only=True)
    assert isinstance(blob, dict), f"{path}: not a voltrix handle file"
    assert blob.get("format") == "voltrix-handle-1", f"{path}: not a voltrix handle file"
    blk_offsets, packed, hind = (t.to(device) for t in blob["handle"])
    hspa_packed = packed.view(torch.uint32)
    if blob.get("hash_tag") is not None:
        hspa_packed.hash_tag = blob["hash_tag"]
    tl = blob["two_level"]
    two = None
    if tl is not None:
        pt = {k: (v.to(device) if v is not None else None) for k, v in tl["plan_tensors"].items()}
        pt["panel_bits"] = pt["panel_bits"].view(torch.uint32)
        scalars = {k: tl["plan_scalars"][k] for k in ("num_nodes", "waves", "row_blocks", "tau", "num_ksteps",
                                                       "num_shared_edges", "num_resid_edges", "max_panels_per_xcd")}
        plan = hybrid.PanelPlan(**pt, **scalars)
        if tl.get("parts_cap") is not None:
            plan.parts = hybrid.panel_parts(plan.panel_ptr, tl["parts_cap"], plan.xcd_ptr)
        r0, r1, r2 = (t.to(device) for t in tl["residual"])
        two = hybrid.TwoLevelHandle(r0, r1.view(torch.uint32), r2, plan, tl["num_nodes"], tl["num_edges"],
                                    hash_tag=tl["hash_tag"], format_choice=dict(tl["format_choice"]))
        if tl.get("window_xcd_ptr") is not None:
            two.window_xcd_ptr = tl["window_xcd_ptr"].to(device)
        if tl["fused"] is not None:
            two.fused = hybrid.FusedRecords(tl["fused"]["wave_ptr"].to(device),
                                            tl["fused"]["records"].to(device).view(torch.uint32), tl["fused"]["num_records"])
    if blob["decided"]:
        register(hspa_packed, two)
    return blk_offsets, hspa_packed, hind
```

Baseline: 21440.

## Detect contiguous column runs per kstep and skip column-id gathers in panel SpMM

```diff
diff --git a/include/voltrix_capi.h b/include/voltrix_capi.h
--- a/include/voltrix_capi.h
+++ b/include/voltrix_capi.h
@@ -121,6 +121,11 @@
                                           void* input, int64_t input_rows, void* output, int accumulate, int fs, int depth,
                                           int waves, int row_blocks, int ksteps, int slab_policy, void* out_scale, void* stream,
                                           int* return_code);
+void voltrix_launch_spmm_panel_runs(int bf16, void* panel_ptr, void* panel_cols, void* panel_bits, void* kstep_base,
+                                    void* panel_order, void* parts, int num_parts, void* xcd_ptr, int max_per_xcd,
+                                    void* partials, int num_nodes, int embedding_dim, void* input, int64_t input_rows,
+                                    void* output, int accumulate, int fs, int depth, int waves, int row_blocks, int ksteps,
+                                    int slab_policy, void* out_scale, void* stream, int* return_code);
 void voltrix_launch_combine_panel_partials(void* cuts, int num_cuts, void* partials, void* output, int num_nodes,
                                            int embedding_dim, int panel_rows, int accumulate, void* stream, int* return_code);
 
@@ -160,6 +165,14 @@
                                     int waves, int row_blocks, int tau, void* workspace, void* panel_ptr,
                                     void* resid_node_pointer, int64_t total_ksteps, void* resid_edge_list,
                                     void* panel_cols, void* panel_bits, void* stream, int* return_code);
+
+void voltrix_launch_panel_plan_fill_runs(void* node_pointer, void* edge_list, int num_nodes, int num_cols, int64_t num_edges,
+                                         int waves, int row_blocks, int tau, void* workspace, void* panel_ptr,
+                                         void* resid_node_pointer, int64_t total_ksteps, void* resid_edge_list,
+                                         void* panel_cols, void* panel_bits, void* kstep_base, void* stream,
+                                         int* return_code);
+void voltrix_launch_panel_kstep_base(void* panel_cols, int64_t total_ksteps, int num_cols, void* kstep_base, void* stream,
+                                     int* return_code);
 
 void voltrix_launch_panel_order(void* panel_ptr, int num_panels, int group, void* xcd_ptr, void* order_out, void* stream,
                                 int* return_code);
diff --git a/voltrix-spmm_amd/csrc/capi_spmm_panel.hip b/voltrix-spmm_amd/csrc/capi_spmm_panel.hip
--- a/voltrix-spmm_amd/csrc/capi_spmm_panel.hip
+++ b/voltrix-spmm_amd/csrc/capi_spmm_panel.hip
@@ -22,19 +22,19 @@
              const uint32_t* panel_bits, const int* panel_order, int num_nodes, int embedding_dim, const void* input,
              float* output, int accumulate, const float* out_scale, hipStream_t stream, int64_t input_rows,
              int slab_policy, const int* xcd_ptr, int max_panels_per_xcd, const int* parts = nullptr, int num_parts = 0,
-             float* partials = nullptr) {
+             float* partials = nullptr, const int* kstep_base = nullptr) {
 #define X(FS, D, W, RB, KS)                                                                                          \
   if (fs == FS && depth == D && waves == W && rb == RB && ks == KS)                                                  \
     return voltrix::launch_spmm_panel<voltrix::PanelTile<FS, D, W, RB, KS, BF16>>(                                   \
         panel_ptr, panel_cols, panel_bits, panel_order, num_nodes, embedding_dim, input, output, accumulate, out_scale, \
-        stream, 0, 0, input_rows, slab_policy, xcd_ptr, max_panels_per_xcd, parts, num_parts, partials);
+        stream, 0, 0, input_rows, slab_policy, xcd_ptr, max_panels_per_xcd, parts, num_parts, partials, kstep_base);
   VOLTRIX_PANEL_SPACE(X)
 #undef X
 #define X(FS, D, W, RB)                                                                                              \
   if (fs == FS && depth == D && waves == W && rb == RB && ks == kPipelined)                                           \
     return voltrix::launch_spmm_panel<voltrix::PanelTile<FS, D, W, RB, 1, BF16, true>>(                               \
         panel_ptr, panel_cols, panel_bits, panel_order, num_nodes, embedding_dim, input, output, accumulate, out_scale, \
-        stream, 0, 0, input_rows, slab_policy, xcd_ptr, max_panels_per_xcd, parts, num_parts, partials);
+        stream, 0, 0, input_rows, slab_policy, xcd_ptr, max_panels_per_xcd, parts, num_parts, partials, kstep_base);
   VOLTRIX_PANEL_PIPE_SPACE(X)
 #undef X
   return voltrix::kErrBadConfig;
@@ -98,6 +98,24 @@
                                                    static_cast<const int*>(parts), num_parts, static_cast<float*>(partials));
 }
 
+void voltrix_launch_spmm_panel_runs(int bf16, void* panel_ptr, void* panel_cols, void* panel_bits, void* kstep_base,
+                                    void* panel_order, void* parts, int num_parts, void* xcd_ptr, int max_per_xcd,
+                                    void* partials, int num_nodes, int embedding_dim, void* input, int64_t input_rows,
+                                    void* output, int accumulate, int fs, int depth, int waves, int row_blocks, int ksteps,
+                                    int slab_policy, void* out_scale, void* stream, int* return_code) {
+  if (parts != nullptr && panel_order != nullptr) {
+    *return_code = voltrix::kErrBadShape;
+    return;
+  }
+  auto* const fn = bf16 ? &dispatch<true> : &dispatch<false>;
+  *return_code = fn(fs, depth, waves, row_blocks, ksteps, static_cast<const int*>(panel_ptr),
+                    static_cast<const int*>(panel_cols), static_cast<const uint32_t*>(panel_bits),
+                    static_cast<const int*>(panel_order), num_nodes, embedding_dim, input, static_cast<float*>(output),
+                    accumulate, static_cast<const float*>(out_scale), static_cast<hipStream_t>(stream), input_rows,
+                    slab_policy, static_cast<const int*>(xcd_ptr), max_per_xcd, static_cast<const int*>(parts), num_parts,
+                    static_cast<float*>(partials), static_cast<const int*>(kstep_base));
+}
+
 void voltrix_launch_combine_panel_partials(void* cuts, int num_cuts, void* partials, void* output, int num_nodes,
                                            int embedding_dim, int panel_rows, int accumulate, void* stream, int* return_code) {
   *return_code = voltrix::launch_combine_panel_partials(static_cast<const int*>(cuts), num_cuts,
@@ -136,4 +154,25 @@
                                           static_cast<uint32_t*>(panel_bits), static_cast<hipStream_t>(stream));
 }
 
+void voltrix_launch_panel_plan_fill_runs(void* node_pointer, void* edge_list, int num_nodes, int num_cols, int64_t num_edges,
+                                         int waves, int row_blocks, int tau, void* workspace, void* panel_ptr,
+                                         void* resid_node_pointer, int64_t total_ksteps, void* resid_edge_list,
+                                         void* panel_cols, void* panel_bits, void* kstep_base, void* stream,
+                                         int* return_code) {
+  *return_code = kstep_base == nullptr
+                     ? voltrix::kErrBadShape
+                     : voltrix::panel_plan_fill(static_cast<const int*>(node_pointer), static_cast<const int*>(edge_list),
+                                                num_nodes, num_cols, num_edges, waves, row_blocks, tau, workspace,
+                                                static_cast<const int*>(panel_ptr), static_cast<const int*>(resid_node_pointer),
+                                                total_ksteps, static_cast<int*>(resid_edge_list), static_cast<int*>(panel_cols),
+                                                static_cast<uint32_t*>(panel_bits), static_cast<hipStream_t>(stream),
+                                                static_cast<int*>(kstep_base));
 }
+
+void voltrix_launch_panel_kstep_base(void* panel_cols, int64_t total_ksteps, int num_cols, void* kstep_base, void* stream,
+                                     int* return_code) {
+  *return_code = voltrix::panel_kstep_base(static_cast<const int*>(panel_cols), total_ksteps, num_cols,
+                                           static_cast<int*>(kstep_base), static_cast<hipStream_t>(stream));
+}
+
+}
diff --git a/voltrix-spmm_amd/voltrix/capi.py b/voltrix-spmm_amd/voltrix/capi.py
--- a/voltrix-spmm_amd/voltrix/capi.py
+++ b/voltrix-spmm_amd/voltrix/capi.py
@@ -35,6 +35,7 @@
     "voltrix_launch_spmm_panel_bf16",
     "voltrix_launch_spmm_panel_parts_f16",
     "voltrix_launch_spmm_panel_parts_bf16",
+    "voltrix_launch_spmm_panel_runs",
     "voltrix_launch_combine_panel_partials",
     "voltrix_launch_xcd_ranges_of_work",
     "voltrix_launch_xcd_ranges_of_windows",
@@ -51,6 +52,8 @@
     "voltrix_panel_plan_workspace_bytes",
     "voltrix_launch_panel_plan_count",
     "voltrix_launch_panel_plan_fill",
+    "voltrix_launch_panel_plan_fill_runs",
+    "voltrix_launch_panel_kstep_base",
     "voltrix_launch_panel_order",
     "voltrix_spmm_default_tile",
     "voltrix_spmm_num_tiles",
@@ -392,9 +395,25 @@
 
 
 def launch_spmm_panel(plan, input_ptr, output_ptr, embedding_dim, accumulate, bf16, tile, out_scale, stream,
-                      input_rows: int = 0, slab_policy: int = SLAB_AUTO, partials_ptr: int = 0) -> int:
+                      input_rows: int = 0, slab_policy: int = SLAB_AUTO, partials_ptr: int = 0, use_runs: bool = True) -> int:
     rc = ctypes.c_int(-1)
     parts = getattr(plan, "parts", None)
+    kstep_base = getattr(plan, "kstep_base", None) if use_runs else None
+    if kstep_base is not None:
+        xcd_ptr = parts.xcd_ptr if parts is not None else getattr(plan, "xcd_ptr", None)
+        max_per_xcd = parts.max_parts_per_xcd if parts is not None else (plan.max_panels_per_xcd if xcd_ptr is not None else 0)
+        order = plan.panel_order if parts is None else None
+        lib().voltrix_launch_spmm_panel_runs(
+            ctypes.c_int(int(bool(bf16))), _ptr(plan.panel_ptr), _ptr(plan.panel_cols), _ptr(plan.panel_bits), _ptr(kstep_base),
+            ctypes.c_void_p(order.data_ptr() if order is not None else 0),
+            ctypes.c_void_p(parts.parts.data_ptr() if parts is not None else 0),
+            ctypes.c_int(parts.num_parts if parts is not None else 0),
+            ctypes.c_void_p(xcd_ptr.data_ptr() if xcd_ptr is not None else 0), ctypes.c_int(max_per_xcd),
+            ctypes.c_void_p(partials_ptr), ctypes.c_int(plan.num_nodes), ctypes.c_int(embedding_dim), ctypes.c_void_p(input_ptr),
+            ctypes.c_int64(input_rows), ctypes.c_void_p(output_ptr), ctypes.c_int(int(accumulate)), ctypes.c_int(tile[0]),
+            ctypes.c_int(tile[1]), ctypes.c_int(plan.waves), ctypes.c_int(plan.row_blocks), ctypes.c_int(tile[2]),
+            ctypes.c_int(slab_policy), ctypes.c_void_p(out_scale), ctypes.c_void_p(stream), ctypes.byref(rc))
+        return rc.value
     if parts is not None:
         fn = lib().voltrix_launch_spmm_panel_parts_bf16 if bf16 else lib().voltrix_launch_spmm_panel_parts_f16
         fn(_ptr(plan.panel_ptr), _ptr(plan.panel_cols), _ptr(plan.panel_bits), _ptr(parts.parts), ctypes.c_int(parts.num_parts),
@@ -495,14 +514,29 @@
 
 
 def launch_panel_plan_fill(indptr, indices, num_nodes, num_cols, waves, row_blocks, tau, workspace, panel_ptr,
-                           resid_indptr, total_ksteps, resid_indices, panel_cols, panel_bits, stream) -> None:
-    rc = ctypes.c_int(-1)
+                           resid_indptr, total_ksteps, resid_indices, panel_cols, panel_bits, stream, kstep_base=None) -> None:
+    rc = ctypes.c_int(-1)
+    if kstep_base is not None:
+        lib().voltrix_launch_panel_plan_fill_runs(_ptr(indptr), _ptr(indices), ctypes.c_int(num_nodes), ctypes.c_int(num_cols),
+                                                  ctypes.c_int64(indices.numel()), ctypes.c_int(waves), ctypes.c_int(row_blocks),
+                                                  ctypes.c_int(tau), _ptr(workspace), _ptr(panel_ptr), _ptr(resid_indptr),
+                                                  ctypes.c_int64(total_ksteps), _ptr(resid_indices), _ptr(panel_cols),
+                                                  _ptr(panel_bits), _ptr(kstep_base), ctypes.c_void_p(stream), ctypes.byref(rc))
+        check(rc.value, "voltrix_launch_panel_plan_fill_runs")
+        return
     lib().voltrix_launch_panel_plan_fill(_ptr(indptr), _ptr(indices), ctypes.c_int(num_nodes), ctypes.c_int(num_cols),
                                          ctypes.c_int64(indices.numel()), ctypes.c_int(waves), ctypes.c_int(row_blocks),
                                          ctypes.c_int(tau), _ptr(workspace), _ptr(panel_ptr), _ptr(resid_indptr),
                                          ctypes.c_int64(total_ksteps), _ptr(resid_indices), _ptr(panel_cols),
                                          _ptr(panel_bits), ctypes.c_void_p(stream), ctypes.byref(rc))
     check(rc.value, "voltrix_launch_panel_plan_fill")
+
+
+def launch_panel_kstep_base(panel_cols, total_ksteps, num_cols, kstep_base, stream) -> None:
+    rc = ctypes.c_int(-1)
+    lib().voltrix_launch_panel_kstep_base(_ptr(panel_cols), ctypes.c_int64(total_ksteps), ctypes.c_int(num_cols),
+                                          _ptr(kstep_base), ctypes.c_void_p(stream), ctypes.byref(rc))
+    check(rc.value, "voltrix_launch_panel_kstep_base")
 
 
 def launch_window_order(blk_offsets, num_nodes, order_out, stream, chunk: int = 256) -> None:
diff --git a/voltrix-spmm_amd/voltrix/hybrid.py b/voltrix-spmm_amd/voltrix/hybrid.py
--- a/voltrix-spmm_amd/voltrix/hybrid.py
+++ b/voltrix-spmm_amd/voltrix/hybrid.py
@@ -45,6 +45,7 @@
     xcd_ptr: torch.Tensor = None
     max_panels_per_xcd: int = 0
     parts: PanelParts = None
+    kstep_base: torch.Tensor = None
 
     @property
     def panel_rows(self) -> int:
@@ -185,6 +186,24 @@
     return out_indptr.to(torch.int32), (key - rows * num_cols).to(torch.int32)
 
 
+def kstep_base_torch(panel_cols: torch.Tensor, num_ksteps: int, num_cols: int) -> torch.Tensor:
+    out = torch.full((num_ksteps + 2,), -1, dtype=torch.int32, device=panel_cols.device)
+    if num_ksteps > 0:
+        ids = panel_cols[:KSTEP * num_ksteps].view(num_ksteps, KSTEP).to(torch.int64)
+        first = ids[:, 0]
+        run = (ids == first[:, None] + torch.arange(KSTEP, device=ids.device)).all(dim=1) & (first >= 0) & (first + KSTEP <= num_cols)
+        out[:num_ksteps] = torch.where(run, first, torch.full_like(first, -1)).to(torch.int32)
+    return out
+
+
+def kstep_base_of_plan(plan: "PanelPlan", num_cols: int) -> torch.Tensor:
+    if not plan.panel_cols.is_cuda:
+        return kstep_base_torch(plan.panel_cols, plan.num_ksteps, num_cols)
+    out = torch.empty(plan.num_ksteps + 2, dtype=torch.int32, device=plan.panel_cols.device)
+    capi.launch_panel_kstep_base(plan.panel_cols, plan.num_ksteps, num_cols, out, torch.cuda.current_stream().cuda_stream)
+    return out
+
+
 def empty_plan(num_nodes, waves, row_blocks, tau, device, num_edges):
     np_ = (num_nodes + waves * row_blocks * 16 - 1) // (waves * row_blocks * 16)
     return PanelPlan(panel_ptr=torch.zeros(np_ + 1, dtype=torch.int32, device=device),
@@ -346,9 +365,10 @@
     resid_indices = torch.empty(num_resid, dtype=torch.int32, device=device)
     panel_cols = torch.empty(KSTEP * (total_ksteps + 2), dtype=torch.int32, device=device)
     panel_bits = torch.empty((total_ksteps + 1) * waves * 64, dtype=torch.int32, device=device).view(torch.uint32)
+    kstep_base = torch.empty(total_ksteps + 2, dtype=torch.int32, device=device)
     capi.launch_panel_plan_fill(indptr, indices, num_nodes, num_cols, waves, row_blocks, tau, workspace, panel_ptr,
-                                resid_indptr, total_ksteps, resid_indices, panel_cols, panel_bits, stream)
-    plan = PanelPlan(panel_ptr=panel_ptr, panel_cols=panel_cols, panel_bits=panel_bits,
+                                resid_indptr, total_ksteps, resid_indices, panel_cols, panel_bits, stream, kstep_base)
+    plan = PanelPlan(panel_ptr=panel_ptr, panel_cols=panel_cols, panel_bits=panel_bits, kstep_base=kstep_base,
                      panel_order=longest_first_order(panel_ptr) if total_ksteps > 0 else None,
                      num_nodes=num_nodes, waves=waves, row_blocks=row_blocks, tau=tau, num_ksteps=total_ksteps,
                      num_shared_edges=indices.numel() - num_resid, num_resid_edges=num_resid)
@@ -394,8 +414,9 @@
     bits.index_add_(0, word, torch.ones_like(word) << (16 * (k % 2) + 4 * j + (k % 8) // 2))
     panel_bits = ((bits + 2 ** 31) % 2 ** 32 - 2 ** 31).to(torch.int32).view(torch.uint32)
 
-    plan = PanelPlan(panel_ptr=panel_ptr.to(torch.int32), panel_cols=panel_cols.to(torch.int32), panel_bits=panel_bits,
-                     panel_order=None, num_nodes=num_nodes, waves=waves, row_blocks=row_blocks, tau=tau,
+    panel_cols = panel_cols.to(torch.int32)
+    plan = PanelPlan(panel_ptr=panel_ptr.to(torch.int32), panel_cols=panel_cols, panel_bits=panel_bits,
+                     kstep_base=kstep_base_torch(panel_cols, total_ksteps, num_cols), panel_order=None, num_nodes=num_nodes, waves=waves, row_blocks=row_blocks, tau=tau,
                      num_ksteps=total_ksteps, num_shared_edges=int(rp.numel()),
                      num_resid_edges=int(resid_indices.numel()))
     return resid_indptr, resid_indices, plan
@@ -483,7 +504,7 @@
 
 
 def launch_panel(plan: PanelPlan, feat: torch.Tensor, output: torch.Tensor, accumulate, out_scale=None,
-                 tile=None, stream=None, slab_policy: int = None, defer_combine: bool = False):
+                 tile=None, stream=None, slab_policy: int = None, defer_combine: bool = False, use_runs: bool = True):
     assert feat.is_cuda and feat.is_contiguous() and feat.dtype in (torch.float16, torch.bfloat16)
     assert output.is_cuda and output.is_contiguous() and output.dtype == torch.float32
     f = feat.shape[1]
@@ -502,7 +523,7 @@
     rc = capi.launch_spmm_panel(plan, feat.data_ptr(), output.data_ptr(), f, int(accumulate),
                                 feat.dtype == torch.bfloat16, tile, out_scale.data_ptr() if out_scale is not None else 0,
                                 stream, input_rows=feat.shape[0], slab_policy=slab_policy,
-                                partials_ptr=partials.data_ptr() if partials is not None else 0)
+                                partials_ptr=partials.data_ptr() if partials is not None else 0, use_runs=use_runs)
     capi.check(rc, "voltrix_launch_spmm_panel")
     if partials is None:
         return None
@@ -582,7 +603,7 @@
 def two_level_bytes(two: "TwoLevelHandle") -> int:
     plan = two.plan
     total = handle_bytes((two.blk_offsets, two.hspa_packed, two.hind, plan.panel_ptr, plan.panel_cols, plan.panel_bits,
-                          plan.panel_order))
+                          plan.panel_order, plan.kstep_base))
     if two.fused is not None:
         total += two.fused.nbytes()
     return total
diff --git a/voltrix-spmm_amd/voltrix/include/voltrix/panel_plan.hpp b/voltrix-spmm_amd/voltrix/include/voltrix/panel_plan.hpp
--- a/voltrix-spmm_amd/voltrix/include/voltrix/panel_plan.hpp
+++ b/voltrix-spmm_amd/voltrix/include/voltrix/panel_plan.hpp
@@ -164,11 +164,27 @@
   }
 }
 
+__device__ __forceinline__ int kstep_run_base(const int* __restrict__ ids, const int num_cols) {
+  const int c = ids[0];
+  bool run = c >= 0 && c <= num_cols - kStageK;
+#pragma unroll 8
+  for (int i = 1; i < kStageK; ++i) run = run && ids[i] == c + i;
+  return run ? c : -1;
+}
+
+static __global__ __launch_bounds__(256) void panel_kstep_base_kernel(const int* __restrict__ panel_cols,
+                                                                      const long long total_ksteps, const int num_cols,
+                                                                      int* __restrict__ kstep_base) {
+  const long long k = (long long)blockIdx.x * 256 + threadIdx.x;
+  if (k < total_ksteps) kstep_base[k] = kstep_run_base(panel_cols + k * kStageK, num_cols);
+}
+
 static __global__ __launch_bounds__(kPlanThreads) void panel_plan_fill_kernel(
     const int* __restrict__ indptr, const int* __restrict__ indices, const int num_nodes, const int panel_rows,
     const int waves, const int row_blocks, const unsigned tau, const int nranges, const int* __restrict__ panel_ptr,
     const int* __restrict__ shared_count, const int* __restrict__ resid_indptr, int* __restrict__ resid_indices,
-    int* __restrict__ panel_cols, unsigned* __restrict__ panel_bits ) {
+    int* __restrict__ panel_cols, unsigned* __restrict__ panel_bits , const int num_cols,
+    int* __restrict__ kstep_base ) {
   extern __shared__ __attribute__((aligned(16))) char smem[];
   PlanLds& s = *reinterpret_cast<PlanLds*>(smem);
   const int p = blockIdx.x;
@@ -274,6 +290,12 @@
   const int cnt = shared_count[p];
   const int padded = (cnt + kStageK - 1) / kStageK * kStageK;
   if ((int)threadIdx.x < padded - cnt) panel_cols[ks0 * kStageK + cnt + threadIdx.x] = s.first_col;
+  if (kstep_base == nullptr) return;
+  __threadfence_block();
+  __syncthreads();
+  const int* const cols = panel_cols;
+  for (int k = threadIdx.x; k < padded / kStageK; k += kPlanThreads)
+    kstep_base[ks0 + k] = kstep_run_base(cols + (ks0 + k) * kStageK, num_cols);
 }
 
 static __global__ __launch_bounds__(256) void panel_order_kernel(const int* __restrict__ panel_ptr, const int num_panels,
@@ -372,20 +394,31 @@
 inline int panel_plan_fill(const int* indptr, const int* indices, int num_nodes, int num_cols, long long num_edges,
                            int waves, int row_blocks, int tau, void* workspace, const int* panel_ptr,
                            const int* resid_indptr, long long total_ksteps, int* resid_indices, int* panel_cols,
-                           uint32_t* panel_bits, hipStream_t stream) {
+                           uint32_t* panel_bits, hipStream_t stream, int* kstep_base = nullptr ) {
   if (int rc = plan_check(num_nodes, num_cols, num_edges, waves, row_blocks, tau)) return rc;
   if (((uintptr_t)workspace & 15) || total_ksteps < 0) return kErrBadShape;
   const int panel_rows = waves * row_blocks * 16;
   const int np = (num_nodes + panel_rows - 1) / panel_rows;
   if (hipMemsetAsync(panel_bits, 0, (size_t)(total_ksteps + 1) * waves * kWave * 4, stream) != hipSuccess) return kErrLaunch;
   if (hipMemsetAsync(panel_cols + total_ksteps * kStageK, 0, 2 * kStageK * 4, stream) != hipSuccess) return kErrLaunch;
+  if (kstep_base != nullptr && hipMemsetAsync(kstep_base + total_ksteps, 0xFF, 2 * 4, stream) != hipSuccess) return kErrLaunch;
   if (num_nodes == 0) return kOk;
   const PlanWorkspace ws = plan_workspace(workspace, num_nodes, panel_rows);
   const int nranges = num_cols > 0 ? (num_cols + kPlanRange - 1) / kPlanRange : 1;
   if (int rc = bm_set_lds(panel_plan_fill_kernel, sizeof(PlanLds))) return rc;
   hipLaunchKernelGGL(panel_plan_fill_kernel, dim3(np), dim3(kPlanThreads), sizeof(PlanLds), stream, indptr, indices,
                      num_nodes, panel_rows, waves, row_blocks, (unsigned)tau, nranges, panel_ptr, ws.shared_count,
-                     resid_indptr, resid_indices, panel_cols, panel_bits);
+                     resid_indptr, resid_indices, panel_cols, panel_bits, num_cols, kstep_base);
+  return hipGetLastError() == hipSuccess ? kOk : kErrLaunch;
+}
+
+inline int panel_kstep_base(const int* panel_cols, long long total_ksteps, int num_cols, int* kstep_base, hipStream_t stream) {
+  if (total_ksteps < 0 || total_ksteps >= (1ll << 26) || num_cols < 0 || panel_cols == nullptr || kstep_base == nullptr)
+    return kErrBadShape;
+  if (hipMemsetAsync(kstep_base + total_ksteps, 0xFF, 2 * 4, stream) != hipSuccess) return kErrLaunch;
+  if (total_ksteps == 0) return kOk;
+  hipLaunchKernelGGL(panel_kstep_base_kernel, dim3((unsigned)((total_ksteps + 255) / 256)), dim3(256), 0, stream, panel_cols,
+                     total_ksteps, num_cols, kstep_base);
   return hipGetLastError() == hipSuccess ? kOk : kErrLaunch;
 }
 
diff --git a/voltrix-spmm_amd/voltrix/include/voltrix/spmm_panel_kernels.hpp b/voltrix-spmm_amd/voltrix/include/voltrix/spmm_panel_kernels.hpp
--- a/voltrix-spmm_amd/voltrix/include/voltrix/spmm_panel_kernels.hpp
+++ b/voltrix-spmm_amd/voltrix/include/voltrix/spmm_panel_kernels.hpp
@@ -56,12 +56,30 @@
   return __builtin_bit_cast(half8_t, r);
 }
 
+template <int MAX>
+__device__ __forceinline__ void wait_vmcnt_upto(const int c) {
+  if constexpr (MAX == 0) {
+    wait_vmcnt<0>();
+  } else {
+    if (c >= MAX) wait_vmcnt<MAX>();
+    else wait_vmcnt_upto<MAX - 1>(c);
+  }
+}
+
+__device__ __forceinline__ int run_word_load(const int* base , const int index) {
+  int v;
+  asm volatile("s_load_dword %0, %1, %2" : "=s"(v) : "s"(base), "s"(__builtin_amdgcn_readfirstlane(index * 4)));
+  return v;
+}
+__device__ __forceinline__ void run_word_wait(int& v) { asm volatile("s_waitcnt lgkmcnt(0)" : "+s"(v)); }
+
 template <class T>
 struct PanelArgs {
   using in_t = typename std::conditional<T::BF16, bfloat16_bits, _Float16>::type;
   const int* panel_ptr;
   const int* panel_cols;
   const uint32_t* panel_bits;
+  const int* kstep_base;
   const int* panel_order;
   const int* xcd_ptr;
   const int* parts;
@@ -125,7 +143,6 @@
     const unsigned row_bytes = (unsigned)F * 2u;
     const int dma0 = (wave * DPW) % T::NDMA;
     const char* cbase[DPW];
-    unsigned hr_off[DPW];
 #pragma unroll
     for (int d = 0; d < DPW; ++d) {
       const int r = (dma0 + d) * RPD + lane / LPR;
@@ -135,10 +152,28 @@
       unsigned long long cb = (unsigned long long)((const char*)a.input + (long long)col * 2);
       asm volatile("" : "+v"(cb));
       cbase[d] = (const char*)cb;
-      hr_off[d] = T::BITS_BYTES + 4 * r;
     }
     const int* const cols_base = a.panel_cols + (long long)ks0 * kStageK;
-    auto issue_meta = [&](int s, int ms) {
+    static_assert(KS <= T::WAVES && (DPW * RPD) <= kStageK && kStageK % (DPW * RPD) == 0, "a wave's rows of a step: one k-step");
+    const bool use_runs = !T::PIPE && a.kstep_base != nullptr;
+    const int my_k = (dma0 * RPD) / kStageK;
+    auto run_word = [&](const int s, const int k) -> int {
+      const int sc = s < ngroups ? s : ngroups - 1;
+      return run_word_load(a.kstep_base, ks0 + sc * KS + k);
+    };
+    auto run_base = [&](const int s, const int k) -> int {
+      if (!use_runs) return -1;
+      int v = run_word(s, k);
+      run_word_wait(v);
+      return v;
+    };
+    auto all_runs = [&](const int s) -> bool {
+      bool all = use_runs;
+#pragma unroll
+      for (int k = 0; k < KS; ++k) all = all && run_base(s, k) >= 0;
+      return all;
+    };
+    auto issue_meta = [&](int s, int ms, const bool no_ids = false) {
       const int sc = s < ngroups ? s : ngroups - 1;
       const unsigned dst = meta0 + (unsigned)ms * T::META_BYTES;
       int ml = lane;
@@ -146,32 +181,45 @@
       if (wave < T::NBITS_DMA) {
         const char* src = (const char*)(a.panel_bits + (long long)(ks0 + sc * KS) * (T::WAVES * kWave)) + wave * 1024 + ml * 16;
         if (a.meta_nt) dma_b128_nt(src, dst + wave * 1024); else dma_b128(src, dst + wave * 1024);
-      } else if (wave == T::NBITS_DMA) {
+      } else if (wave == T::NBITS_DMA && !no_ids) {
         const int* src = cols_base + (long long)sc * (KS * kStageK) + ml;
         if (a.meta_nt) dma_b32_nt(src, dst + T::BITS_BYTES); else dma_b32(src, dst + T::BITS_BYTES);
       }
     };
-    auto issue_rows = [&](int ms, int ds) {
+    auto issue_rows = [&](int ms, int ds, const int base = -1) {
       const unsigned mslot = meta0 + (unsigned)ms * T::META_BYTES;
       const unsigned dst = data0 + (unsigned)ds * STAGE_BYTES + (unsigned)dma0 * 1024u;
       unsigned hrow[DPW];
-#pragma unroll
-      for (int d = 0; d < DPW; ++d) hrow[d] = lds_read_b32(mslot + hr_off[d]);
-      wait_lgkmcnt0();
+      int rl = lane;
+      asm volatile("" : "+v"(rl));
+      const unsigned rin = (unsigned)rl / (unsigned)LPR;
+      if (base >= 0) {
+#pragma unroll
+        for (int d = 0; d < DPW; ++d) hrow[d] = rin + (unsigned)(base + (dma0 + d) * RPD - my_k * kStageK);
+      } else {
+#pragma unroll
+        for (int d = 0; d < DPW; ++d)
+          hrow[d] = lds_read_b32(rin * 4u + (mslot + (unsigned)(T::BITS_BYTES + 4 * (dma0 + d) * RPD)));
+        wait_lgkmcnt0();
+      }
 #pragma unroll
       for (int d = 0; d < DPW; ++d)
         if (!(VOLTRIX_PANEL_DIAG & 2)) dma_b128(cbase[d] + (unsigned long long)hrow[d] * row_bytes, dst + d * 1024);
     };
 
     constexpr int PRO = T::PIPE ? D : D - 1;
-#pragma unroll
-    for (int s = 0; s < PRO; ++s) issue_meta(s, s % MS);
+    const bool id_wave = wave == T::NBITS_DMA;
+    unsigned id_mask = 0u;
+#pragma unroll
+    for (int s = 0; s < PRO; ++s) issue_meta(s, s % MS, all_runs(s));
     wait_vmcnt<0>();
     __builtin_amdgcn_s_barrier();
 #pragma unroll
     for (int s = 0; s < PRO; ++s) {
-      issue_rows(s % MS, s % D);
-      issue_meta(s + PRO, (s + PRO) % MS);
+      issue_rows(s % MS, s % D, run_base(s, my_k));
+      const bool no_ids = all_runs(s + PRO);
+      issue_meta(s + PRO, (s + PRO) % MS, no_ids);
+      id_mask = (id_mask << 1) | (no_ids ? 0u : 1u);
     }
 
     const int g = lane >> 4;
@@ -312,7 +360,12 @@
     int ds_t = 0, ms_t = 0;
     int ds_r = (D - 1) % D, ms_r = (D - 1) % MS;
     int ms_m = (2 * D - 2) % MS;
+    int base_r = run_base(D - 1, my_k);
+    bool no_ids_m = id_wave && all_runs(2 * D - 2);
     for (int t = 0; t < ngroups; ++t) {
+      int next_r = -1, next_m[KS];
+#pragma unroll
+      for (int k = 0; k < KS; ++k) next_m[k] = -1;
       const int young = ngroups - 1 - t;
       auto wait_steps = [&](auto per_step) {
         constexpr int VM = decltype(per_step)::value;
@@ -329,15 +382,29 @@
           }
         }
       };
-      if (meta_wave) wait_steps(std::integral_constant<int, T::VM_PER_STEP>{});
-      else wait_steps(std::integral_constant<int, T::VM_PER_STEP_PLAIN>{});
+      if (id_wave && use_runs && !(VOLTRIX_PANEL_DIAG & 16)) {
+        const int n = young < D - 2 ? young : D - 2;
+        wait_vmcnt_upto<T::VM_PER_STEP*(D - 2)>(DPW * n + (int)__builtin_popcount(id_mask & ((1u << n) - 1u)));
+      } else if (meta_wave) {
+        wait_steps(std::integral_constant<int, T::VM_PER_STEP>{});
+      } else {
+        wait_steps(std::integral_constant<int, T::VM_PER_STEP_PLAIN>{});
+      }
       if (!(VOLTRIX_PANEL_DIAG & 4))
         __builtin_amdgcn_s_barrier();
       __builtin_amdgcn_sched_barrier(0);
 
       if (t + D - 1 < ngroups) {
-        issue_rows(ms_r, ds_r);
-        if (!(VOLTRIX_PANEL_DIAG & 16)) issue_meta(t + 2 * D - 2, ms_m);
+        issue_rows(ms_r, ds_r, base_r);
+        if (!(VOLTRIX_PANEL_DIAG & 16)) issue_meta(t + 2 * D - 2, ms_m, no_ids_m);
+        id_mask = (id_mask << 1) | (no_ids_m ? 0u : 1u);
+        if (use_runs) {
+          next_r = run_word(t + D, my_k);
+          if (id_wave) {
+#pragma unroll
+            for (int k = 0; k < KS; ++k) next_m[k] = run_word(t + 2 * D - 1, k);
+          }
+        }
       }
 
       const unsigned mt = meta0 + (unsigned)ms_t * T::META_BYTES;
@@ -387,6 +454,16 @@
                                                                    0, 0);
             }
           }
+        }
+      }
+      if (use_runs) {
+        run_word_wait(next_r);
+        base_r = next_r;
+        no_ids_m = id_wave;
+#pragma unroll
+        for (int k = 0; k < KS; ++k) {
+          run_word_wait(next_m[k]);
+          no_ids_m = no_ids_m && next_m[k] >= 0;
         }
       }
     }
@@ -486,7 +563,8 @@
                              int slab_policy = kSlabAuto, const int* xcd_ptr = nullptr ,
                              int max_panels_per_xcd = 0 ,
                              const int* parts = nullptr , int num_parts = 0,
-                             float* partials = nullptr) {
+                             float* partials = nullptr,
+                             const int* kstep_base = nullptr ) {
   if (num_nodes < 0 || embedding_dim < 0 || accumulate < 0 || accumulate > 2) return kErrBadShape;
   if (parts != nullptr && num_parts < 1) return kErrBadShape;
   if (num_nodes == 0 || embedding_dim == 0) return kOk;
@@ -495,6 +573,7 @@
   a.panel_ptr = panel_ptr;
   a.panel_cols = panel_cols;
   a.panel_bits = panel_bits;
+  a.kstep_base = kstep_base;
   a.panel_order = panel_order;
   a.input = static_cast<const typename PanelArgs<T>::in_t*>(input);
   a.output = output;
@@ -522,7 +601,7 @@
       const int rc = launch_spmm_panel<T>(panel_ptr, panel_cols, panel_bits, panel_order, num_nodes, embedding_dim, input,
                                           output, accumulate, out_scale, stream, s,
                                           total_slabs - s < group ? total_slabs - s : group, input_rows, slab_policy, xcd_ptr,
-                                          max_panels_per_xcd, parts, num_parts, partials);
+                                          max_panels_per_xcd, parts, num_parts, partials, kstep_base);
       if (rc != kOk) return rc;
     }
     return kOk;
diff --git a/voltrix-spmm_amd/voltrix/sidecar.py b/voltrix-spmm_amd/voltrix/sidecar.py
--- a/voltrix-spmm_amd/voltrix/sidecar.py
+++ b/voltrix-spmm_amd/voltrix/sidecar.py
@@ -129,7 +129,7 @@
         blob["two_level"] = {
             "residual": [t.detach().cpu() for t in (two.blk_offsets, two.hspa_packed.view(torch.int32), two.hind)],
             "plan_tensors": {k: (getattr(plan, k).detach().cpu().view(torch.int32) if getattr(plan, k) is not None else None)
-                             for k in ("panel_ptr", "panel_cols", "panel_bits", "panel_order", "xcd_ptr")},
+                             for k in ("panel_ptr", "panel_cols", "panel_bits", "panel_order", "xcd_ptr", "kstep_base")},
             "parts_cap": plan.parts.cap if plan.parts is not None else None,
             "plan_scalars": {f.name: getattr(plan, f.name) for f in dataclasses.fields(plan)
                              if isinstance(getattr(plan, f.name), (int, float, str, bool))
@@ -164,6 +164,9 @@
         scalars = {k: tl["plan_scalars"][k] for k in ("num_nodes", "waves", "row_blocks", "tau", "num_ksteps",
                                                        "num_shared_edges", "num_resid_edges", "max_panels_per_xcd")}
         plan = hybrid.PanelPlan(**pt, **scalars)
+        if plan.kstep_base is None and plan.num_ksteps > 0:
+            num_cols = int(plan.panel_cols[:hybrid.KSTEP * plan.num_ksteps].max()) + 1
+            plan.kstep_base = hybrid.kstep_base_of_plan(plan, num_cols)
         if tl.get("parts_cap") is not None:
             plan.parts = hybrid.panel_parts(plan.panel_ptr, tl["parts_cap"], plan.xcd_ptr)
         r0, r1, r2 = (t.to(device) for t in tl["residual"])
```

New measurement: 21340, median of 2. No clear change (-0.4%).
